# shendurelab/MIPGEN

Hardware: AMD Instinct MI355X
Metric: candidate MIPs scored/sec (SVR) (higher is better)
Workload: dtype f64

## Files before the change

### mipgen_amd/csrc/accel.hip

```cpp
#include "accel_internal.h"

thread_local char g_mipgen_accel_err[512] = "";

extern "C" {

int mipgen_accel_abi_version(void) { return MIPGEN_ACCEL_ABI_VERSION; }
const char* mipgen_accel_last_error(void) { return g_err; }

int mipgen_accel_device_count(void)
{
    int n = 0;
    if (hipGetDeviceCount(&n) != hipSuccess) return 0;
    return n;
}

int mipgen_accel_create(const mipgen_params* params, int device, void* stream, mipgen_accel** out)
{
    if (!params || !out) return fail(MIPGEN_E_INVALID, "null argument");
    *out = nullptr;
    if (params->abi_version != MIPGEN_ACCEL_ABI_VERSION) return fail(MIPGEN_E_INVALID, "abi_version %d != %d", params->abi_version, MIPGEN_ACCEL_ABI_VERSION);
    if (params->n_arm_pairs < 1 || params->n_arm_pairs > MIPGEN_MAX_ARM_PAIRS) return fail(MIPGEN_E_INVALID, "n_arm_pairs out of range");
    if (params->capture_increment <= 0) return fail(MIPGEN_E_INVALID, "capture_increment must be positive (the reference coerces 0 to 1 before this call)");
    if (params->max_capture_size < params->min_capture_size) return fail(MIPGEN_E_INVALID, "max_capture_size < min_capture_size");
    int ndev = mipgen_accel_device_count();
    if (ndev <= 0) return fail(MIPGEN_E_NODEVICE, "no HIP device: libmipgen_accel has no CPU path");
    if (device < 0 || device >= ndev) return fail(MIPGEN_E_INVALID, "device %d out of range (%d devices)", device, ndev);
    HIP_TRY(hipSetDevice(device));

    mipgen_accel* h = new mipgen_accel();
    h->copy.pool = h->scores.pool = h->partials.pool = h->records.pool = h->emitted.pool = h->survivors.pool = h->collapsed.pool = h->pos_region.pool =
        h->pos_local.pool = h->bases.pool = h->letters.pool = h->unmap.pool = h->fmt_pool.pool = h->fmt_text.pool = h->scan_temp.pool = &h->pool;
    h->device = device;
    h->params = *params;
    DevParams& D = h->hp;
    memset(&D, 0, sizeof D);
    D.min_capture = params->min_capture_size; D.max_capture = params->max_capture_size; D.inc = params->capture_increment;
    D.n_sizes_all = n_sizes_all(*params);
    D.n_pairs = params->n_arm_pairs;
    D.check_copy_number = params->check_copy_number; D.logistic_heuristic = params->logistic_heuristic;
    D.score_method = params->score_method;
    D.masked_arm_threshold = params->masked_arm_threshold; D.upper = params->upper_score_limit; D.lower = params->lower_score_limit;
    D.max_arm_copy_product = params->max_arm_copy_product; D.target_arm_copy = params->target_arm_copy;
    D.min_sum = 1 << 30; D.max_sum = 0; D.e_min = D.l_min = 1 << 30; D.e_max = D.l_max = 0;
    for (int i = 0; i <= MIPGEN_MAX_OLIGO; i++) D.len_slot[i] = -1;
    for (int i = 0; i < D.n_pairs; i++) {
        int e = params->arm_ext[i], l = params->arm_lig[i];
        if (e < 2 || l < 2 || e > MIPGEN_MAX_OLIGO || l > MIPGEN_MAX_OLIGO) { delete h; return fail(MIPGEN_E_INVALID, "arm length out of range [2,%d]", MIPGEN_MAX_OLIGO); }
        D.arm_ext[i] = (uint8_t)e; D.arm_lig[i] = (uint8_t)l;
        D.min_sum = std::min(D.min_sum, e + l); D.max_sum = std::max(D.max_sum, e + l);
        D.e_min = std::min(D.e_min, e); D.e_max = std::max(D.e_max, e);
        D.l_min = std::min(D.l_min, l); D.l_max = std::max(D.l_max, l);
        D.len_slot[e] = 0; D.len_slot[l] = 0;
    }
    if (params->min_capture_size - D.max_sum < 1) { delete h; return fail(MIPGEN_E_INVALID, "min_capture_size leaves no scan target (capture size <= arm length sum)"); }
    if ((params->arm_sum_key_max > 0 && params->arm_sum_key_max < D.max_sum) || (params->arm_sum_key_min > 0 && params->arm_sum_key_min > D.min_sum)) {
        delete h; return fail(MIPGEN_E_INVALID, "arm_sum_key_max / arm_sum_key_min inside the arm pairs' own sums [%d, %d]", D.min_sum, D.max_sum);
    }
    D.key_min_sum = params->arm_sum_key_min > 0 ? params->arm_sum_key_min : D.min_sum;
    if (params->min_capture_size - D.max_sum < 3) h->svr_geometry_error = "min_capture_size leaves a scan size < 3 (insert 3-mer frequencies are undefined)";
    int slot = 0;
    for (int i = 0; i <= MIPGEN_MAX_OLIGO; i++) if (D.len_slot[i] == 0) D.len_slot[i] = (int8_t)slot++;
    D.n_len_slots = slot;
    for (int i = 0; i < D.n_pairs;) {
        int j = i, s = D.arm_ext[i] + D.arm_lig[i];
        while (j < D.n_pairs && D.arm_ext[j] + D.arm_lig[j] == s) j++;
        for (int k = i; k < j; k++) D.group_end[k] = (uint16_t)j;
        i = j;
    }
    SvrGeom& G = h->geom;
    memset(&G, 0, sizeof G);
    G.nchunk = (D.n_pairs + SVR_MAX_CHUNK - 1) / SVR_MAX_CHUNK;
    G.chunk_len = (D.n_pairs + G.nchunk - 1) / G.nchunk;
    G.n_e = D.e_max - D.e_min + 1; G.n_l = D.l_max - D.l_min + 1;
    G.group = SVR_GROUP;
    G.wpc = 4;
    while (G.wpc > 1 && G.nchunk * G.wpc * 64 > SVR_MAX_THREADS) G.wpc--;
    if (G.nchunk * G.wpc * 64 > SVR_MAX_THREADS) {
        char msg[128];
        snprintf(msg, sizeof msg, "too many arm pairs for the dense SVR kernel (max %d)", SVR_MAX_CHUNK * (SVR_MAX_THREADS / 64));
        h->svr_geometry_error = msg;
        G.wpc = 1;
    }
    h->geom_few = G;
    h->have_few = false;
    if (h->svr_geometry_error.empty() && G.wpc == 4 && G.chunk_len > 8) {
        SvrGeom& F = h->geom_few;
        const int max_chunks = SVR_MAX_THREADS / 64 / 2;
        F.chunk_len = (D.n_pairs + max_chunks - 1) / max_chunks;
        F.nchunk = (D.n_pairs + F.chunk_len - 1) / F.chunk_len;
        F.wpc = 2;
        h->have_few = F.chunk_len < G.chunk_len && F.nchunk * F.wpc * 64 <= SVR_MAX_THREADS;
    }
    {
        const int n_arm = std::max(G.n_e, G.n_l) | 1;
        for (int strand = 0; strand < 2; strand++) {
            const int up_min = strand ? D.l_min : D.e_min, dn_min = strand ? D.e_min : D.l_min;
            for (int i = 0; i < MIPGEN_MAX_ARM_PAIRS + 16; i++) {
                const int a = std::min(i, D.n_pairs - 1);
                const int e = D.arm_ext[a], l = D.arm_lig[a];
                const uint32_t uU = (uint32_t)(((strand ? l : e) - up_min) * SVR_GROUP * 8);
                const uint32_t uD = (uint32_t)(((D.max_sum - (e + l)) * n_arm + ((strand ? e : l) - dn_min)) * SVR_GROUP * 8);
                D.pair_prog[strand][i] = uU | (uD << 16);
            }
        }
    }

    if (stream) { h->stream = (hipStream_t)stream; h->own_stream = false; }
    else {
        hipError_t e = hipStreamCreateWithFlags(&h->stream, hipStreamNonBlocking);
        if (e != hipSuccess) { delete h; return fail(MIPGEN_E_HIP, "hipStreamCreate: %s", hipGetErrorString(e)); }
        h->own_stream = true;
    }
    for (int i = 0; i < 101; i++) h->hconsts.log10_tab[i] = log10((double)i);
    h->hconsts.ln_base = log(MIPGEN_LOGISTIC_BASE);
    hipError_t e1 = hipMalloc((void**)&h->dp, sizeof(DevParams));
    hipError_t e2 = hipMalloc((void**)&h->dconsts, sizeof(HostConsts));
    if (e1 != hipSuccess || e2 != hipSuccess) { mipgen_accel_destroy(h); return fail(MIPGEN_E_NOMEM, "hipMalloc failed"); }
    if (hipHostMalloc((void**)&h->pb_over, sizeof(unsigned int), hipHostMallocMapped) != hipSuccess) { h->pb_over = nullptr; mipgen_accel_destroy(h); return fail(MIPGEN_E_NOMEM, "hipHostMalloc failed"); }
    *h->pb_over = 0u;
    hipError_t e3 = hipMemcpy(h->dp, &D, sizeof D, hipMemcpyHostToDevice);
    if (e3 == hipSuccess) e3 = hipMemcpy(h->dconsts, &h->hconsts, sizeof(HostConsts), hipMemcpyHostToDevice);
    if (e3 != hipSuccess) { mipgen_accel_destroy(h); return fail(MIPGEN_E_HIP, "hipMemcpy of the run parameters: %s", hipGetErrorString(e3)); }
    { int cus = 0; if (hipDeviceGetAttribute(&cus, hipDeviceAttributeMultiprocessorCount, device) == hipSuccess && cus > 0) h->n_cu = cus; }
    *out = h;
    return MIPGEN_OK;
}

void mipgen_accel_destroy(mipgen_accel* h)
{
    if (!h) return;
    (void)hipSetDevice(h->device);
    if (h->stream) (void)hipStreamSynchronize(h->stream);
    mipgen_reads_release(h);
    mipgen_consensus_release(h);
    h->call_run.release();
    h->locus_run.release();
    h->ins_call.release();
    h->locus_ins.release();
    h->locus_ins_call.release();
    h->model.release(); h->model_t.release(); h->sv_norm.release(); h->sv_coef.release(); h->sv_center.release(); h->regions.release(); h->bases.release(); h->unmap.release(); h->copy.release();
    h->log_tiles.release(); h->svr_tiles.release(); h->ld_tiles.release(); h->scores.release(); h->records.release();
    h->emitted.release(); h->survivors.release(); h->emitted_per_region.release(); h->pos_region.release(); h->pos_local.release();
    h->letters.release(); h->fmt_regions.release(); h->fmt_pool.release(); h->fmt_text.release(); h->scan_temp.release();
    h->fmt_a.release(); h->fmt_b.release(); h->fmt_c.release(); h->fmt_d.release();
    h->region_pos0.release(); h->region_base0.release(); h->col_tiles.release(); h->collapsed.release();
    h->cand_in.release(); h->cand_scores.release(); h->cand_feats.release(); h->cand_records.release(); h->cand_ints.release();
    h->win_img.release();
    h->pb.release(); h->sat.release(); h->surv_svr.release(); h->rs_keep.release(); h->rs_offs.release(); h->rs_idx.release();
    h->svr_tiles_lvl.release(); h->svr_tiles_kept.release(); h->run_bounds.release(); h->run_pbs.release(); h->run_state.release(); h->run_keep.release();
    h->run_offs.release(); h->skip_count.release();
    h->probe_recs.release(); h->probe_bytes.release(); h->probe_lrc.release(); h->probe_order.release();
    h->lrc_seq.release(); h->lrc_out.release(); h->lrc_offs.release(); h->lrc_lens.release(); h->lrc_denoms.release(); h->partials.release();
    h->pool.clear();
    if (h->dp) (void)hipFree(h->dp);
    if (h->dconsts) (void)hipFree(h->dconsts);
    if (h->pb_over) (void)hipHostFree(h->pb_over);
    for (hipEvent_t e : h->ev) if (e) (void)hipEventDestroy(e);
    if (h->own_stream && h->stream) (void)hipStreamDestroy(h->stream);
    delete h;
}

static int build_list_model(mipgen_accel* h, const std::vector<double>& rows, int n_sv)
{
    const int pad = std::max(64, (n_sv + 63) / 64 * 64);
    std::vector<double> center(MIPGEN_N_FEATURES, 0.0), mt((size_t)MIPGEN_N_FEATURES * pad, 0.0), sn((size_t)pad, 0.0), cf((size_t)pad, 0.0);
    for (int j = 0; j < MIPGEN_N_FEATURES; j++) {
        double s = 0.0;
        for (int i = 0; i < n_sv; i++) s += rows[(size_t)i * SV_ROW + j];
        center[(size_t)j] = n_sv ? s / n_sv : 0.0;
    }
    for (int i = 0; i < n_sv; i++) {
        double q = 0.0;
        for (int j = 0; j < MIPGEN_N_FEATURES; j++) {
            const double v = rows[(size_t)i * SV_ROW + j] - center[(size_t)j];
            mt[(size_t)j * pad + i] = v;
            q += v * v;
        }
        sn[(size_t)i] = q + rows[(size_t)i * SV_ROW + SVR_N_EXTRA];
        cf[(size_t)i] = rows[(size_t)i * SV_ROW + SVR_COEF];
    }
    if (h->model_t.reserve(mt.size()) || h->sv_norm.reserve(sn.size()) || h->sv_coef.reserve(cf.size()) || h->sv_center.reserve(center.size())) return MIPGEN_E_NOMEM;
    HIP_TRY(hipMemcpy(h->model_t.p, mt.data(), mt.size() * sizeof(double), hipMemcpyHostToDevice));
    HIP_TRY(hipMemcpy(h->sv_norm.p, sn.data(), sn.size() * sizeof(double), hipMemcpyHostToDevice));
    HIP_TRY(hipMemcpy(h->sv_coef.p, cf.data(), cf.size() * sizeof(double), hipMemcpyHostToDevice));
    HIP_TRY(hipMemcpy(h->sv_center.p, center.data(), center.size() * sizeof(double), hipMemcpyHostToDevice));
    h->n_sv_pad = pad;
    return MIPGEN_OK;
}

int mipgen_accel_set_model(mipgen_accel* h, int32_t n_sv, double gamma, double rho, const double* coef, const double* sv)
{
    if (!h || n_sv < 0 || (n_sv > 0 && (!coef || !sv))) return fail(MIPGEN_E_INVALID, "bad model arguments");
    HIP_TRY(hipSetDevice(h->device));
    std::vector<double> rows((size_t)std::max(n_sv, 1) * SV_ROW, 0.0);
    double s_guard = 0.0;
    for (int i = 0; i < n_sv; i++) {
        double* r = &rows[(size_t)i * SV_ROW];
        const double* x = sv + (size_t)i * MIPGEN_N_FEATURES;
        double ne = 0, ni = 0, nl = 0, nj = 0, tot = 0;
        for (int j = 0; j < MIPGEN_N_FEATURES; j++) {
            r[j] = x[j];
            double q = x[j] * x[j];
            tot += q;
            if (j <= 20) ne += q;
            else if (j >= F_INS && j <= 150) ni += q;
            else if (j >= F_LIG && j <= 172) nl += q;
            else if (j >= F_JUNC && j <= 189) nj += q;
        }
        r[SVR_COEF] = coef[i]; r[SVR_N_EXT] = ne; r[SVR_N_INS] = ni; r[SVR_N_LIG] = nl; r[SVR_N_JUNC] = nj;
        r[SVR_N_TOTAL] = tot; r[SVR_N_EXTRA] = 0.0;
        const int blk_base[3] = {F_EXT, F_INS, F_LIG}, blk_gc[3] = {F_EXT_GC, F_INS_GC, F_LIG_GC}, blk_step[3] = {5, 21, 5}, blk_thr[3] = {15, 63, 15};
        for (int b = 0; b < 3; b++)
            for (int c = 0; c < 4; c++) {
                const int idx = blk_step[b] * c;
                r[SVR_C1 + 4 * b + c] = x[blk_base[b] + idx + (idx >= blk_thr[b])] + ((c == BASE_C || c == BASE_G) ? x[blk_gc[b]] : 0.0);
            }
        s_guard += coef[i] * exp(-gamma * tot);
    }
    if (h->model.reserve(rows.size())) return MIPGEN_E_NOMEM;
    HIP_TRY(hipMemcpy(h->model.p, rows.data(), rows.size() * sizeof(double), hipMemcpyHostToDevice));
    h->n_sv = n_sv; h->gamma = gamma; h->rho = rho; h->s_guard = s_guard - rho;
    h->sum_abs_coef = 0.0;
    for (int i = 0; i < n_sv; i++) h->sum_abs_coef += fabs(coef[i]);
    return build_list_model(h, rows, n_sv);
}

int mipgen_accel_load_model_file(mipgen_accel* h, const char* path)
{
    if (!h || !path) return fail(MIPGEN_E_INVALID, "null argument");
    FILE* fp = fopen(path, "rb");
    if (!fp) return fail(MIPGEN_E_MODEL, "cannot open model file %s (the reference would dereference NULL here, svm.cpp:2507)", path);
    char cmd[128];
    std::string svm_type, kernel_type;
    double gamma = 0, rho = 0;
    int nr_class = 2, total_sv = -1;
    bool ok = true, seen_sv = false;
    while (ok && fscanf(fp, "%127s", cmd) == 1) {
        std::string c(cmd);
        if (c == "svm_type") { ok = fscanf(fp, "%127s", cmd) == 1; svm_type = cmd; }
        else if (c == "kernel_type") { ok = fscanf(fp, "%127s", cmd) == 1; kernel_type = cmd; }
        else if (c == "degree") { int d; ok = fscanf(fp, "%d", &d) == 1; }
        else if (c == "gamma") ok = fscanf(fp, "%lf", &gamma) == 1;
        else if (c == "coef0") { double d; ok = fscanf(fp, "%lf", &d) == 1; }
        else if (c == "nr_class") ok = fscanf(fp, "%d", &nr_class) == 1;
        else if (c == "total_sv") ok = fscanf(fp, "%d", &total_sv) == 1;
        else if (c == "rho") { int n = nr_class * (nr_class - 1) / 2; for (int i = 0; i < n && ok; i++) { double r; ok = fscanf(fp, "%lf", &r) == 1; if (i == 0) rho = r; } }
        else if (c == "label" || c == "nr_sv") { for (int i = 0; i < nr_class && ok; i++) { int d; ok = fscanf(fp, "%d", &d) == 1; } }
        else if (c == "probA" || c == "probB") { int n = nr_class * (nr_class - 1) / 2; for (int i = 0; i < n && ok; i++) { double d; ok = fscanf(fp, "%lf", &d) == 1; } }
        else if (c == "SV") { int ch; while ((ch = getc(fp)) != EOF && ch != '\n') {} seen_sv = true; break; }
        else { fclose(fp); return fail(MIPGEN_E_MODEL, "unknown text in model file: [%s]", cmd); }
    }
    if (!ok || !seen_sv || total_sv < 0) { fclose(fp); return fail(MIPGEN_E_MODEL, "malformed model header in %s", path); }
    if (svm_type != "epsilon_svr" && svm_type != "nu_svr") { fclose(fp); return fail(MIPGEN_E_MODEL, "svm_type %s unsupported (SVR only)", svm_type.c_str()); }
    if (kernel_type != "rbf") { fclose(fp); return fail(MIPGEN_E_MODEL, "kernel_type %s unsupported (rbf only)", kernel_type.c_str()); }
    std::vector<double> sv((size_t)std::max(total_sv, 1) * MIPGEN_N_FEATURES, 0.0), coef((size_t)std::max(total_sv, 1), 0.0), extra((size_t)std::max(total_sv, 1), 0.0);
    char* line = nullptr; size_t cap = 0;
    int got = 0;
    while (got < total_sv && getline(&line, &cap, fp) >= 0) {
        char* save = nullptr;
        char* p = strtok_r(line, " \t\n", &save);
        if (!p) continue;
        coef[got] = strtod(p, nullptr);
        for (int k = 1; k < nr_class - 1; k++) strtok_r(nullptr, " \t", &save);
        for (;;) {
            char* idx = strtok_r(nullptr, ":", &save);
            char* val = strtok_r(nullptr, " \t\n", &save);
            if (!val) break;
            long j = strtol(idx, nullptr, 10);
            double v = strtod(val, nullptr);
            if (j >= 1 && j <= MIPGEN_N_FEATURES) sv[(size_t)got * MIPGEN_N_FEATURES + (j - 1)] = v;
            else if (j > MIPGEN_N_FEATURES) extra[got] += v * v;
        }
        got++;
    }
    free(line);
    fclose(fp);
    if (got != total_sv) return fail(MIPGEN_E_MODEL, "model file has %d SV lines, header says %d", got, total_sv);
    int rc = mipgen_accel_set_model(h, total_sv, gamma, rho, coef.data(), sv.data());
    if (rc) return rc;
    bool any_extra = false;
    for (double x : extra) any_extra |= x != 0.0;
    if (any_extra) {
        std::vector<double> rows((size_t)total_sv * SV_ROW);
        HIP_TRY(hipMemcpy(rows.data(), h->model.p, rows.size() * sizeof(double), hipMemcpyDeviceToHost));
        double sg = 0;
        for (int i = 0; i < total_sv; i++) {
            rows[(size_t)i * SV_ROW + SVR_N_EXTRA] = extra[i];
            rows[(size_t)i * SV_ROW + SVR_N_TOTAL] += extra[i];
            sg += coef[i] * exp(-gamma * rows[(size_t)i * SV_ROW + SVR_N_TOTAL]);
        }
        HIP_TRY(hipMemcpy(h->model.p, rows.data(), rows.size() * sizeof(double), hipMemcpyHostToDevice));
        h->s_guard = sg - rho;
        return build_list_model(h, rows, total_sv);
    }
    return MIPGEN_OK;
}

int mipgen_accel_model_info(const mipgen_accel* h, int32_t* n_sv, double* gamma, double* rho)
{
    if (!h) return fail(MIPGEN_E_INVALID, "null handle");
    if (n_sv) *n_sv = h->n_sv;
    if (gamma) *gamma = h->gamma;
    if (rho) *rho = h->rho;
    return MIPGEN_OK;
}

int mipgen_accel_set_window_candidates(mipgen_accel* h, int64_t max_candidates)
{
    if (!h || max_candidates < 0) return fail(MIPGEN_E_INVALID, "bad arguments");
    h->window_cap = max_candidates;
    return MIPGEN_OK;
}

int mipgen_accel_set_window_breaks(mipgen_accel* h, const int32_t* first_regions, int32_t n)
{
    if (!h || n < 0 || (n > 0 && !first_regions)) return fail(MIPGEN_E_INVALID, "bad arguments");
    for (int i = 0; i < n; i++)
        if (first_regions[i] < 0 || (i > 0 && first_regions[i] <= first_regions[i - 1])) return fail(MIPGEN_E_INVALID, "window breaks must be ascending batch indices");
    h->window_breaks.assign(first_regions, first_regions + n);
    return MIPGEN_OK;
}

int mipgen_accel_set_print_exact(mipgen_accel* h, int32_t on)
{
    if (!h) return fail(MIPGEN_E_INVALID, "null handle");
    h->print_exact = on != 0;
    return MIPGEN_OK;
}

int mipgen_accel_set_logistic_subruns(mipgen_accel* h, int32_t n)
{
    if (!h || n < 0 || n > 8) return fail(MIPGEN_E_INVALID, "bad arguments");
    h->ld_subruns = n;
    h->logistic_tiles_ready = false;
    return MIPGEN_OK;
}

int mipgen_accel_set_sv_split(mipgen_accel* h, int32_t n_split)
{
    if (!h || n_split < 0 || n_split > 64) return fail(MIPGEN_E_INVALID, "n_split must be in [0, 64] (0 = automatic)");
    h->sv_split = n_split;
    return MIPGEN_OK;
}


int mipgen_accel_upload_regions(mipgen_accel* h, const mipgen_region* regions, int32_t n, mipgen_grid* grids_out)
{
    if (!h || n < 0 || (n > 0 && !regions)) return fail(MIPGEN_E_INVALID, "bad arguments");
    DIAG_CLOCK("upload");
    HIP_TRY(hipSetDevice(h->device));
    const mipgen_params& P = h->params;
    const DevParams& D = h->hp;
    h->cur_window = -1;
    h->windows.clear(); h->win_state.clear();
    h->hregions.assign((size_t)n, DevRegion());
    h->grids.assign((size_t)n, mipgen_grid());
    int64_t seq_total = 0, copy_total = 0, unmap_total = 0, cand_total = 0, pos_total = 0, cand_max = 0;
    int n_resident = 0;
    for (int i = 0; i < n; i++) n_resident += regions[i].copy == MIPGEN_COPY_RESIDENT;
    if (n_resident) {
        bool same = n_resident == n && h->resident_lens.size() == (size_t)n;
        for (int i = 0; same && i < n; i++) same = h->resident_lens[(size_t)i] == regions[i].seq_len;
        if (!same) return fail(MIPGEN_E_INVALID, "MIPGEN_COPY_RESIDENT: the batch is not the one mipgen_accel_count_oligo_copies_resident counted (regions, order, seq_len)");
    } else {
        h->resident_lens.clear();
    }
    for (int i = 0; i < n; i++) {
        const mipgen_region& R = regions[i];
        if (!R.seq || R.seq_len <= 0) return fail(MIPGEN_E_INVALID, "region %d has no sequence", i);
        if (R.seq_stop - R.seq_start + 1 != R.seq_len) return fail(MIPGEN_E_INVALID, "region %d: seq_len %d != seq_stop-seq_start+1 = %d", i, R.seq_len, R.seq_stop - R.seq_start + 1);
        DevRegion& d = h->hregions[i];
        mipgen_grid& g = h->grids[i];
        grid_of(P, D, R, &g);
        g.offset = cand_total;
        d.seq_off = seq_total;
        d.seq_len = R.seq_len; d.seq_start = R.seq_start; d.seq_stop = R.seq_stop;
        d.start_fl = R.start_flanked; d.stop_fl = R.stop_flanked;
        d.first_pos = g.first_pos; d.n_pos = g.n_pos; d.k0 = g.first_size_index; d.n_sizes = g.n_sizes;
        d.copy_off = R.copy ? copy_total : -1;
        d.unmap_off = R.unmappable ? unmap_total : -1;
        memcpy(d.lrc, R.long_range_content, sizeof d.lrc);
        seq_total += R.seq_len;
        if (R.copy) copy_total += (int64_t)D.n_len_slots * R.seq_len;
        if (R.unmappable) unmap_total += (int64_t)D.n_sizes_all * R.seq_len;
        cand_total += g.count;
        pos_total += g.n_pos;
        cand_max = std::max(cand_max, g.count);
    }
    if (pos_total > INT32_MAX) return fail(MIPGEN_E_INVALID, "batch has %lld scan positions (max %d): split the design", (long long)pos_total, INT32_MAX);
    DIAG_LAP("layout");
    uint8_t code_lut[256];
    for (int c = 0; c < 256; c++) code_lut[c] = base_code((char)c);
    std::vector<uint8_t> hb((size_t)std::max<int64_t>(seq_total, 1));
    std::vector<char> hl((size_t)std::max<int64_t>(seq_total, 1));
    std::vector<uint8_t> hu((size_t)std::max<int64_t>(unmap_total, 1));
    for (int i = 0; i < n; i++) {
        const mipgen_region& R = regions[i];
        const DevRegion& d = h->hregions[i];
        uint8_t* b = &hb[(size_t)d.seq_off];
        memcpy(&hl[(size_t)d.seq_off], R.seq, (size_t)R.seq_len);
        const char* ms = R.masked_seq ? R.masked_seq : R.seq;
        if (R.snp_class) for (int k = 0; k < R.seq_len; k++) b[k] = (uint8_t)(code_lut[(uint8_t)R.seq[k]] | (ms[k] == 'N' ? BASE_MASKED_BIT : 0) | ((R.snp_class[k] & 3) << BASE_SNP_SHIFT));
        else for (int k = 0; k < R.seq_len; k++) b[k] = (uint8_t)(code_lut[(uint8_t)R.seq[k]] | (ms[k] == 'N' ? BASE_MASKED_BIT : 0));
        if (R.unmappable) memcpy(&hu[(size_t)d.unmap_off], R.unmappable, (size_t)D.n_sizes_all * R.seq_len);
    }
    DIAG_LAP("pack");
    if (h->letters.reserve(hl.size())) return MIPGEN_E_NOMEM;
    HIP_TRY(hipMemcpyAsync(h->letters.p, hl.data(), hl.size(), hipMemcpyHostToDevice, h->stream));
    HIP_TRY(hipStreamSynchronize(h->stream));
    if (h->regions.reserve((size_t)std::max(n, 1)) || h->bases.reserve(hb.size()) || h->copy.reserve((size_t)std::max<int64_t>(copy_total, 1)) || h->unmap.reserve(hu.size()) ||
        h->survivors.reserve((size_t)std::max<int64_t>(2 * pos_total, 1)) || h->emitted_per_region.reserve((size_t)std::max(n, 1)) ||
        h->pos_region.reserve((size_t)std::max<int64_t>(pos_total, 1)) || h->pos_local.reserve((size_t)std::max<int64_t>(pos_total, 1)))
        return MIPGEN_E_NOMEM;

    DIAG_LAP("input buffers");
    int64_t cap = h->window_cap;
    if (cap <= 0) {
        size_t free_b = 0, total_b = 0;
        HIP_TRY(hipMemGetInfo(&free_b, &total_b));
        const int64_t have = (int64_t)(h->scores.cap * 8 + h->records.cap * 8 + h->emitted.cap) + (int64_t)free_b + (int64_t)h->pool.held();
        cap = std::max<int64_t>(1, (int64_t)((double)have * 0.85) / 17);
        cap = std::min<int64_t>(cap, std::max<int64_t>((int64_t)1 << 30, cand_max));
    }
    if (cand_max > cap && h->window_cap > 0) cap = cand_max;
    if (cand_max > cap) return fail(MIPGEN_E_NOMEM, "a single region has %lld dense candidates; device memory holds %lld", (long long)cand_max, (long long)cap);
    {
        Window w;
        size_t nb = 0;
        for (int i = 0; i < n; i++) {
            const mipgen_grid& g = h->grids[i];
            while (nb < h->window_breaks.size() && h->window_breaks[nb] < i) nb++;
            const bool forced = nb < h->window_breaks.size() && h->window_breaks[nb] == i;
            if (w.r1 > w.r0 && (forced || w.n_cand + g.count > cap)) {
                h->windows.push_back(w);
                Window nw; nw.r0 = nw.r1 = i; nw.cand0 = w.cand0 + w.n_cand; nw.pos0 = w.pos0 + w.n_pos;
                w = nw;
            }
            h->hregions[i].out_off = w.n_cand;
            w.n_cand += g.count; w.n_pos += g.n_pos; w.r1 = i + 1;
        }
        h->windows.push_back(w);
        h->win_state.assign(h->windows.size(), 0);
    }
    int64_t win_cand_max = 0;
    for (const Window& w : h->windows) win_cand_max = std::max(win_cand_max, w.n_cand);

    std::vector<int64_t> rpos0((size_t)n + 1, 0);
    h->h_region_base0.assign((size_t)n + 1, 0);
    for (int i = 0; i < n; i++) {
        const DevRegion& d = h->hregions[i];
        const int max_scan = D.max_capture - d.k0 * D.inc - D.min_sum;
        const int64_t nb = (d.n_pos > 0 && d.n_sizes > 0) ? (int64_t)d.n_pos + max_scan - 1 : 0;
        rpos0[(size_t)i + 1] = rpos0[(size_t)i] + d.n_pos;
        h->h_region_base0[(size_t)i + 1] = h->h_region_base0[(size_t)i] + 2 * nb;
    }
    std::vector<CollapseTile> ct;
    for (Window& w : h->windows) {
        w.col_tile0 = (int)ct.size();
        w.base0 = h->h_region_base0[(size_t)w.r0]; w.n_base_entries = h->h_region_base0[(size_t)w.r1] - w.base0;
        w.log_tile0 = w.n_log_tiles = w.svr_tile0 = w.n_svr_tiles = w.ld_tile0 = w.n_ld_tiles = 0;
        for (int i = w.r0; i < w.r1; i++) {
            const DevRegion& d = h->hregions[i];
            if (d.n_pos <= 0 || d.n_sizes <= 0) continue;
            for (int64_t j0 = 0; 2 * j0 < h->h_region_base0[(size_t)i + 1] - h->h_region_base0[(size_t)i]; j0 += 128) { CollapseTile t = {i, (int32_t)j0}; ct.push_back(t); }
        }
        w.n_col_tiles = (int)ct.size() - w.col_tile0;
    }
    h->record_tiles_ready = h->logistic_tiles_ready = h->svr_tiles_ready = false;
    h->svr_batch_error.clear();
    h->ld_lds = 0; h->log_span_max = 0; h->svr_lds = 0;
    DIAG_LAP("tiles");
    if (h->scores.reserve((size_t)std::max<int64_t>(win_cand_max, 1)) || h->records.reserve((size_t)std::max<int64_t>(win_cand_max, 1)) ||
        h->emitted.reserve((size_t)std::max<int64_t>(win_cand_max, 1)))
        return MIPGEN_E_NOMEM;
    if (h->region_pos0.reserve((size_t)n + 1) || h->region_base0.reserve((size_t)n + 1) || h->col_tiles.reserve(std::max<size_t>(ct.size(), 1)) ||
        h->collapsed.reserve((size_t)std::max<int64_t>(h->h_region_base0[(size_t)n], 1)))
        return MIPGEN_E_NOMEM;
    HIP_TRY(hipMemcpyAsync(h->region_pos0.p, rpos0.data(), ((size_t)n + 1) * sizeof(int64_t), hipMemcpyHostToDevice, h->stream));
    HIP_TRY(hipMemcpyAsync(h->region_base0.p, h->h_region_base0.data(), ((size_t)n + 1) * sizeof(int64_t), hipMemcpyHostToDevice, h->stream));
    if (!ct.empty()) HIP_TRY(hipMemcpyAsync(h->col_tiles.p, ct.data(), ct.size() * sizeof(CollapseTile), hipMemcpyHostToDevice, h->stream));
    HIP_TRY(mipgen_launch_fill_pos_map(h->stream, h->region_pos0.p, n, pos_total, h->pos_region.p, h->pos_local.p));
    if (n > 0) HIP_TRY(hipMemcpyAsync(h->regions.p, h->hregions.data(), (size_t)n * sizeof(DevRegion), hipMemcpyHostToDevice, h->stream));
    HIP_TRY(hipMemcpyAsync(h->bases.p, hb.data(), hb.size(), hipMemcpyHostToDevice, h->stream));
    if (copy_total && !n_resident) {
        int64_t max_block = 0;
        for (int i = 0; i < n; i++) if (regions[i].copy) max_block = std::max(max_block, (int64_t)D.n_len_slots * regions[i].seq_len);
        const int64_t chunk = std::min(copy_total, std::max<int64_t>((int64_t)1 << 20, max_block));
        PinnedPair<int32_t> pin;
        HIP_TRY(pin.alloc((size_t)chunk));
        int cur = 0;
        int64_t fill = 0, base = 0;
        auto flush = [&]() -> hipError_t {
            if (fill == 0) return hipSuccess;
            hipError_t e = hipMemcpyAsync(h->copy.p + base, pin.buf[cur], (size_t)fill * sizeof(int32_t), hipMemcpyHostToDevice, h->stream);
            if (e == hipSuccess) e = hipEventRecord(pin.done[cur], h->stream);
            if (e != hipSuccess) return e;
            pin.busy[cur] = true;
            base += fill; fill = 0; cur ^= 1;
            return pin.wait(cur);
        };
        for (int i = 0; i < n; i++) {
            const mipgen_region& R = regions[i];
            if (!R.copy) continue;
            const int64_t block = (int64_t)D.n_len_slots * R.seq_len;
            if (fill + block > chunk) HIP_TRY(flush());
            if (h->hregions[i].copy_off != base + fill) return fail(MIPGEN_E_INVALID, "internal: copy table offsets out of order");
            for (int len = 0; len <= MIPGEN_MAX_OLIGO; len++) {
                const int s = D.len_slot[len];
                if (s < 0) continue;
                int32_t* dst = pin.buf[cur] + fill + (int64_t)s * R.seq_len;
                if (R.copy[len]) memcpy(dst, R.copy[len], (size_t)R.seq_len * sizeof(int32_t));
                else memset(dst, 0, (size_t)R.seq_len * sizeof(int32_t));
            }
            fill += block;
        }
        HIP_TRY(flush());
        HIP_TRY(pin.wait(0)); HIP_TRY(pin.wait(1));
    }
    if (unmap_total) HIP_TRY(hipMemcpyAsync(h->unmap.p, hu.data(), hu.size(), hipMemcpyHostToDevice, h->stream));
    HIP_TRY(hipStreamSynchronize(h->stream));
    DIAG_LAP("buffers + copies");
    h->n_regions = n; h->n_cand = cand_total; h->total_pos = pos_total;
    h->ev_used.assign(h->windows.size(), 0);
#ifdef MIPGEN_DIAG
    fprintf(stderr, "[mipgen_accel] batch: %d regions, %lld candidates in %zu window(s)\n", n, (long long)cand_total, h->windows.size());
#endif
    if (grids_out) memcpy(grids_out, h->grids.data(), (size_t)n * sizeof(mipgen_grid));
    return MIPGEN_OK;
}

int64_t mipgen_accel_batch_candidates(const mipgen_accel* h) { return h ? h->n_cand : 0; }
int32_t mipgen_accel_window_count(const mipgen_accel* h) { return h ? (int32_t)h->windows.size() : 0; }

int mipgen_accel_window_info(const mipgen_accel* h, int32_t w, int32_t* first_region, int32_t* n_regions, int64_t* first_candidate,
                             int64_t* n_candidates, int64_t* first_position, int64_t* n_positions)
{
    if (!h || w < 0 || w >= (int32_t)h->windows.size()) return fail(MIPGEN_E_INVALID, "window %d out of range", w);
    const Window& W = h->windows[(size_t)w];
    if (first_region) *first_region = W.r0;
    if (n_regions) *n_regions = W.r1 - W.r0;
    if (first_candidate) *first_candidate = W.cand0;
    if (n_candidates) *n_candidates = W.n_cand;
    if (first_position) *first_position = W.pos0;
    if (n_positions) *n_positions = W.n_pos;
    return MIPGEN_OK;
}


double mipgen_accel_last_kernel_ms(mipgen_accel* h, int32_t which)
{
    if (h && which == 4) return h->kmer_count_ms;
    if (h && which == 5) return h->list_svr_ms;
    if (h && which == 6) return h->list_feat_ms;
    if (h && which == 7) return h->reads_assign_ms;
    if (h && which == 8) return h->sample_assign_ms;
    if (h && which == 9) return h->consensus_vote_ms;
    if (h && which == 10) return h->consensus_sort_ms;
    if (h && which == 11) return h->pileup_ms;
    if (h && which == 12) return h->gapped_ms;
    if (h && which == 13) return h->call_ms;
    if (h && which == 14) return h->locus_ms;
    if (h && which == 15) return h->insertions_ms;
    if (h && which == 16) return h->ins_call_ms;
    if (h && which == 17) return h->locus_ins_ms;
    if (h && which == 18) return h->tag_merge_ms;
    if (h && which == 19) return h->deletions_ms;
    if (!h || !h->timing) return -1.0;
    if (hipSetDevice(h->device) != hipSuccess) return -1.0;
    double total = 0.0;
    bool any = false;
    for (size_t w = 0; w < h->windows.size() && 4 * (w + 1) <= h->ev.size(); w++) {
        const uint8_t used = h->ev_used[w];
        if (!(used & 1)) continue;
        hipEvent_t* ev = &h->ev[4 * w];
        float ms = 0.f;
        hipError_t e = hipSuccess;
        if (which == 3) {
            if (!(used & 2)) continue;
            if (hipEventSynchronize(ev[3]) != hipSuccess) return -1.0;
            e = hipEventElapsedTime(&ms, ev[2], ev[3]);
        } else {
            if (hipEventSynchronize(ev[2]) != hipSuccess) return -1.0;
            if (which == 0) e = hipEventElapsedTime(&ms, ev[1], ev[2]);
            else if (which == 2) e = hipEventElapsedTime(&ms, ev[0], ev[1]);
            else e = hipEventElapsedTime(&ms, ev[0], ev[2]);
        }
        if (e != hipSuccess) return -1.0;
        total += ms; any = true;
    }
    return any ? total : -1.0;
}

int mipgen_accel_set_timing(mipgen_accel* h, int32_t enabled)
{
    if (!h) return fail(MIPGEN_E_INVALID, "null handle");
    h->timing = enabled != 0;
    std::fill(h->ev_used.begin(), h->ev_used.end(), 0);
    return MIPGEN_OK;
}

}
```

### mipgen_amd/csrc/accel_internal.h

```cpp
#pragma once
#include <hip/hip_runtime.h>

#include <algorithm>
#include <chrono>
#include <cmath>
#include <cstdarg>
#include <cstdio>
#include <cstdlib>
#include <cstring>
#include <string>
#include <unordered_map>
#include <vector>

#include "kernels.h"
#include "logistic_device.h"

extern thread_local char g_mipgen_accel_err[512];
#define g_err g_mipgen_accel_err
static inline int fail(int code, const char* fmt, ...)
{
    va_list ap;
    va_start(ap, fmt);
    vsnprintf(g_err, sizeof g_err, fmt, ap);
    va_end(ap);
    return code;
}
#define HIP_TRY(expr)                                                                             \
    do {                                                                                          \
        hipError_t e__ = (expr);                                                                  \
        if (e__ != hipSuccess) return fail(MIPGEN_E_HIP, "%s: %s", #expr, hipGetErrorString(e__)); \
    } while (0)

struct Window {
    int r0 = 0, r1 = 0;
    int64_t cand0 = 0, n_cand = 0;
    int64_t pos0 = 0, n_pos = 0;
    int log_tile0 = 0, n_log_tiles = 0, svr_tile0 = 0, n_svr_tiles = 0, col_tile0 = 0, n_col_tiles = 0, ld_tile0 = 0, n_ld_tiles = 0;
    int n_svr_few = 0;
    std::vector<int> lvl_tile0;
    int lvl0_few = 0;
    int64_t base0 = 0, n_base_entries = 0;
};

struct DevPool {
    struct Block { void* p; size_t bytes; };
    std::vector<Block> blocks;
    size_t held() const { size_t n = 0; for (const Block& b : blocks) n += b.bytes; return n; }
    void* take(size_t bytes, size_t* got)
    {
        int best = -1;
        for (int i = 0; i < (int)blocks.size(); i++)
            if (blocks[(size_t)i].bytes >= bytes && blocks[(size_t)i].bytes / 4 <= bytes && (best < 0 || blocks[(size_t)i].bytes < blocks[(size_t)best].bytes)) best = i;
        if (best < 0) return nullptr;
        void* p = blocks[(size_t)best].p;
        *got = blocks[(size_t)best].bytes;
        blocks.erase(blocks.begin() + best);
        return p;
    }
    void give(void* p, size_t bytes) { if (bytes >= ((size_t)1 << 20)) blocks.push_back({p, bytes}); else (void)hipFree(p); }
    void clear() { for (const Block& b : blocks) (void)hipFree(b.p); blocks.clear(); }
};

template <typename T>
struct DevBuf {
    T* p = nullptr;
    size_t cap = 0;
    DevPool* pool = nullptr;
    int reserve(size_t n)
    {
        if (n <= cap) return 0;
        release();
        size_t want = n + std::min<size_t>(n / 8, (size_t)1 << 20) + 64;
        if (pool) {
            size_t got = 0;
            if (void* q = pool->take(want * sizeof(T), &got)) { p = (T*)q; cap = got / sizeof(T); return 0; }
        }
        hipError_t e = hipMalloc((void**)&p, want * sizeof(T));
        if (e != hipSuccess && pool && !pool->blocks.empty()) {
            (void)hipGetLastError();
            pool->clear();
            e = hipMalloc((void**)&p, want * sizeof(T));
        }
        if (e != hipSuccess) { p = nullptr; return fail(MIPGEN_E_NOMEM, "hipMalloc(%zu bytes): %s", want * sizeof(T), hipGetErrorString(e)); }
        cap = want;
        return 0;
    }
    void release()
    {
        if (p) { if (pool) pool->give(p, cap * sizeof(T)); else (void)hipFree(p); }
        p = nullptr; cap = 0;
    }
};
static inline size_t padded(size_t count, size_t size) { return (count + count / 8 + 64) * size; }

struct SortedPairs {
    DevBuf<uint64_t> keys, keys_sorted;
    DevBuf<uint32_t> ids, ids_sorted;
    DevBuf<char> temp;
    size_t held() const { return (keys.cap + keys_sorted.cap) * 8 + (ids.cap + ids_sorted.cap) * 4 + temp.cap; }
    void release() { keys.release(); keys_sorted.release(); ids.release(); ids_sorted.release(); temp.release(); }
    static size_t bytes(size_t n, size_t scratch) { return 2 * padded(n, 8) + 2 * padded(n, 4) + padded(scratch, 1); }
    static hipError_t scratch_bytes(hipStream_t st, int64_t n, int end_bit, int64_t n_runs, int64_t n_scan, size_t* scratch)
    {
        size_t t_sort = 0, t_runs = 0, t_scan = 0;
        hipError_t e = mipgen_consensus_sort(st, nullptr, &t_sort, nullptr, nullptr, nullptr, nullptr, n, end_bit);
        if (e == hipSuccess && n_runs) e = mipgen_consensus_runs(st, nullptr, &t_runs, nullptr, n_runs, nullptr, nullptr, nullptr);
        if (e == hipSuccess && n_scan) e = mipgen_consensus_scan_u32(st, nullptr, &t_scan, nullptr, nullptr, n_scan);
        *scratch = std::max<size_t>(std::max(t_sort, std::max(t_runs, t_scan)), 1);
        return e;
    }
    int reserve(size_t n, size_t scratch) { return keys.reserve(n) || keys_sorted.reserve(n) || ids.reserve(n) || ids_sorted.reserve(n) || temp.reserve(scratch) ? MIPGEN_E_NOMEM : MIPGEN_OK; }
    hipError_t sort(hipStream_t st, int64_t n, int end_bit) { size_t all = temp.cap; return mipgen_consensus_sort(st, temp.p, &all, keys.p, keys_sorted.p, ids.p, ids_sorted.p, n, end_bit); }
    hipError_t runs(hipStream_t st, int64_t n, uint64_t* run_keys, int32_t* run_counts, unsigned long long* n_runs) { size_t all = temp.cap; return mipgen_consensus_runs(st, temp.p, &all, keys_sorted.p, n, run_keys, run_counts, n_runs); }
    hipError_t scan_u32(hipStream_t st, const int32_t* in, uint32_t* out, int64_t n) { size_t all = temp.cap; return mipgen_consensus_scan_u32(st, temp.p, &all, in, out, n); }
    hipError_t scan_i64(hipStream_t st, const int64_t* in, int64_t* out, int64_t n) { size_t all = temp.cap; return mipgen_consensus_scan_i64(st, temp.p, &all, in, out, n); }
};

template <typename T>
struct PinnedPair {
    T* buf[2] = {nullptr, nullptr};
    hipEvent_t done[2] = {nullptr, nullptr};
    bool busy[2] = {false, false};
    hipError_t alloc(size_t n)
    {
        for (int b = 0; b < 2; b++) {
            hipError_t e = hipHostMalloc((void**)&buf[b], std::max<size_t>(n, 1) * sizeof(T), hipHostMallocDefault);
            if (e != hipSuccess) return e;
            e = hipEventCreateWithFlags(&done[b], hipEventDisableTiming);
            if (e != hipSuccess) return e;
        }
        return hipSuccess;
    }
    hipError_t wait(int b) { hipError_t e = busy[b] ? hipEventSynchronize(done[b]) : hipSuccess; busy[b] = false; return e; }
    ~PinnedPair() { for (int b = 0; b < 2; b++) { if (done[b]) { if (busy[b]) (void)hipEventSynchronize(done[b]); (void)hipEventDestroy(done[b]); } if (buf[b]) (void)hipHostFree(buf[b]); } }
};

enum : uint8_t {
    WIN_SURVIVORS = 1,
    WIN_MASK = 2,
    WIN_COLLAPSED = 4,
    WIN_SURV_SVR = 8,
    WIN_TEXT = 16,
};

struct RescoreList {
    DevBuf<mipgen_candidate> cands; DevBuf<int64_t> idx; DevBuf<double> vals; DevBuf<unsigned int> count;
    void release() { cands.release(); idx.release(); vals.release(); count.release(); }
};

struct ReadsSession;

struct RowScratch {
    DevBuf<int32_t> mol_len;
    DevBuf<int64_t> pos_off;
    DevBuf<uint32_t> start;
    DevBuf<uint2> units;
    DevBuf<PileupCounters> pctr;
    size_t held() const { return mol_len.cap * 4 + pos_off.cap * 8 + start.cap * 4 + units.cap * 8 + pctr.cap * sizeof(PileupCounters); }
    void release() { mol_len.release(); pos_off.release(); start.release(); units.release(); pctr.release(); }
};
struct CountScratch {
    RowScratch row;
    DevBuf<int32_t> counts;
    DevBuf<int64_t> proj_off;
    DevBuf<uint32_t> list;
    DevBuf<uint8_t> mol_seq, need, proj;
    DevBuf<GappedCounters> ctr;
    size_t held() const { return row.held() + counts.cap * 4 + proj_off.cap * 8 + list.cap * 4 + mol_seq.cap + need.cap + proj.cap + ctr.cap * sizeof(GappedCounters); }
    void release() { row.release(); counts.release(); proj_off.release(); list.release(); mol_seq.release(); need.release(); proj.release(); ctr.release(); }
};
struct RowArgs;
struct PoolArgs {
    bool have = false;
    std::vector<int32_t> mol_len;
    std::string mol_seq;
    int32_t min_family = 1, min_quality = 0, max_indel = 0, bg_max_ppm = 0;
    void remember(const RowArgs& A, int64_t n_pos, int32_t bg_max_ppm_);
};
struct PoolState : PoolArgs {
    DevBuf<int32_t> pool;
    mipgen_gapped_totals last{0, 0, 0, 0, 0, 0, 0, 0};
    bool have_last = false;
    void drop() { have = have_last = false; }
    void release() { drop(); pool.release(); }
};
struct CallScratch {
    CountScratch pile, gapped;
    PoolState state;
    DevBuf<uint8_t> ref;
    size_t held() const { return pile.held() + gapped.held() + state.pool.cap * 4 + ref.cap; }
    void release() { state.release(); pile.release(); gapped.release(); ref.release(); }
};
struct CallRun {
    DevBuf<mipgen_call_record> cand, records;
    SortedPairs pairs;
    DevBuf<CallCounters> ctr;
    DevBuf<int32_t> counts, pool;
    DevBuf<uint8_t> ref;
    int64_t n_calls = -1;
    size_t held() const { return (cand.cap + records.cap) * sizeof(mipgen_call_record) + pairs.held() + ctr.cap * sizeof(CallCounters) + (counts.cap + pool.cap) * 4 + ref.cap; }
    void release() { cand.release(); records.release(); pairs.release(); ctr.release(); counts.release(); pool.release(); ref.release(); n_calls = -1; }
};
struct LocusPlan {
    DevBuf<int64_t> plan;
    SortedPairs pairs;
    DevBuf<uint32_t> src, first;
    int64_t n_pos = 0, n_loci = 0;
    bool have = false;
    size_t held() const { return plan.cap * 8 + pairs.held() + (src.cap + first.cap) * 4; }
    void release_transient() { plan.release(); pairs.release(); }
    void release() { release_transient(); src.release(); first.release(); have = false; n_pos = n_loci = 0; }
};
struct LocusRun {
    LocusPlan plan;
    DevBuf<int32_t> counts, merged;
    DevBuf<LocusCounters> ctr;
    size_t held() const { return plan.held() + (counts.cap + merged.cap) * 4 + ctr.cap * sizeof(LocusCounters); }
    void release() { plan.release(); counts.release(); merged.release(); ctr.release(); }
};
struct LocusScratch {
    LocusPlan plan;
    DevBuf<uint8_t> ref;
    CountScratch pile, gapped;
    DevBuf<int32_t> merged;
    DevBuf<LocusCounters> ctr;
    PoolState state;
    size_t held() const { return plan.held() + ref.cap + pile.held() + gapped.held() + (merged.cap + state.pool.cap) * 4 + ctr.cap * sizeof(LocusCounters); }
    void release() { plan.release(); ref.release(); pile.release(); gapped.release(); merged.release(); ctr.release(); state.release(); }
};
struct InsScratch {
    CountScratch count;
    DevBuf<int32_t> anchors;
    DevBuf<InsCounters> ctr;
    SortedPairs pairs;
    DevBuf<mipgen_insertion_record> records;
    int64_t n_alleles = -1;
    size_t event_held() const { return pairs.held() + records.cap * sizeof(mipgen_insertion_record); }
    size_t table_held() const { return anchors.cap * 4 + ctr.cap * sizeof(InsCounters); }
    void release() { count.release(); anchors.release(); ctr.release(); pairs.release(); records.release(); n_alleles = -1; }
};
struct DelScratch {
    CountScratch count;
    DevBuf<int32_t> sites;
    DevBuf<DelCounters> ctr;
    SortedPairs pairs;
    DevBuf<mipgen_deletion_record> records;
    int64_t n_alleles = -1;
    size_t event_held() const { return pairs.held() + records.cap * sizeof(mipgen_deletion_record); }
    size_t table_held() const { return sites.cap * 4 + ctr.cap * sizeof(DelCounters); }
    void release() { count.release(); sites.release(); ctr.release(); pairs.release(); records.release(); n_alleles = -1; }
};
struct InsPool {
    PoolArgs args;
    DevBuf<int32_t> S;
    DevBuf<uint64_t> pool_keys;
    DevBuf<InsPoolSums> pool_sums;
    DevBuf<InsPoolCounters> ctr;
    SortedPairs pairs;
    DevBuf<InsPoolSums> sums;
    DevBuf<uint32_t> run_start;
    DevBuf<int32_t> run_counts;
    int64_t n_pos = 0, rows = 0, n_entries = 0, n_alleles = 0;
    size_t entry_held() const { return pairs.held() + pool_keys.cap * 8 + (sums.cap + pool_sums.cap) * sizeof(InsPoolSums) + (run_start.cap + run_counts.cap) * 4; }
    size_t table_held() const { return S.cap * 4 + ctr.cap * sizeof(InsPoolCounters); }
    void release_transient() { pairs.release(); sums.release(); run_start.release(); run_counts.release(); }
    void release() { args.have = false; release_transient(); S.release(); pool_keys.release(); pool_sums.release(); ctr.release(); n_pos = rows = n_entries = n_alleles = 0; }
};
struct InsCallRun {
    CallRun run;
    DevBuf<mipgen_insertion_call_record> out;
    DevBuf<mipgen_insertion_record> records;
    DevBuf<int32_t> span, pool_span;
    DevBuf<uint64_t> pool_keys;
    DevBuf<InsPoolSums> pool_sums;
    int64_t n_calls = -1;
    size_t call_held() const { return run.held() + out.cap * sizeof(mipgen_insertion_call_record); }
    size_t upload_held() const { return records.cap * sizeof(mipgen_insertion_record) + (span.cap + pool_span.cap) * 4 + pool_keys.cap * 8 + pool_sums.cap * sizeof(InsPoolSums); }
    void release() { run.release(); out.release(); records.release(); span.release(); pool_span.release(); pool_keys.release(); pool_sums.release(); n_calls = -1; }
};
struct LocusInsMap {
    DevBuf<uint32_t> own, prev;
    bool have = false;
    size_t held() const { return (own.cap + prev.cap) * 4; }
    void release() { own.release(); prev.release(); have = false; }
};
struct LocusInsFold {
    SortedPairs pairs;
    DevBuf<uint32_t> run_start;
    DevBuf<mipgen_insertion_record> records;
    DevBuf<int32_t> anchors;
    DevBuf<LocusInsCounters> ctr;
    int64_t n_alleles = -1;
    size_t pair_held() const { return pairs.held() + run_start.cap * 4 + records.cap * sizeof(mipgen_insertion_record); }
    size_t table_held() const { return anchors.cap * 4 + ctr.cap * sizeof(LocusInsCounters); }
    void release() { pairs.release(); run_start.release(); records.release(); anchors.release(); ctr.release(); n_alleles = -1; }
};
struct LocusInsRun {
    LocusPlan plan;
    LocusInsMap map;
    DevBuf<mipgen_insertion_record> records;
    DevBuf<int32_t> anchors;
    LocusInsFold fold;
    size_t upload_held() const { return records.cap * sizeof(mipgen_insertion_record) + anchors.cap * 4; }
    void release() { plan.release(); map.release(); records.release(); anchors.release(); fold.release(); }
};
struct LocusInsScratch {
    LocusInsMap map;
    InsPool pool;
    void drop() { map.have = false; pool.args.have = false; }
    void release() { map.release(); pool.release(); }
};
struct ConsensusResult {
    int64_t n_groups = 0, ext_bytes = 0, lig_bytes = 0;
    int64_t n = 0, rows = 0;
    CountScratch pile, gapped;
    CallScratch call;
    LocusScratch locus;
    InsScratch ins;
    InsPool ins_pool;
    LocusInsScratch locus_ins;
    DelScratch del;
    DevBuf<uint64_t> keys;
    DevBuf<int32_t> family;
    DevBuf<int64_t> ext_off, lig_off;
    DevBuf<uint8_t> ext_seq, ext_qual, lig_seq, lig_qual;
    mipgen_tag_merge_totals tag_totals{0, 0, 0, 0, 0};
    bool merged = false;
    DevBuf<uint64_t> raw_keys;
    DevBuf<int32_t> raw_family, raw_root;
    ConsensusView view() const { return {keys.p, family.p, ext_off.p, lig_off.p, ext_seq.p, ext_qual.p, lig_seq.p, lig_qual.p, n_groups}; }
    void release() { keys.release(); family.release(); ext_off.release(); lig_off.release(); ext_seq.release(); ext_qual.release(); lig_seq.release(); lig_qual.release(); raw_keys.release(); raw_family.release(); raw_root.release(); pile.release(); gapped.release(); call.release(); locus.release(); ins.release(); ins_pool.release(); locus_ins.release(); del.release(); }
};

struct mipgen_accel {
    int device = 0;
    hipStream_t stream = nullptr;
    bool own_stream = false;
    mipgen_params params;
    DevParams hp;
    DevParams* dp = nullptr;
    HostConsts* dconsts = nullptr;
    HostConsts hconsts;
    SvrGeom geom;
    SvrGeom geom_few;
    bool have_few = false;
    int n_sv = 0;
    double gamma = 0, rho = 0, s_guard = 0;
    DevBuf<double> model;
    std::string svr_geometry_error;
    std::string svr_batch_error;
    bool record_tiles_ready = false, logistic_tiles_ready = false, svr_tiles_ready = false;
    int sv_split = 0;
    int ld_subruns = 0;
    int n_cu = 256;
    int n_regions = 0;
    int64_t n_cand = 0;
    int64_t total_pos = 0;
    std::vector<DevRegion> hregions;
    std::vector<mipgen_grid> grids;
    DevBuf<DevRegion> regions;
    DevBuf<uint8_t> bases, unmap;
    DevBuf<char> letters;
    DevBuf<FmtRegion> fmt_regions;
    DevBuf<char> fmt_pool, fmt_text, scan_temp;
    DevBuf<int64_t> fmt_a, fmt_b, fmt_c, fmt_d;
    int64_t fmt_bytes = 0;
    DevPool pool;
    DevBuf<int32_t> copy;
    std::vector<int32_t> resident_lens;
    std::vector<mipgen_big_copy> big_copies;
    DevBuf<LogTile> log_tiles;
    DevBuf<SvrTile> svr_tiles, ld_tiles;
    size_t ld_lds = 0;
    int log_span_max = 0;
    size_t svr_lds = 0;
    int64_t window_cap = 0;
    std::vector<int32_t> window_breaks;
    std::vector<Window> windows;
    int cur_window = -1;
    std::vector<uint8_t> win_state;
    DevBuf<double> scores, partials;
    DevBuf<uint64_t> records;
    DevBuf<uint8_t> emitted;
    DevBuf<mipgen_survivor> survivors;
    DevBuf<unsigned long long> emitted_per_region;
    DevBuf<int32_t> pos_region, pos_local;
    std::vector<int64_t> h_region_base0;
    DevBuf<int64_t> region_pos0, region_base0;
    DevBuf<CollapseTile> col_tiles;
    DevBuf<int32_t> collapsed;
    bool print_exact = true;
    double sum_abs_coef = 0.0;
    RescoreList pb;
    DevBuf<double> surv_svr;
    DevBuf<int64_t> rs_keep, rs_offs, rs_idx;
    RescoreList sat;
    DevBuf<uint8_t> win_img;
    std::vector<int64_t> win_roff;
    std::vector<int32_t> win_lens;
    int win_sizes = 0;
    int64_t win_total = 0;
    bool dyn_skip = false;
    int svr_levels = 1;
    DevBuf<SvrTile> svr_tiles_lvl, svr_tiles_kept;
    DevBuf<uint32_t> run_bounds;
    DevBuf<double> run_pbs;
    DevBuf<uint8_t> run_state;
    DevBuf<int64_t> run_keep, run_offs;
    DevBuf<unsigned long long> skip_count;
    unsigned long long skipped_total = 0;
    bool skip_count_valid = false;
    unsigned int* pb_over = nullptr;
    DevBuf<double> model_t, sv_norm, sv_coef, sv_center;
    int n_sv_pad = 0;
    double kmer_count_ms = -1.0;
    double list_feat_ms = -1.0, list_svr_ms = -1.0;
    int64_t kmer_genome_bytes = 0;
    DevBuf<mipgen_candidate> cand_in;
    DevBuf<double> cand_scores, cand_feats;
    DevBuf<uint64_t> cand_records;
    DevBuf<mipgen_candidate_ints> cand_ints;
    DevBuf<ProbeRec> probe_recs;
    DevBuf<uint8_t> probe_bytes;
    DevBuf<double> probe_lrc;
    DevBuf<int32_t> probe_order;
    DevBuf<char> lrc_seq;
    DevBuf<double> lrc_out;
    DevBuf<int64_t> lrc_offs;
    DevBuf<int32_t> lrc_lens, lrc_denoms;
    ReadsSession* reads = nullptr;
    int64_t reads_key_cap = 0;
    double reads_assign_ms = -1.0;
    double sample_assign_ms = -1.0;
    ConsensusResult* consensus = nullptr;
    double consensus_vote_ms = -1.0;
    double consensus_sort_ms = -1.0;
    double tag_merge_ms = -1.0;
    double pileup_ms = -1.0;
    double gapped_ms = -1.0;
    CallRun call_run;
    double call_ms = -1.0;
    LocusRun locus_run;
    double locus_ms = -1.0;
    double insertions_ms = -1.0;
    InsCallRun ins_call;
    double ins_call_ms = -1.0;
    LocusInsRun locus_ins;
    InsCallRun locus_ins_call;
    double locus_ins_ms = -1.0;
    double deletions_ms = -1.0;
    bool timing = false;
    std::vector<hipEvent_t> ev;
    std::vector<uint8_t> ev_used;
};

static inline int n_sizes_all(const mipgen_params& P)
{
    if (P.max_capture_size < P.min_capture_size) return 0;
    return (P.max_capture_size - P.min_capture_size) / P.capture_increment + 1;
}

static inline void grid_of(const mipgen_params& P, const DevParams& D, const mipgen_region& R, mipgen_grid* g)
{
    int cur = R.start_flanked - P.max_capture_size + (P.arm_sum_key_max > 0 ? P.arm_sum_key_max : D.max_sum);
    if (cur < 0) cur = 0;
    g->first_pos = cur + 1;
    g->n_pos = std::max(0, R.stop_flanked - cur);
    int K = D.n_sizes_all, k0 = 0;
    while (k0 < K) {
        int C = P.max_capture_size - k0 * P.capture_increment;
        if (C > R.stop_flanked - R.start_flanked + P.max_mip_overlap && C - P.capture_increment >= P.min_capture_size) k0++;
        else break;
    }
    g->first_size_index = k0;
    g->n_sizes = K - k0;
    g->count = (int64_t)g->n_pos * g->n_sizes * P.n_arm_pairs * 2;
    g->offset = 0;
}

static inline bool win_has(const mipgen_accel* h, int w, uint8_t bits) { return w >= 0 && (h->win_state[(size_t)w] & bits) == bits; }
static inline void win_set(mipgen_accel* h, int w, uint8_t bits) { h->win_state[(size_t)w] |= bits; }

static inline uint8_t base_code(char c)
{
    switch (c) {
        case 'A': return BASE_A; case 'C': return BASE_C; case 'G': return BASE_G; case 'T': return BASE_T;
        case 'N': return BASE_N; case '-': return BASE_DASH; default: return BASE_OTHER;
    }
}

#ifdef MIPGEN_DIAG
struct DiagClock {
    const char* what; std::chrono::steady_clock::time_point t = std::chrono::steady_clock::now();
    explicit DiagClock(const char* w) : what(w) {}
    void lap(const char* stage) { const auto n_ = std::chrono::steady_clock::now(); fprintf(stderr, "[mipgen_accel] %s: %s %.3f s\n", what, stage, std::chrono::duration<double>(n_ - t).count()); t = n_; }
};
#define DIAG_CLOCK(name) DiagClock diag_clock(name)
#define DIAG_LAP(stage) diag_clock.lap(stage)
#else
#define DIAG_CLOCK(name) do { } while (0)
#define DIAG_LAP(stage) do { } while (0)
#endif

static inline int free_device_bytes(size_t* free_b)
{
    size_t total_b = 0;
    HIP_TRY(hipMemGetInfo(free_b, &total_b));
    return MIPGEN_OK;
}
struct IdleOnExit { hipStream_t s; bool idle = false; hipError_t wait() { idle = true; return hipStreamSynchronize(s); } ~IdleOnExit() { if (!idle) (void)hipStreamSynchronize(s); } };

struct SpanTimer {
    bool on;
    hipStream_t st;
    std::vector<hipEvent_t> ev;
    ~SpanTimer() { for (hipEvent_t e : ev) (void)hipEventDestroy(e); }
    void mark() { hipEvent_t e = nullptr; if (on && (on = hipEventCreate(&e) == hipSuccess)) { ev.push_back(e); (void)hipEventRecord(e, st); } }
    int add_to(double* sum) const
    {
        int n = 0;
        float ms = 0.f;
        for (size_t k = 0; on && k + 1 < ev.size(); k += 2)
            if (hipEventElapsedTime(&ms, ev[k], ev[k + 1]) == hipSuccess) { *sum += ms; n++; }
        return n;
    }
};

extern "C" {
int mipgen_pick_sv_split(int n_tiles, int n_sv, int n_cu);
int mipgen_ensure_events(mipgen_accel* h);
int mipgen_ensure_tiles(mipgen_accel* h, int32_t method);
int mipgen_pb_check(mipgen_accel* h);
void mipgen_reads_release(mipgen_accel* h);
void mipgen_consensus_release(mipgen_accel* h);
}
```

### mipgen_amd/csrc/accel_score.hip

```cpp
#include "accel_internal.h"

extern "C" {

int mipgen_pb_check(mipgen_accel* h)
{
    if (!h->pb_over || *h->pb_over == 0u) return MIPGEN_OK;
    const unsigned int v = *h->pb_over;
    *h->pb_over = 0u;
    return fail(MIPGEN_E_STATE, "print-exact re-score: %u scores on a 6-digit rounding boundary did not fit the re-score list "
                                "(mipgen_accel_set_print_exact(h, 0) waives the guarantee)", v);
}

struct RescoreLimits { unsigned int cap; double tol_rel, tol_abs; };
static RescoreLimits rescore_limits(const mipgen_accel* h, int kind, int method, int64_t n)
{
    const bool svr = method == MIPGEN_SCORE_SVR;
    int64_t cap;
    if (kind == RESCORE_SATURATED) cap = std::min<int64_t>(n / 4096 + 4096, (int64_t)1 << 20);
    else if (kind == RESCORE_SURV) cap = svr ? std::min<int64_t>(n / 256 + 1024, (int64_t)1 << 22) : std::min<int64_t>(n / 4096 + 64, (int64_t)1 << 20);
    else cap = svr ? std::min<int64_t>(n / 1024 + 4096, (int64_t)1 << 24) : std::min<int64_t>(n / 8192 + 256, (int64_t)1 << 22);
    return {(unsigned int)cap, svr ? 1e-10 : 1e-11, svr ? 1e-13 * std::max(1.0, h->sum_abs_coef) : 1e-300};
}

static ListSrc list_src(const mipgen_accel* h, const mipgen_candidate* cands, const ProbeSrc* ps)
{
    if (ps) return {LIST_PROBES, {}, *ps};
    return {LIST_BATCH, {h->dp, h->regions.p, cands, h->bases.p, h->copy.p, h->unmap.p}, {}};
}

static int rescore(mipgen_accel* h, const RescoreSrc& src, int method, const ProbeSrc* ps = nullptr)
{
    const bool sat = src.kind == RESCORE_SATURATED;
    if (!sat && (!h->print_exact || src.n <= 0 || (method == MIPGEN_SCORE_SVR && h->n_sv <= 0))) return MIPGEN_OK;
    const RescoreLimits lim = rescore_limits(h, src.kind, method, src.n);
    RescoreList& L = sat ? h->sat : h->pb;
    if ((!ps && L.cands.reserve(lim.cap)) || L.idx.reserve(lim.cap) || L.vals.reserve(lim.cap) || L.count.reserve(1)) return MIPGEN_E_NOMEM;
    if (sat) HIP_TRY(mipgen_launch_index_candidates(h->stream, h->dp, h->regions.p, src.r0, src.r1, L.idx.p, L.count.p, lim.cap, L.cands.p));
    else {
        HIP_TRY(hipMemsetAsync(L.count.p, 0, sizeof(unsigned int), h->stream));
        HIP_TRY(mipgen_launch_print_boundary_scan(h->stream, h->dp, h->regions.p, &src, lim.tol_rel, lim.tol_abs, L.cands.p, L.idx.p, L.count.p, lim.cap, h->n_cu));
    }
    ListSrc listed = list_src(h, L.cands.p, ps);
    if (ps) { listed.probes.sel = L.idx.p; listed.probes.order = nullptr; }
    HIP_TRY(mipgen_launch_candidates(h->stream, (int)lim.cap, listed, h->dconsts, h->model.p, h->n_sv, h->gamma, h->rho, method, L.vals.p, nullptr, nullptr, nullptr, 1,
                                     L.count.p));
    HIP_TRY(mipgen_launch_scatter_scores(h->stream, L.vals.p, L.idx.p, lim.cap, L.count.p, src.scores, src.surv, sat ? nullptr : h->pb_over));
    return MIPGEN_OK;
}

static int device_scan_i64(mipgen_accel* h, const int64_t* in, int64_t* out, int64_t n)
{
    size_t temp_bytes = 0;
    HIP_TRY(mipgen_scan_i64(h->stream, nullptr, &temp_bytes, in, out, n));
    if (h->scan_temp.reserve(temp_bytes + 16)) return MIPGEN_E_NOMEM;
    HIP_TRY(mipgen_scan_i64(h->stream, h->scan_temp.p, &temp_bytes, in, out, n));
    return MIPGEN_OK;
}

static int fix_survivor_print_boundaries(mipgen_accel* h, int w, int method)
{
    const Window& W = h->windows[(size_t)w];
    return rescore(h, {RESCORE_SURV, 2 * W.n_pos, nullptr, nullptr, nullptr, h->survivors.p + 2 * W.pos0, W.r0, W.r1, W.cand0}, method);
}

static bool list_is_batched(int n, int method, bool want_scores) { return method == MIPGEN_SCORE_SVR && n >= 256 && want_scores; }
static bool list_runs_feature_kernel(int n, int method, bool want_scores, bool ints) { return list_is_batched(n, method, want_scores) && !ints; }

static int score_list(mipgen_accel* h, int n, int method, bool want_scores, bool features, bool ints, hipEvent_t* le, const ProbeSrc* ps = nullptr)
{
    const bool batched = list_is_batched(n, method, want_scores);
    if (batched && h->cand_feats.reserve((size_t)n * MIPGEN_N_FEATURES)) return MIPGEN_E_NOMEM;
    const bool time_list = le && batched && !ints && h->timing;
    if (time_list) { for (int k = 0; k < 3; k++) HIP_TRY(hipEventCreate(&le[k])); HIP_TRY(hipEventRecord(le[0], h->stream)); }
    const ListSrc src = list_src(h, h->cand_in.p, ps);
    if (list_runs_feature_kernel(n, method, want_scores, ints))
        HIP_TRY(mipgen_launch_features_batch(h->stream, n, src, h->dconsts, h->cand_records.p, h->cand_feats.p));
    else
        HIP_TRY(mipgen_launch_candidates(h->stream, n, src, h->dconsts, h->model.p, h->n_sv, h->gamma, h->rho, method, batched ? nullptr : h->cand_scores.p,
                                         h->cand_records.p, (features || batched) ? h->cand_feats.p : nullptr, ints ? h->cand_ints.p : nullptr, 0, nullptr));
    if (time_list) HIP_TRY(hipEventRecord(le[1], h->stream));
    if (batched) HIP_TRY(mipgen_launch_svr_gemm(h->stream, n, h->cand_feats.p, h->cand_records.p, h->model_t.p, h->sv_norm.p, h->sv_coef.p, h->sv_center.p, h->n_sv_pad,
                                            h->gamma, h->rho, h->cand_scores.p));
    if (time_list) HIP_TRY(hipEventRecord(le[2], h->stream));
    if (!batched) return MIPGEN_OK;
    return rescore(h, {ps ? RESCORE_PROBES : RESCORE_LIST, n, h->cand_scores.p, h->cand_records.p, ps ? nullptr : h->cand_in.p, nullptr, 0, 0, 0}, MIPGEN_SCORE_SVR, ps);
}

static int svr_window_via_list(mipgen_accel* h, const Window& W)
{
    const int64_t CH = (int64_t)1 << 19;
    const size_t n_max = (size_t)std::min<int64_t>(CH, std::max<int64_t>(W.n_cand, 1));
    if (h->cand_in.reserve(n_max) || h->cand_records.reserve(n_max) || h->cand_feats.reserve(n_max * MIPGEN_N_FEATURES)) return MIPGEN_E_NOMEM;
    for (int64_t c0 = 0; c0 < W.n_cand; c0 += CH) {
        const int n = (int)std::min<int64_t>(CH, W.n_cand - c0);
        HIP_TRY(mipgen_launch_dense_candidates(h->stream, h->dp, h->regions.p, W.r0, W.r1, c0, n, h->cand_in.p));
        HIP_TRY(mipgen_launch_features_batch(h->stream, n, list_src(h, h->cand_in.p, nullptr), h->dconsts, h->cand_records.p, h->cand_feats.p));
        HIP_TRY(mipgen_launch_svr_gemm(h->stream, n, h->cand_feats.p, h->cand_records.p, h->model_t.p, h->sv_norm.p, h->sv_coef.p, h->sv_center.p, h->n_sv_pad,
                                       h->gamma, h->rho, h->scores.p + c0));
        HIP_TRY(mipgen_launch_dense_list_fix(h->stream, n, h->records.p + c0, h->rho, h->s_guard, h->scores.p + c0));
    }
    return MIPGEN_OK;
}

static int score_window_impl(mipgen_accel* h, int w, int32_t method, bool fix_dense = true)
{
    if (int rc = mipgen_ensure_tiles(h, method)) return rc;
    const Window& W = h->windows[(size_t)w];
    const bool svr_via_list = method == MIPGEN_SCORE_SVR && (!h->svr_geometry_error.empty() || !h->svr_batch_error.empty());
    if (svr_via_list && h->model_t.p == nullptr) return fail(MIPGEN_E_MODEL, "SVR scoring requested but no model is loaded");
    hipEvent_t* ev = nullptr;
    if (h->timing) { if (mipgen_ensure_events(h)) return MIPGEN_E_HIP; ev = &h->ev[4 * (size_t)w]; }
    if (ev) HIP_TRY(hipEventRecord(ev[0], h->stream));
    unsigned int sat_cap = 0;
    if (method == MIPGEN_SCORE_LOGISTIC) {
        sat_cap = rescore_limits(h, RESCORE_SATURATED, method, W.n_cand).cap;
        if (h->sat.idx.reserve(sat_cap) || h->sat.count.reserve(1)) return MIPGEN_E_NOMEM;
        HIP_TRY(hipMemsetAsync(h->sat.count.p, 0, sizeof(unsigned int), h->stream));
    }
    if (method == MIPGEN_SCORE_LOGISTIC && h->ld_lds > 0)
        HIP_TRY(mipgen_launch_logistic_dense(h->stream, W.n_ld_tiles, h->ld_lds, h->dp, h->regions.p, h->ld_tiles.p + W.ld_tile0, h->bases.p, h->copy.p,
                                             h->unmap.p, h->dconsts, h->scores.p, h->records.p, h->sat.idx.p, h->sat.count.p, sat_cap));
    else
        HIP_TRY(mipgen_launch_records_logistic(h->stream, method == MIPGEN_SCORE_LOGISTIC, W.n_log_tiles, h->log_span_max, h->dp, h->regions.p,
                                               h->log_tiles.p + W.log_tile0, h->bases.p, h->copy.p, h->unmap.p, h->dconsts, h->scores.p, h->records.p,
                                               sat_cap ? h->sat.idx.p : nullptr, sat_cap ? h->sat.count.p : nullptr, sat_cap));
    if (ev) HIP_TRY(hipEventRecord(ev[1], h->stream));
    if (sat_cap) { if (int rc = rescore(h, {RESCORE_SATURATED, W.n_cand, h->scores.p, nullptr, nullptr, nullptr, W.r0, W.r1, 0}, method)) return rc; }
    if (svr_via_list) {
        if (int rc = svr_window_via_list(h, W)) return rc;
    } else if (method == MIPGEN_SCORE_SVR) {
        const double gamma_l2e = h->gamma * 1.4426950408889634074;
        int split = h->sv_split > 0 ? h->sv_split : mipgen_pick_sv_split(W.n_svr_tiles, h->n_sv, h->n_cu);
        split = std::max(1, std::min(split, (h->n_sv + SVR_GROUP - 1) / SVR_GROUP));
        if (split > 1 && h->partials.reserve((size_t)(split - 1) * (size_t)std::max<int64_t>(W.n_cand, 1))) return MIPGEN_E_NOMEM;
        const int levels = (int)W.lvl_tile0.size() - 1;
        if (h->dyn_skip && h->svr_levels > 1 && levels > 1) {
            int max_run = 0;
            for (int l = 0; l < levels; l++) max_run = std::max(max_run, W.lvl_tile0[(size_t)l + 1] - W.lvl_tile0[(size_t)l]);
            if (h->run_pbs.reserve((size_t)W.n_pos) || h->run_state.reserve((size_t)W.n_pos) || h->run_keep.reserve((size_t)max_run + 1) ||
                h->run_offs.reserve((size_t)max_run + 1) || h->svr_tiles_kept.reserve((size_t)max_run) || h->skip_count.reserve(1))
                return MIPGEN_E_NOMEM;
            HIP_TRY(hipMemsetAsync(h->run_pbs.p, 0, (size_t)W.n_pos * sizeof(double), h->stream));
            HIP_TRY(hipMemsetAsync(h->run_state.p, 0, (size_t)W.n_pos, h->stream));
            if (!h->skip_count_valid) { HIP_TRY(hipMemsetAsync(h->skip_count.p, 0, sizeof(unsigned long long), h->stream)); h->skip_count_valid = true; }
            const double margin = 1e-6 * std::max(1.0, fabs(h->hp.upper)) + 1e-12 * std::max(1.0, h->sum_abs_coef);
            for (int l = 0; l < levels; l++) {
                const SvrTile* tl = h->svr_tiles_lvl.p + W.lvl_tile0[(size_t)l];
                int nt = W.lvl_tile0[(size_t)l + 1] - W.lvl_tile0[(size_t)l];
                if (l > 0 && nt > 0) {
                    HIP_TRY(mipgen_launch_svr_run_state(h->stream, W.n_pos, h->dp, h->regions.p, h->pos_region.p + W.pos0, h->pos_local.p + W.pos0, h->run_bounds.p,
                                                        h->svr_levels, l - 1, margin, h->scores.p, h->records.p, h->run_pbs.p, h->run_state.p));
                    HIP_TRY(mipgen_launch_svr_tile_keep(h->stream, nt, tl, h->region_pos0.p, W.pos0, h->run_state.p, h->run_keep.p));
                    if (int rc = device_scan_i64(h, h->run_keep.p, h->run_offs.p, (int64_t)nt + 1)) return rc;
                    HIP_TRY(mipgen_launch_svr_tile_compact(h->stream, nt, tl, h->run_keep.p, h->run_offs.p, h->svr_tiles_kept.p, h->dp, h->regions.p, h->scores.p,
                                                           h->skip_count.p));
                    int64_t kept = 0;
                    HIP_TRY(hipMemcpyAsync(&kept, h->run_offs.p + nt, sizeof kept, hipMemcpyDeviceToHost, h->stream));
                    HIP_TRY(hipStreamSynchronize(h->stream));
                    tl = h->svr_tiles_kept.p; nt = (int)kept;
                }
                const int nt_few = l == 0 ? W.lvl0_few : 0;
                HIP_TRY(mipgen_launch_svr_dense(h->stream, nt - nt_few, nt_few, h->svr_lds, h->dp, &h->geom, &h->geom_few, h->regions.p, tl, h->bases.p, h->copy.p,
                                                (const double*)h->dconsts, h->model.p, h->n_sv, gamma_l2e, h->rho, h->s_guard, h->records.p, h->scores.p, W.n_cand, 1,
                                                nullptr));
            }
        } else
        HIP_TRY(mipgen_launch_svr_dense(h->stream, W.n_svr_tiles - W.n_svr_few, W.n_svr_few, h->svr_lds, h->dp, &h->geom, &h->geom_few, h->regions.p,
                                        h->svr_tiles.p + W.svr_tile0, h->bases.p, h->copy.p, (const double*)h->dconsts ,
                                        h->model.p, h->n_sv, gamma_l2e, h->rho, h->s_guard, h->records.p, h->scores.p, W.n_cand, split, h->partials.p));
    }
    if (fix_dense) { if (int rc = rescore(h, {RESCORE_DENSE, W.n_cand, h->scores.p, h->records.p, nullptr, nullptr, W.r0, W.r1, 0}, method)) return rc; }
    if (ev) { HIP_TRY(hipEventRecord(ev[2], h->stream)); h->ev_used[(size_t)w] |= 1; }
    if (h->cur_window >= 0) h->win_state[(size_t)h->cur_window] &= (uint8_t)~(WIN_MASK | WIN_TEXT);
    h->win_state[(size_t)w] = 0; h->cur_window = w;
    return MIPGEN_OK;
}

static int replay_window_impl(mipgen_accel* h, bool want_mask)
{
    const int w = h->cur_window;
    const Window& W = h->windows[(size_t)w];
    if (W.r1 > W.r0) HIP_TRY(hipMemsetAsync(h->emitted_per_region.p + W.r0, 0, (size_t)(W.r1 - W.r0) * sizeof(unsigned long long), h->stream));
    if (want_mask && W.n_cand) HIP_TRY(hipMemsetAsync(h->emitted.p, 0, (size_t)W.n_cand, h->stream));
    HIP_TRY(mipgen_launch_replay_condense(h->stream, (int)W.n_pos, h->dp, h->hp.n_pairs, h->hp.n_sizes_all, h->regions.p, h->pos_region.p + W.pos0,
                                          h->pos_local.p + W.pos0, h->scores.p, h->records.p, h->copy.p, W.cand0, want_mask ? h->emitted.p : nullptr,
                                          h->survivors.p + 2 * W.pos0, h->emitted_per_region.p));
    if (h->timing && h->ev.size() >= 4 * ((size_t)w + 1)) { HIP_TRY(hipEventRecord(h->ev[4 * (size_t)w + 3], h->stream)); h->ev_used[(size_t)w] |= 2; }
    h->win_state[(size_t)w] = (uint8_t)((h->win_state[(size_t)w] & WIN_TEXT) | WIN_SURVIVORS | (want_mask ? WIN_MASK : 0));
    return MIPGEN_OK;
}

static int collapse_window_impl(mipgen_accel* h)
{
    const Window& W = h->windows[(size_t)h->cur_window];
    HIP_TRY(mipgen_launch_collapse(h->stream, W.n_col_tiles, h->col_tiles.p + W.col_tile0, h->dp, h->regions.p, h->region_pos0.p, h->region_base0.p,
                                   h->survivors.p, h->copy.p, W.cand0, h->collapsed.p, h->hp.max_capture - h->hp.min_sum));
    win_set(h, h->cur_window, WIN_COLLAPSED);
    return MIPGEN_OK;
}

static int check_scoring_args(mipgen_accel* h, int32_t method)
{
    if (!h) return fail(MIPGEN_E_INVALID, "null handle");
    if (method != MIPGEN_SCORE_LOGISTIC && method != MIPGEN_SCORE_SVR) return fail(MIPGEN_E_INVALID, "method must be logistic or svr");
    if (h->windows.empty()) return fail(MIPGEN_E_STATE, "no resident region batch");
    if (method == MIPGEN_SCORE_SVR && h->n_sv <= 0 && h->model.p == nullptr) return fail(MIPGEN_E_MODEL, "SVR scoring requested but no model is loaded");
    return MIPGEN_OK;
}

static int begin_scoring_call(mipgen_accel* h, int32_t method, int32_t w)
{
    if (int rc = check_scoring_args(h, method)) return rc;
    if (w < 0 || w >= (int32_t)h->windows.size()) return fail(MIPGEN_E_INVALID, "window %d out of range (%zu windows)", w, h->windows.size());
    HIP_TRY(hipSetDevice(h->device));
    std::fill(h->ev_used.begin(), h->ev_used.end(), 0);
    return MIPGEN_OK;
}

int mipgen_accel_score_window(mipgen_accel* h, int32_t w, int32_t method)
{
    if (int rc = begin_scoring_call(h, method, w)) return rc;
    return score_window_impl(h, w, method);
}

int mipgen_accel_score_resident(mipgen_accel* h, int32_t method)
{
    if (int rc = check_scoring_args(h, method)) return rc;
    if (h->windows.size() != 1)
        return fail(MIPGEN_E_STATE, "the resident batch spans %zu result windows: use mipgen_accel_score_window / mipgen_accel_score_condense_all", h->windows.size());
    return mipgen_accel_score_window(h, 0, method);
}

int mipgen_accel_score_condense_window(mipgen_accel* h, int32_t w, int32_t method)
{
    if (int rc = begin_scoring_call(h, method, w)) return rc;
    if (int rc = score_window_impl(h, w, method, false)) return rc;
    if (int rc = replay_window_impl(h, false)) return rc;
    return fix_survivor_print_boundaries(h, w, method);
}

int mipgen_accel_score_condense_all(mipgen_accel* h, int32_t method)
{
    if (int rc = begin_scoring_call(h, method, 0)) return rc;
    for (int w = 0; w < (int)h->windows.size(); w++) {
        if (int rc = score_window_impl(h, w, method, false)) return rc;
        if (int rc = replay_window_impl(h, false)) return rc;
        if (int rc = fix_survivor_print_boundaries(h, w, method)) return rc;
        if (int rc = collapse_window_impl(h)) return rc;
    }
    return MIPGEN_OK;
}

int mipgen_accel_set_dynamic_skip(mipgen_accel* h, int32_t on)
{
    if (!h) return fail(MIPGEN_E_INVALID, "null handle");
    h->dyn_skip = on != 0;
    return MIPGEN_OK;
}

int mipgen_accel_skip_state(mipgen_accel* h, uint8_t* state, double* previous_best, int64_t capacity)
{
    if (!h || capacity < 0) return fail(MIPGEN_E_INVALID, "bad arguments");
    if (h->cur_window < 0 || !h->run_state.p) return fail(MIPGEN_E_STATE, "no window scored with the dynamic skip");
    const Window& W = h->windows[(size_t)h->cur_window];
    if (capacity < W.n_pos) return fail(MIPGEN_E_INVALID, "capacity %lld < %lld scan positions", (long long)capacity, (long long)W.n_pos);
    HIP_TRY(hipSetDevice(h->device));
    if (state) HIP_TRY(hipMemcpyAsync(state, h->run_state.p, (size_t)W.n_pos, hipMemcpyDeviceToHost, h->stream));
    if (previous_best) HIP_TRY(hipMemcpyAsync(previous_best, h->run_pbs.p, (size_t)W.n_pos * sizeof(double), hipMemcpyDeviceToHost, h->stream));
    HIP_TRY(hipStreamSynchronize(h->stream));
    return MIPGEN_OK;
}

int mipgen_accel_skipped_candidates(mipgen_accel* h, int64_t* n)
{
    if (!h || !n) return fail(MIPGEN_E_INVALID, "bad arguments");
    *n = 0;
    if (!h->skip_count_valid) return MIPGEN_OK;
    HIP_TRY(hipSetDevice(h->device));
    unsigned long long v = 0;
    HIP_TRY(hipMemcpyAsync(&v, h->skip_count.p, sizeof v, hipMemcpyDeviceToHost, h->stream));
    HIP_TRY(hipMemsetAsync(h->skip_count.p, 0, sizeof v, h->stream));
    HIP_TRY(hipStreamSynchronize(h->stream));
    *n = (int64_t)v;
    return MIPGEN_OK;
}

int mipgen_accel_result_device_ptrs(const mipgen_accel* h, void** scores_dev, void** records_dev)
{
    if (!h) return fail(MIPGEN_E_INVALID, "null handle");
    if (scores_dev) *scores_dev = h->scores.p;
    if (records_dev) *records_dev = h->records.p;
    return MIPGEN_OK;
}

int mipgen_accel_download_results(mipgen_accel* h, double* scores, uint64_t* records, int64_t first, int64_t count)
{
    if (!h) return fail(MIPGEN_E_INVALID, "null handle");
    if (h->cur_window < 0) return fail(MIPGEN_E_STATE, "nothing scored yet");
    const Window& W = h->windows[(size_t)h->cur_window];
    if (first < W.cand0 || count < 0 || first + count > W.cand0 + W.n_cand)
        return fail(MIPGEN_E_INVALID, "range [%lld,+%lld) outside the scored window [%lld,+%lld)", (long long)first, (long long)count, (long long)W.cand0, (long long)W.n_cand);
    HIP_TRY(hipSetDevice(h->device));
    if (count == 0) { HIP_TRY(hipStreamSynchronize(h->stream)); return MIPGEN_OK; }
    const int64_t off = first - W.cand0;
    if (scores) HIP_TRY(hipMemcpyAsync(scores, h->scores.p + off, (size_t)count * sizeof(double), hipMemcpyDeviceToHost, h->stream));
    if (records) HIP_TRY(hipMemcpyAsync(records, h->records.p + off, (size_t)count * sizeof(uint64_t), hipMemcpyDeviceToHost, h->stream));
    HIP_TRY(hipStreamSynchronize(h->stream));
    return mipgen_pb_check(h);
}

int mipgen_accel_score_regions(mipgen_accel* h, const mipgen_region* regions, int32_t n, int32_t method, mipgen_grid* grids_out,
                               double* scores, uint64_t* records, int64_t capacity)
{
    int rc = mipgen_accel_upload_regions(h, regions, n, grids_out);
    if (rc) return rc;
    if (h->n_cand > capacity) return fail(MIPGEN_E_INVALID, "result capacity %lld < %lld candidates", (long long)capacity, (long long)h->n_cand);
    for (int w = 0; w < (int)h->windows.size(); w++) {
        const Window& W = h->windows[(size_t)w];
        rc = mipgen_accel_score_window(h, w, method);
        if (rc) return rc;
        rc = mipgen_accel_download_results(h, scores ? scores + W.cand0 : nullptr, records ? records + W.cand0 : nullptr, W.cand0, W.n_cand);
        if (rc) return rc;
    }
    return MIPGEN_OK;
}

int mipgen_accel_score_candidates(mipgen_accel* h, const mipgen_candidate* cands, int32_t n, int32_t method, double* scores,
                                  uint64_t* records, double* features, mipgen_candidate_ints* ints)
{
    if (!h || n < 0 || (n > 0 && !cands)) return fail(MIPGEN_E_INVALID, "bad arguments");
    if (method != MIPGEN_SCORE_LOGISTIC && method != MIPGEN_SCORE_SVR) return fail(MIPGEN_E_INVALID, "method must be logistic or svr");
    if (h->regions.p == nullptr) return fail(MIPGEN_E_STATE, "no resident region batch");
    if (method == MIPGEN_SCORE_SVR && h->model.p == nullptr) return fail(MIPGEN_E_MODEL, "SVR scoring requested but no model is loaded");
    if (n == 0) return MIPGEN_OK;
    for (int i = 0; i < n; i++) if (cands[i].region < 0 || cands[i].region >= h->n_regions) return fail(MIPGEN_E_INVALID, "candidate %d: region %d not resident", i, cands[i].region);
    HIP_TRY(hipSetDevice(h->device));
    if (h->cand_in.reserve((size_t)n) || h->cand_scores.reserve((size_t)n) || h->cand_records.reserve((size_t)n) ||
        (features && h->cand_feats.reserve((size_t)n * MIPGEN_N_FEATURES)) || (ints && h->cand_ints.reserve((size_t)n)))
        return MIPGEN_E_NOMEM;
    HIP_TRY(hipMemcpyAsync(h->cand_in.p, cands, (size_t)n * sizeof(mipgen_candidate), hipMemcpyHostToDevice, h->stream));
    hipEvent_t le[3] = {nullptr, nullptr, nullptr};
    if (int rc = score_list(h, n, method, scores != nullptr, features != nullptr, ints != nullptr, le)) return rc;
    if (scores) HIP_TRY(hipMemcpyAsync(scores, h->cand_scores.p, (size_t)n * sizeof(double), hipMemcpyDeviceToHost, h->stream));
    if (records) HIP_TRY(hipMemcpyAsync(records, h->cand_records.p, (size_t)n * sizeof(uint64_t), hipMemcpyDeviceToHost, h->stream));
    if (features) HIP_TRY(hipMemcpyAsync(features, h->cand_feats.p, (size_t)n * MIPGEN_N_FEATURES * sizeof(double), hipMemcpyDeviceToHost, h->stream));
    if (ints) HIP_TRY(hipMemcpyAsync(ints, h->cand_ints.p, (size_t)n * sizeof(mipgen_candidate_ints), hipMemcpyDeviceToHost, h->stream));
    HIP_TRY(hipStreamSynchronize(h->stream));
    if (int rc_pb = mipgen_pb_check(h)) return rc_pb;
    if (le[0]) {
        float a = 0.f, b = 0.f;
        if (hipEventElapsedTime(&a, le[0], le[1]) == hipSuccess && hipEventElapsedTime(&b, le[1], le[2]) == hipSuccess) { h->list_feat_ms = a; h->list_svr_ms = b; }
        for (hipEvent_t e : le) (void)hipEventDestroy(e);
    }
    return MIPGEN_OK;
}

int mipgen_accel_score_probes(mipgen_accel* h, const mipgen_probe* probes, int32_t n, const double* lrc, int32_t n_lrc, int32_t method, double* scores,
                              double* features, mipgen_candidate_ints* ints)
{
    if (!h || n < 0 || (n > 0 && !probes) || n_lrc < 0 || (n_lrc > 0 && !lrc)) return fail(MIPGEN_E_INVALID, "bad arguments");
    if (method != MIPGEN_SCORE_LOGISTIC && method != MIPGEN_SCORE_SVR) return fail(MIPGEN_E_INVALID, "method must be logistic or svr");
    if (method == MIPGEN_SCORE_SVR && h->model.p == nullptr) return fail(MIPGEN_E_MODEL, "SVR scoring requested but no model is loaded");
    if (n == 0) return MIPGEN_OK;
    int64_t total = 0;
    for (int i = 0; i < n; i++) {
        const mipgen_probe& q = probes[i];
        if (!q.ext_seq || !q.lig_seq || !q.ins_seq) return fail(MIPGEN_E_INVALID, "probe %d: %s sequence is NULL", i, !q.ext_seq ? "extension arm" : !q.lig_seq ? "ligation arm" : "insert");
        const size_t e = strlen(q.ext_seq), l = strlen(q.lig_seq), s = strlen(q.ins_seq);
        if (e < MIPGEN_MIN_OLIGO || l < MIPGEN_MIN_OLIGO) return fail(MIPGEN_E_INVALID, "probe %d: empty %s arm", i, e < MIPGEN_MIN_OLIGO ? "extension" : "ligation");
        if (e > MIPGEN_MAX_OLIGO || l > MIPGEN_MAX_OLIGO) return fail(MIPGEN_E_INVALID, "probe %d: arm of %zu bases (at most %d)", i, std::max(e, l), MIPGEN_MAX_OLIGO);
        if (s > (size_t)INT32_MAX) return fail(MIPGEN_E_INVALID, "probe %d: insert too long", i);
        if (q.lrc_index < -1 || q.lrc_index >= n_lrc) return fail(MIPGEN_E_INVALID, "probe %d: long-range row %d out of range (%d rows)", i, q.lrc_index, n_lrc);
        total += (int64_t)(e + l + s);
    }
    std::vector<ProbeRec> recs((size_t)n);
    std::vector<uint8_t> packed((size_t)std::max<int64_t>(total, 1));
    int64_t at = 0;
    for (int i = 0; i < n; i++) {
        const mipgen_probe& q = probes[i];
        ProbeRec& r = recs[(size_t)i];
        r.ext_len = (int32_t)strlen(q.ext_seq); r.lig_len = (int32_t)strlen(q.lig_seq); r.ins_len = (int32_t)strlen(q.ins_seq);
        r.ext_off = at; memcpy(&packed[(size_t)at], q.ext_seq, (size_t)r.ext_len); at += r.ext_len;
        r.lig_off = at; memcpy(&packed[(size_t)at], q.lig_seq, (size_t)r.lig_len); at += r.lig_len;
        r.ins_off = at; memcpy(&packed[(size_t)at], q.ins_seq, (size_t)r.ins_len); at += r.ins_len;
        r.ext_copy = q.ext_copy; r.lig_copy = q.lig_copy; r.lrc_index = q.lrc_index;
        r.guard = q.mip_seq && strchr(q.mip_seq, '-') != nullptr;
        r.pad = 0;
    }
    std::vector<int32_t> order;
    if (list_runs_feature_kernel(n, method, scores != nullptr, ints != nullptr)) {
        const int NB = 64;
        auto bucket = [](int32_t len) { return NB - 1 - std::min(len >> 6, NB - 1); };
        int64_t first[NB + 1] = {0};
        for (int i = 0; i < n; i++) first[bucket(recs[(size_t)i].ins_len) + 1]++;
        for (int b = 0; b < NB; b++) first[b + 1] += first[b];
        order.resize((size_t)n);
        for (int i = 0; i < n; i++) order[(size_t)first[bucket(recs[(size_t)i].ins_len)]++] = i;
    }
    HIP_TRY(hipSetDevice(h->device));
    HIP_TRY(hipStreamSynchronize(h->stream));
    struct KeepOver { unsigned int* p; unsigned int v; ~KeepOver() { if (p) *p = v; } } keep_over{h->pb_over, h->pb_over ? *h->pb_over : 0u};
    if (h->pb_over) *h->pb_over = 0u;
    if (h->probe_recs.reserve((size_t)n) || h->probe_bytes.reserve(packed.size()) || (n_lrc > 0 && h->probe_lrc.reserve((size_t)n_lrc * MIPGEN_N_LRC)) ||
        (!order.empty() && h->probe_order.reserve((size_t)n)) || h->cand_scores.reserve((size_t)n) || h->cand_records.reserve((size_t)n) ||
        (features && h->cand_feats.reserve((size_t)n * MIPGEN_N_FEATURES)) || (ints && h->cand_ints.reserve((size_t)n)))
        return MIPGEN_E_NOMEM;
    struct IdleOnExit { hipStream_t s; ~IdleOnExit() { (void)hipStreamSynchronize(s); } } idle_on_exit{h->stream};
    HIP_TRY(hipMemcpyAsync(h->probe_recs.p, recs.data(), (size_t)n * sizeof(ProbeRec), hipMemcpyHostToDevice, h->stream));
    HIP_TRY(hipMemcpyAsync(h->probe_bytes.p, packed.data(), packed.size(), hipMemcpyHostToDevice, h->stream));
    if (n_lrc > 0) HIP_TRY(hipMemcpyAsync(h->probe_lrc.p, lrc, (size_t)n_lrc * MIPGEN_N_LRC * sizeof(double), hipMemcpyHostToDevice, h->stream));
    if (!order.empty()) HIP_TRY(hipMemcpyAsync(h->probe_order.p, order.data(), (size_t)n * sizeof(int32_t), hipMemcpyHostToDevice, h->stream));
    const ProbeSrc ps = {h->probe_recs.p, h->probe_bytes.p, h->probe_lrc.p, nullptr, order.empty() ? nullptr : h->probe_order.p};
    hipEvent_t le[3] = {nullptr, nullptr, nullptr};
    int rc = score_list(h, n, method, scores != nullptr, features != nullptr, ints != nullptr, le, &ps);
    if (rc == MIPGEN_OK) {
        hipError_t e_ = hipSuccess;
        if (scores) e_ = hipMemcpyAsync(scores, h->cand_scores.p, (size_t)n * sizeof(double), hipMemcpyDeviceToHost, h->stream);
        if (e_ == hipSuccess && features) e_ = hipMemcpyAsync(features, h->cand_feats.p, (size_t)n * MIPGEN_N_FEATURES * sizeof(double), hipMemcpyDeviceToHost, h->stream);
        if (e_ == hipSuccess && ints) e_ = hipMemcpyAsync(ints, h->cand_ints.p, (size_t)n * sizeof(mipgen_candidate_ints), hipMemcpyDeviceToHost, h->stream);
        if (e_ == hipSuccess) e_ = hipStreamSynchronize(h->stream);
        if (e_ != hipSuccess) rc = fail(MIPGEN_E_HIP, "mipgen_accel_score_probes: %s", hipGetErrorString(e_));
    } else (void)hipStreamSynchronize(h->stream);
    if (rc == MIPGEN_OK) rc = mipgen_pb_check(h);
    if (le[0]) {
        float a = 0.f, b = 0.f;
        if (rc == MIPGEN_OK && hipEventElapsedTime(&a, le[0], le[1]) == hipSuccess && hipEventElapsedTime(&b, le[1], le[2]) == hipSuccess) { h->list_feat_ms = a; h->list_svr_ms = b; }
        for (hipEvent_t e : le) if (e) (void)hipEventDestroy(e);
    }
    return rc;
}

static void lrc_mers(LrcMers& M)
{
    static const char* mers[MIPGEN_N_LRC] = MIPGEN_FEATURE_MERS;
    auto code = [](char c) { return c == 'A' ? 0 : c == 'C' ? 1 : c == 'G' ? 2 : 3; };
    for (int i = 0; i < MIPGEN_N_LRC; i++) {
        const int k = (int)strlen(mers[i]);
        int cd = 0, rc = 0;
        for (int j = 0; j < k; j++) cd = cd * 4 + code(mers[i][j]);
        for (int j = k - 1; j >= 0; j--) rc = rc * 4 + (3 - code(mers[i][j]));
        M.k[i] = (int8_t)k; M.code[i] = (int8_t)cd; M.rc[i] = (int8_t)(rc == cd ? -1 : rc);
    }
}

int mipgen_accel_long_range_content_batch(mipgen_accel* h, int32_t n, const char* const* extended_seqs, const int32_t* lens,
                                          const int32_t* chrom_seq_starts, const int32_t* chrom_seq_stops, double* out)
{
    if (!h || n < 0 || (n > 0 && (!extended_seqs || !lens || !chrom_seq_starts || !chrom_seq_stops || !out))) return fail(MIPGEN_E_INVALID, "bad arguments");
    if (n == 0) return MIPGEN_OK;
    HIP_TRY(hipSetDevice(h->device));
    LrcMers M;
    lrc_mers(M);
    std::vector<int64_t> offs((size_t)n);
    std::vector<int32_t> denoms((size_t)n);
    int64_t total = 0;
    for (int i = 0; i < n; i++) {
        if (lens[i] < 0 || (lens[i] > 0 && !extended_seqs[i])) return fail(MIPGEN_E_INVALID, "long-range sequence %d is missing", i);
        offs[(size_t)i] = total; total += lens[i];
        denoms[(size_t)i] = chrom_seq_stops[i] - chrom_seq_starts[i] + 2001;
    }
    std::vector<char> packed((size_t)std::max<int64_t>(total, 1));
    for (int i = 0; i < n; i++) if (lens[i]) memcpy(&packed[(size_t)offs[(size_t)i]], extended_seqs[i], (size_t)lens[i]);
    if (h->lrc_seq.reserve(packed.size()) || h->lrc_out.reserve((size_t)n * MIPGEN_N_LRC) || h->lrc_offs.reserve((size_t)n) ||
        h->lrc_lens.reserve((size_t)n) || h->lrc_denoms.reserve((size_t)n))
        return MIPGEN_E_NOMEM;
    HIP_TRY(hipMemcpyAsync(h->lrc_seq.p, packed.data(), packed.size(), hipMemcpyHostToDevice, h->stream));
    HIP_TRY(hipMemcpyAsync(h->lrc_offs.p, offs.data(), (size_t)n * sizeof(int64_t), hipMemcpyHostToDevice, h->stream));
    HIP_TRY(hipMemcpyAsync(h->lrc_lens.p, lens, (size_t)n * sizeof(int32_t), hipMemcpyHostToDevice, h->stream));
    HIP_TRY(hipMemcpyAsync(h->lrc_denoms.p, denoms.data(), (size_t)n * sizeof(int32_t), hipMemcpyHostToDevice, h->stream));
    HIP_TRY(mipgen_launch_long_range(h->stream, n, h->lrc_seq.p, h->lrc_offs.p, h->lrc_lens.p, h->lrc_denoms.p, &M, h->lrc_out.p));
    HIP_TRY(hipMemcpyAsync(out, h->lrc_out.p, (size_t)n * MIPGEN_N_LRC * sizeof(double), hipMemcpyDeviceToHost, h->stream));
    HIP_TRY(hipStreamSynchronize(h->stream));
    return MIPGEN_OK;
}

int mipgen_accel_long_range_content(mipgen_accel* h, const char* extended_seq, int32_t len, int32_t chrom_seq_start,
                                    int32_t chrom_seq_stop, double* out44)
{
    if (!h || !extended_seq || len < 0 || !out44) return fail(MIPGEN_E_INVALID, "bad arguments");
    return mipgen_accel_long_range_content_batch(h, 1, &extended_seq, &len, &chrom_seq_start, &chrom_seq_stop, out44);
}

int mipgen_accel_replay_condense(mipgen_accel* h)
{
    if (!h) return fail(MIPGEN_E_INVALID, "null handle");
    if (h->cur_window < 0) return fail(MIPGEN_E_STATE, "replay requested before scoring");
    HIP_TRY(hipSetDevice(h->device));
    return replay_window_impl(h, true);
}

int mipgen_accel_download_replay(mipgen_accel* h, int64_t* emitted_per_region, mipgen_survivor* survivors, int64_t survivor_capacity,
                                 uint8_t* emitted_mask, int64_t mask_capacity)
{
    if (!h) return fail(MIPGEN_E_INVALID, "null handle");
    if (!win_has(h, h->cur_window, WIN_SURVIVORS)) return fail(MIPGEN_E_STATE, "mipgen_accel_replay_condense has not run on these scores");
    const Window& W = h->windows[(size_t)h->cur_window];
    if (int rc = mipgen_accel_synchronize(h)) return rc;
    if (emitted_per_region && W.r1 > W.r0)
        HIP_TRY(hipMemcpy(emitted_per_region, h->emitted_per_region.p + W.r0, (size_t)(W.r1 - W.r0) * sizeof(int64_t), hipMemcpyDeviceToHost));
    if (survivors) {
        if (survivor_capacity < 2 * W.n_pos) return fail(MIPGEN_E_INVALID, "survivor capacity too small");
        if (W.n_pos) HIP_TRY(hipMemcpy(survivors, h->survivors.p + 2 * W.pos0, (size_t)(2 * W.n_pos) * sizeof(mipgen_survivor), hipMemcpyDeviceToHost));
    }
    if (emitted_mask) {
        if (!win_has(h, h->cur_window, WIN_MASK)) return fail(MIPGEN_E_STATE, "the emitted mask is only kept by mipgen_accel_replay_condense, not by mipgen_accel_score_condense_all");
        if (mask_capacity < W.n_cand) return fail(MIPGEN_E_INVALID, "mask capacity too small");
        if (W.n_cand) HIP_TRY(hipMemcpy(emitted_mask, h->emitted.p, (size_t)W.n_cand, hipMemcpyDeviceToHost));
    }
    return MIPGEN_OK;
}

int mipgen_accel_collapse(mipgen_accel* h)
{
    if (!h) return fail(MIPGEN_E_INVALID, "null handle");
    if (!win_has(h, h->cur_window, WIN_SURVIVORS)) return fail(MIPGEN_E_STATE, "collapse requested before replay + condense");
    HIP_TRY(hipSetDevice(h->device));
    return collapse_window_impl(h);
}

int mipgen_accel_region_bases(const mipgen_accel* h, int32_t region, int64_t* first_entry, int32_t* n_bases)
{
    if (!h || region < 0 || region >= h->n_regions) return fail(MIPGEN_E_INVALID, "region %d out of range", region);
    if (first_entry) *first_entry = h->h_region_base0[(size_t)region];
    if (n_bases) *n_bases = (int32_t)((h->h_region_base0[(size_t)region + 1] - h->h_region_base0[(size_t)region]) / 2);
    return MIPGEN_OK;
}

int mipgen_accel_download_collapsed(mipgen_accel* h, int32_t window, int32_t* best_scan_index, int64_t capacity)
{
    if (!h || !best_scan_index) return fail(MIPGEN_E_INVALID, "bad arguments");
    for (size_t w = 0; w < h->win_state.size(); w++)
        if ((window < 0 || (size_t)window == w) && !win_has(h, (int)w, WIN_COLLAPSED))
            return fail(MIPGEN_E_STATE, "mipgen_accel_collapse / mipgen_accel_score_condense_all has not run on the current scores of window %zu", w);
    if (h->win_state.empty()) return fail(MIPGEN_E_STATE, "no resident region batch");
    int64_t first = 0, count = h->h_region_base0.empty() ? 0 : h->h_region_base0.back();
    if (window >= 0) {
        if (window >= (int32_t)h->windows.size()) return fail(MIPGEN_E_INVALID, "window %d out of range", window);
        first = h->windows[(size_t)window].base0; count = h->windows[(size_t)window].n_base_entries;
    }
    if (capacity < count) return fail(MIPGEN_E_INVALID, "collapsed capacity %lld < %lld entries", (long long)capacity, (long long)count);
    HIP_TRY(hipSetDevice(h->device));
    HIP_TRY(hipStreamSynchronize(h->stream));
    if (count) HIP_TRY(hipMemcpy(best_scan_index, h->collapsed.p + first, (size_t)count * sizeof(int32_t), hipMemcpyDeviceToHost));
    return MIPGEN_OK;
}

int mipgen_accel_format_all_mips(mipgen_accel* h, const mipgen_record_names* names, const char* middle, int64_t first_index, int64_t* n_records, int64_t* n_bytes)
{
    if (!h || !middle || !n_records || !n_bytes) return fail(MIPGEN_E_INVALID, "bad arguments");
    if (!win_has(h, h->cur_window, WIN_SURVIVORS | WIN_MASK)) return fail(MIPGEN_E_STATE, "format_all_mips needs mipgen_accel_replay_condense on the scored window first");
// ... 151 lines not shown
```

### mipgen_amd/csrc/accel_tiles.hip

```cpp
#include "accel_internal.h"

extern "C" {

int mipgen_pick_sv_split(int n_tiles, int n_sv, int n_cu)
{
    const int groups = (n_sv + SVR_GROUP - 1) / SVR_GROUP;
    const double PH0 = 6.0;
    int best = 1;
    double best_cost = 0;
    for (int s = 1; s <= 8; s++) {
        if (s > 1 && groups / s < 32) break;
        const int64_t units = (int64_t)n_tiles * s, rounds = (units + n_cu - 1) / n_cu;
        const double cost = (double)rounds * (PH0 + (double)((groups + s - 1) / s));
        if (s == 1 || cost < best_cost * 0.98) { best = s; best_cost = cost; }
    }
    return best;
}

int mipgen_ensure_events(mipgen_accel* h)
{
    const size_t want = 4 * h->windows.size();
    while (h->ev.size() < want) {
        hipEvent_t e = nullptr;
        HIP_TRY(hipEventCreate(&e));
        h->ev.push_back(e);
    }
    return 0;
}

static int build_record_tiles(mipgen_accel* h)
{
    if (h->record_tiles_ready) return MIPGEN_OK;
    const DevParams& D = h->hp;
    const int Lmax = std::max(D.e_max, D.l_max);
    std::vector<LogTile> lt;
    int span_max = 0;
    for (Window& w : h->windows) {
        w.log_tile0 = (int)lt.size();
        for (int i = w.r0; i < w.r1; i++) {
            const DevRegion& d = h->hregions[i];
            if (d.n_pos <= 0 || d.n_sizes <= 0) continue;
            const int Cmax = D.max_capture - d.k0 * D.inc;
            const int NPL = 8;
            for (int p0 = 0; p0 < d.n_pos; p0 += NPL) {
                LogTile t = {i, p0, std::min(NPL, d.n_pos - p0), 0};
                lt.push_back(t);
                span_max = std::max(span_max, t.np + Cmax + Lmax);
            }
        }
        w.n_log_tiles = (int)lt.size() - w.log_tile0;
    }
    if (h->log_tiles.reserve(std::max<size_t>(lt.size(), 1))) return MIPGEN_E_NOMEM;
    if (!lt.empty()) HIP_TRY(hipMemcpy(h->log_tiles.p, lt.data(), lt.size() * sizeof(LogTile), hipMemcpyHostToDevice));
    h->log_span_max = span_max;
    h->record_tiles_ready = true;
    return MIPGEN_OK;
}

static int build_logistic_tiles(mipgen_accel* h)
{
    if (h->logistic_tiles_ready) return MIPGEN_OK;
    const DevParams& D = h->hp;
    const int Lmax = std::max(D.e_max, D.l_max);
    std::vector<SvrTile> ldt;
    size_t ld_lds = 0;
    bool ld_ok = true;
    const int64_t ld_np_cap = h->total_pos * 2 < 8192 ? 8 : (h->total_pos * 2 < 65536 ? 16 : 64);
    for (Window& w : h->windows) {
        w.ld_tile0 = (int)ldt.size();
        for (int i = w.r0; i < w.r1 && ld_ok; i++) {
            const DevRegion& d = h->hregions[i];
            if (d.n_pos <= 0 || d.n_sizes <= 0) continue;
            const int Cmax = D.max_capture - d.k0 * D.inc;
            const int nkc = (d.n_sizes + 8) / 9;
            int kc_max = 0;
            for (int c = 0; c < nkc; c++) kc_max = std::max(kc_max, (int)((int64_t)d.n_sizes * (c + 1) / nkc) - (int)((int64_t)d.n_sizes * c / nkc));
            const int ssr = (kc_max - 1) * D.inc + D.max_sum - D.min_sum + 1, ssmax = Cmax - D.min_sum;
            const int ssmin_all = Cmax - (d.n_sizes - 1) * D.inc - D.max_sum;
            const int subs = h->ld_subruns > 0 ? h->ld_subruns : (h->total_pos >= 1000000 ? 3 : (h->total_pos >= 25000 ? 2 : 1));
            int np = (int)std::min<int64_t>({ld_np_cap, (int64_t)d.n_pos, 64});
            size_t b = 0;
            for (; np >= 1; np--) {
                const int np_all = std::min(subs * np, d.n_pos);
                b = std::max(mipgen_logistic_dense_lds_bytes(np_all, np, ssr, ssmax, Lmax, D.e_max - D.e_min + 1, D.l_max - D.l_min + 1),
                             mipgen_logistic_dense_lds_bytes(np_all, np, ssr, ssmax, Lmax, D.l_max - D.l_min + 1, D.e_max - D.e_min + 1));
                if (b <= 80 * 1024) break;
            }
            if (np < 1 || ssmin_all < 1) { ld_ok = false; break; }
            ld_lds = std::max(ld_lds, b);
            for (int p0 = 0; p0 < d.n_pos; p0 += subs * np) { SvrTile t = {i, np, p0, std::min(subs * np, d.n_pos - p0), 0, d.n_sizes, 0, 0}; ldt.push_back(t); }
        }
        w.n_ld_tiles = (int)ldt.size() - w.ld_tile0;
    }
    if (!ld_ok) {
        for (Window& w : h->windows) { w.ld_tile0 = 0; w.n_ld_tiles = 0; }
        h->ld_lds = 0;
        h->logistic_tiles_ready = true;
        return build_record_tiles(h);
    }
    if (h->ld_tiles.reserve(std::max<size_t>(ldt.size(), 1))) return MIPGEN_E_NOMEM;
    if (!ldt.empty()) HIP_TRY(hipMemcpy(h->ld_tiles.p, ldt.data(), ldt.size() * sizeof(SvrTile), hipMemcpyHostToDevice));
    h->ld_lds = ld_lds;
    h->logistic_tiles_ready = true;
    return MIPGEN_OK;
}

static int build_svr_tiles(mipgen_accel* h)
{
    if (h->svr_tiles_ready) return MIPGEN_OK;
    if (int rc = build_record_tiles(h)) return rc;
    const DevParams& D = h->hp;
    const int Lmax = std::max(D.e_max, D.l_max);
    const int n_arm = std::max(h->geom.n_e, h->geom.n_l) | 1;
    std::vector<SvrTile> st, st_lvl;
    std::vector<double> st_cost;
    size_t svr_lds = 0;
    int max_levels = 1;
    struct Run { int ki0, kc, np; };
    struct Shape { std::vector<Run> runs; size_t lds = 0; };
    std::unordered_map<uint64_t, Shape> shapes;
    auto shape_of = [&](const DevRegion& d, bool few) -> const Shape& {
        const int lanes = 64 * (few ? h->geom_few.wpc : h->geom.wpc);
        const uint64_t key = ((uint64_t)(uint32_t)d.n_pos << 32) | ((uint64_t)(uint16_t)d.k0 << 16) | (uint64_t)(uint16_t)d.n_sizes | (few ? (uint64_t)1 << 15 : 0);
        auto it = shapes.find(key);
        if (it != shapes.end()) return it->second;
        Shape best;
        double best_cost = 0;
        const int Cmax = D.max_capture - d.k0 * D.inc;
        for (int kc_cap = std::min(9, d.n_sizes); kc_cap >= 1; kc_cap--) {
            const int nkc = (d.n_sizes + kc_cap - 1) / kc_cap;
            if (kc_cap < std::min(9, d.n_sizes) && nkc == (d.n_sizes + kc_cap) / (kc_cap + 1)) continue;
            std::vector<Run> runs;
            double ent = 0, slots = 0;
            size_t lds_r = 0;
            bool ok = true;
            for (int c = 0; c < nkc && ok; c++) {
                const int ki0 = (int)((int64_t)d.n_sizes * c / nkc), ki1 = (int)((int64_t)d.n_sizes * (c + 1) / nkc);
                const int kc = ki1 - ki0;
                const int Cmax_t = Cmax - ki0 * D.inc, Cmin_t = Cmax_t - (kc - 1) * D.inc;
                const int ssmax = Cmax_t - D.min_sum, ssmin = Cmin_t - D.max_sum, ssr = ssmax - ssmin + 1;
                int np = std::max(1, std::min(lanes / kc, d.n_pos));
                size_t lds_t = 0;
                for (; np >= 1; np--) {
                    lds_t = mipgen_svr_lds_bytes_tile(np, ssr, ssmax, Lmax, n_arm, h->geom.group, h->geom.n_e, h->geom.n_l, h->geom.nchunk * h->geom.wpc * 64, 0);
                    if (lds_t <= 160 * 1024) break;
                }
                if (np < 1) { ok = false; break; }
                { const int np_cf = np - ((np + D.inc) % 32); if (np_cf >= 1 && np_cf * 10 >= np * 9) { np = np_cf; lds_t = mipgen_svr_lds_bytes_tile(np, ssr, ssmax, Lmax, n_arm, h->geom.group, h->geom.n_e, h->geom.n_l, h->geom.nchunk * h->geom.wpc * 64, 0); } }
                { const int nt = (d.n_pos + np - 1) / np, np_even = (d.n_pos + nt - 1) / nt;
                  if (np_even < np) { np = np_even; lds_t = mipgen_svr_lds_bytes_tile(np, ssr, ssmax, Lmax, n_arm, h->geom.group, h->geom.n_e, h->geom.n_l, h->geom.nchunk * h->geom.wpc * 64, 0); } }
                runs.push_back({ki0, kc, np});
                lds_r = std::max(lds_r, lds_t);
                const double tiles = std::ceil((double)d.n_pos / np);
                ent += tiles * (np * (h->geom.n_e + h->geom.n_l) / 2.0 + (np + ssr - 1) * (h->geom.n_e + h->geom.n_l) / 2.0 + (double)np * ssr);
                slots += tiles * lanes;
            }
            if (!ok) continue;
            const double cost = 47.0 * ent + 2.7 * slots * D.n_pairs / 1.0;
            if (best.runs.empty() || cost < best_cost) { best.runs = runs; best_cost = cost; best.lds = lds_r; }
        }
        return shapes.emplace(key, std::move(best)).first->second;
    };
    for (Window& w : h->windows) {
        w.svr_tile0 = (int)st.size();
        int n_few_regions = 0;
        for (int i = w.r0; i < w.r1; i++) if (h->hregions[i].n_pos > 0 && h->hregions[i].n_sizes == 1) n_few_regions++;
        const bool win_few = h->have_few && n_few_regions >= h->n_cu;
        std::vector<uint8_t> st_few;
        for (int i = w.r0; i < w.r1; i++) {
            const DevRegion& d = h->hregions[i];
            if (d.n_pos <= 0 || d.n_sizes <= 0) continue;
            const bool few = win_few && d.n_sizes == 1;
            const Shape& shape = shape_of(d, false);
            if (shape.runs.empty()) { svr_lds = (size_t)1 << 30; continue; }
            svr_lds = std::max(svr_lds, shape.lds);
            const int Cmax = D.max_capture - d.k0 * D.inc;
            for (size_t lvl = 0; lvl < shape.runs.size(); lvl++) {
                const Run& r = shape.runs[lvl];
                max_levels = std::max(max_levels, (int)lvl + 1);
                for (int p0 = 0; p0 < d.n_pos; p0 += r.np) {
                    const int npt = std::min(r.np, d.n_pos - p0);
                    const int Cmax_t = Cmax - r.ki0 * D.inc, ssmax = Cmax_t - D.min_sum, ssr = (r.kc - 1) * D.inc + D.max_sum - D.min_sum + 1;
                    const double ent = (npt + (npt + ssr - 1)) * (h->geom.n_e + h->geom.n_l) / 2.0 + (double)npt * ssr;
                    const double cost = 19.0 * ent + 100.0 * (npt + ssmax + 2 * Lmax) + 75000.0;
                    const int nthr = h->geom.nchunk * h->geom.wpc * 64;
                    const int it_pitch = svr_it_pitch(npt, r.kc, D.inc, h->geom.wpc * 64, ssmax - ssr + 1, ssmax, Lmax, n_arm, h->geom.group, h->geom.n_e, h->geom.n_l, nthr);
                    if (it_pitch) svr_lds = std::max(svr_lds, mipgen_svr_lds_bytes_tile(npt, ssr, ssmax, Lmax, n_arm, h->geom.group, h->geom.n_e, h->geom.n_l, nthr, it_pitch));
                    const int fits = mipgen_svr_scores_fit_lds(npt, r.kc, D.n_pairs, ssr, ssmax, Lmax, n_arm, h->geom.group, h->geom.n_e, h->geom.n_l, nthr, it_pitch);
                    for (int s2 = 0; s2 < 2; s2++) { SvrTile t = {i, s2, p0, npt, r.ki0, r.kc, (int)lvl, fits | (it_pitch << 8)}; st.push_back(t); st_cost.push_back(cost); st_few.push_back(few ? 1 : 0); }
                }
            }
        }
        {
            const size_t t0 = (size_t)w.svr_tile0, n = st.size() - t0;
            std::vector<size_t> order(n);
            for (size_t k = 0; k < n; k++) order[k] = k;
            std::stable_sort(order.begin(), order.end(), [&](size_t a, size_t b) { return st_few[a] != st_few[b] ? st_few[a] < st_few[b] : st_cost[t0 + a] > st_cost[t0 + b]; });
            std::vector<SvrTile> sorted(n);
            for (size_t k = 0; k < n; k++) sorted[k] = st[t0 + order[k]];
            std::copy(sorted.begin(), sorted.end(), st.begin() + (ptrdiff_t)t0);
            w.n_svr_few = 0;
            for (size_t k = 0; k < n; k++) w.n_svr_few += st_few[k];
        }
        w.n_svr_tiles = (int)st.size() - w.svr_tile0;
        {
            const size_t t0 = (size_t)w.svr_tile0, n = (size_t)w.n_svr_tiles;
            int wl = 0;
            for (size_t k = 0; k < n; k++) wl = std::max(wl, st[t0 + k].level + 1);
            w.lvl_tile0.assign(1, (int)st_lvl.size());
            for (int lvl = 0; lvl < wl; lvl++) {
                for (size_t k = 0; k < n; k++) if (st[t0 + k].level == lvl) st_lvl.push_back(st[t0 + k]);
                w.lvl_tile0.push_back((int)st_lvl.size());
            }
            w.lvl0_few = w.n_svr_few;
        }
    }
    h->svr_batch_error.clear();
    if (svr_lds > 160 * 1024) {
        h->svr_batch_error = "an SVR tile needs more than 160 KiB of LDS: capture range / arm lists too wide";
        st.clear();
        for (Window& w : h->windows) { w.svr_tile0 = 0; w.n_svr_tiles = 0; }
        svr_lds = 0;
    }
    if (h->svr_tiles.reserve(std::max<size_t>(st.size(), 1))) return MIPGEN_E_NOMEM;
    if (!st.empty()) HIP_TRY(hipMemcpy(h->svr_tiles.p, st.data(), st.size() * sizeof(SvrTile), hipMemcpyHostToDevice));
    h->svr_levels = st.empty() ? 1 : max_levels;
    if (h->svr_levels > 1) {
        std::vector<uint32_t> rb((size_t)h->n_regions * (size_t)max_levels, 0u);
        for (const SvrTile& t : st) rb[(size_t)t.region * (size_t)max_levels + (size_t)t.level] = (uint32_t)t.ki0 | ((uint32_t)t.kc << 16);
        if (h->svr_tiles_lvl.reserve(st_lvl.size()) || h->run_bounds.reserve(rb.size())) return MIPGEN_E_NOMEM;
        HIP_TRY(hipMemcpy(h->svr_tiles_lvl.p, st_lvl.data(), st_lvl.size() * sizeof(SvrTile), hipMemcpyHostToDevice));
        HIP_TRY(hipMemcpy(h->run_bounds.p, rb.data(), rb.size() * sizeof(uint32_t), hipMemcpyHostToDevice));
    }
    h->svr_lds = svr_lds;
    h->svr_tiles_ready = true;
    return MIPGEN_OK;
}

int mipgen_ensure_tiles(mipgen_accel* h, int32_t method)
{
    if (method == MIPGEN_SCORE_SVR) return h->svr_geometry_error.empty() ? build_svr_tiles(h) : build_record_tiles(h);
    return build_logistic_tiles(h);
}


}
```

### mipgen_amd/csrc/kernels.h

```cpp
#pragma once
#include <hip/hip_runtime.h>
#include "common.h"
#include "reads_common.h"
#include "call_model.h"
#include "insertion_call_model.h"

struct HostConsts;
struct LrcMers { int8_t k[MIPGEN_N_LRC], code[MIPGEN_N_LRC], rc[MIPGEN_N_LRC]; };
struct FmtRegion {
    int32_t chr_off, chr_len;
    int32_t label_off, label_len;
    int32_t feature_start, feature_stop;
    int64_t rb0;
};
struct FmtConst {
    char middle[96];
    int32_t middle_len;
    int32_t n_regions;
    int64_t first_index;
};

struct KmerParams {
    int32_t n_k;
    int32_t k[MIPGEN_MAX_OLIGO];
    int32_t kmax;
    int32_t filter_bits;
    uint64_t cap_mask;
};

struct ConsensusView {
    const uint64_t* __restrict__ keys;
    const int32_t* __restrict__ family;
    const int64_t* __restrict__ ext_off;
    const int64_t* __restrict__ lig_off;
    const uint8_t* __restrict__ ext_seq;
    const uint8_t* __restrict__ ext_qual;
    const uint8_t* __restrict__ lig_seq;
    const uint8_t* __restrict__ lig_qual;
    int64_t n_groups;
};

struct PileRow {
    const uint2* __restrict__ units;
    int64_t n_small, n_big;
    const uint32_t* __restrict__ start;
    const int32_t* __restrict__ mol_len;
    const int64_t* __restrict__ pos_off;
    int32_t n;
    int64_t n_pos;
    uint32_t cell0;
    int min_family, min_quality;
};

struct CallCounters { unsigned long long tested, too_deep, candidates, calls; };
#define MIPGEN_CALL_MAX_POSITIONS (((int64_t)1 << 29) - 1)

struct InsPoolCounters { unsigned long long entries, alleles; };

struct LocusCounters { unsigned long long covered, bases, discordant, deletions, insertions, ins_discordant; };

struct LocusInsCounters { unsigned long long loci, span, insertions, ins_discordant, ambiguous, alleles, folded, dropped; };

extern "C" {
size_t mipgen_logistic_lds_bytes(int span);
hipError_t mipgen_launch_records_logistic(hipStream_t, int score, int n_tiles, int span_max, const DevParams*, const DevRegion*, const LogTile*, const uint8_t*, const int32_t*,
                                          const uint8_t*, const HostConsts*, double*, uint64_t*, int64_t* sat_idx, unsigned int* sat_count, unsigned int sat_cap);
size_t mipgen_logistic_dense_lds_bytes(int np_all, int np, int ssr, int ssmax, int Lmax, int n_up, int n_dn);
hipError_t mipgen_launch_logistic_dense(hipStream_t, int n_tiles, size_t lds_bytes, const DevParams*, const DevRegion*, const SvrTile*, const uint8_t*, const int32_t*,
                                        const uint8_t*, const HostConsts*, double*, uint64_t*, int64_t* sat_idx, unsigned int* sat_count, unsigned int sat_cap);
size_t mipgen_svr_lds_bytes_tile(int np, int ss_range, int ssmax, int Lmax, int n_arm, int group, int n_e, int n_l, int n_threads, int it_pitch);
int mipgen_svr_scores_fit_lds(int np, int kc, int n_pairs, int ss_range, int ssmax, int Lmax, int n_arm, int group, int n_e, int n_l, int n_threads, int it_pitch);
hipError_t mipgen_launch_svr_dense(hipStream_t, int n_tiles, int n_tiles_few, size_t lds_bytes, const DevParams*, const SvrGeom*, const SvrGeom* geom_few, const DevRegion*,
                                   const SvrTile*, const uint8_t*, const int32_t*, const double* log10_tab, const double* model, int n_sv, double gamma_l2e, double rho,
                                   double s_guard, const uint64_t* records, double* scores, int64_t n_cand, int n_split, double* partials);
hipError_t mipgen_launch_svr_run_state(hipStream_t s, int64_t n_pos, const DevParams* P, const DevRegion* regions, const int32_t* pos_region, const int32_t* pos_local,
                                       const uint32_t* run_bounds, int max_levels, int level, double margin, const double* scores, const uint64_t* records, double* pbs,
                                       uint8_t* state);
hipError_t mipgen_launch_svr_tile_keep(hipStream_t s, int n_tiles, const SvrTile* tiles, const int64_t* region_pos0, int64_t win_pos0, const uint8_t* state, int64_t* keep);
hipError_t mipgen_launch_svr_tile_compact(hipStream_t s, int n_tiles, const SvrTile* tiles, const int64_t* keep, const int64_t* offs, SvrTile* out, const DevParams* P,
                                          const DevRegion* regions, double* scores, unsigned long long* skipped);
hipError_t mipgen_launch_svr_gemm(hipStream_t, int n, const double* feats, const uint64_t* records, const double* model_t, const double* sv_norm, const double* sv_coef,
                                  const double* center, int n_sv_pad, double gamma, double rho, double* scores);
hipError_t mipgen_launch_features_batch(hipStream_t, int n, const ListSrc&, const HostConsts*, uint64_t* records, double* features);
hipError_t mipgen_launch_candidates(hipStream_t, int n, const ListSrc&, const HostConsts*, const double* model, int n_sv, double gamma, double rho, int method, double* scores,
                                    uint64_t* records, double* features, mipgen_candidate_ints*, int literal, const unsigned int* n_dev);
hipError_t mipgen_launch_dense_candidates(hipStream_t, const DevParams* P, const DevRegion* regions, int r0, int r1, int64_t c0, int n, mipgen_candidate* out);
hipError_t mipgen_launch_dense_list_fix(hipStream_t, int n, const uint64_t* records, double rho, double s_guard, double* scores);
hipError_t mipgen_launch_print_boundary_scan(hipStream_t, const DevParams*, const DevRegion*, const RescoreSrc*, double tol_rel, double tol_abs, mipgen_candidate* out,
                                             int64_t* out_idx, unsigned int* count, unsigned int cap, int n_cu);
hipError_t mipgen_launch_index_candidates(hipStream_t, const DevParams*, const DevRegion*, int r0, int r1, const int64_t* idx, const unsigned int* count, unsigned int cap,
                                          mipgen_candidate* out);
hipError_t mipgen_launch_scatter_scores(hipStream_t, const double* src, const int64_t* idx, int64_t cap, const unsigned int* n_dev, double* dst, mipgen_survivor* dst_surv,
                                        unsigned int* over);
hipError_t mipgen_launch_surv_keep(hipStream_t, const mipgen_survivor* surv, int64_t n, int64_t* keep, double* svr);
hipError_t mipgen_launch_surv_candidates(hipStream_t, const DevParams*, const DevRegion*, int r0, int r1, const mipgen_survivor* surv, int64_t n, int64_t cand0,
                                         const int64_t* offs, mipgen_candidate* out, int64_t* out_idx);
hipError_t mipgen_launch_long_range(hipStream_t, int n, const char* seqs, const int64_t* offs, const int32_t* lens, const int32_t* denoms, const LrcMers*, double* out);
hipError_t mipgen_launch_replay_condense(hipStream_t, int total_pos, const DevParams*, int n_pairs, int n_sizes_max, const DevRegion*, const int32_t* pos_region,
                                         const int32_t* pos_local, const double* scores, const uint64_t* records, const int32_t* copy, int64_t cand_base, uint8_t* emitted,
                                         mipgen_survivor* survivors, unsigned long long* emitted_per_region);
hipError_t mipgen_launch_collapse(hipStream_t, int n_tiles, const CollapseTile* tiles, const DevParams*, const DevRegion*, const int64_t* region_pos0,
                                  const int64_t* region_base0, const mipgen_survivor* survivors, const int32_t* copy, int64_t cand_base, int32_t* collapsed, int max_scan_all);
hipError_t mipgen_launch_fill_pos_map(hipStream_t, const int64_t* region_pos0, int n_regions, int64_t total, int32_t* pos_region, int32_t* pos_local);
hipError_t mipgen_launch_fmt_count(hipStream_t, int64_t n_rb, int r0, const FmtConst*, const FmtRegion*, const DevParams*, const DevRegion*, const uint8_t* emitted,
                                   int64_t* cnt);
hipError_t mipgen_launch_fmt_records(hipStream_t, int write, int64_t n_rb, int r0, const FmtConst*, const FmtRegion*, const char* pool, const DevParams*, const DevRegion*,
                                     const char* letters, const int32_t* copy, const double* scores, const uint64_t* records, const uint8_t* emitted, const int64_t* rank0,
                                     const int64_t* off, int64_t* len_out, char* text);
hipError_t mipgen_scan_i64(hipStream_t, void* temp, size_t* temp_bytes, const int64_t* in, int64_t* out, int64_t n);
hipError_t mipgen_launch_kmer_insert(hipStream_t, const char* seq, int64_t len, const KmerParams*, uint64_t* keys, uint32_t* filter);
hipError_t mipgen_launch_kmer_fold(hipStream_t, const uint32_t* filter, int filter_bits, uint32_t* folded);
hipError_t mipgen_launch_kmer_count(hipStream_t, const char* genome, int64_t len, const KmerParams*, const uint64_t* keys, const uint32_t* filter, const uint32_t* folded,
                                    unsigned int* counts, int n_cu);
hipError_t mipgen_launch_kmer_lookup(hipStream_t, const char* seq, int64_t len, const KmerParams*, const uint64_t* keys, const unsigned int* counts, int32_t* out);
hipError_t mipgen_launch_kmer_place(hipStream_t, const int32_t* src, int64_t len, const KmerParams*, const int64_t* roff, int n_regions, int32_t* dst, void* big,
                                    unsigned int* n_big, unsigned int big_cap);
hipError_t mipgen_launch_window_spans(hipStream_t st, const char* q, const int64_t* roff, int n_regions, uint16_t* dist_bad, uint16_t* dist_end, uint16_t* dist_start);
hipError_t mipgen_launch_seed_index(hipStream_t st, const char* q, int64_t total, int k, const uint64_t* keys, uint64_t cap_mask, unsigned int* rmult, unsigned int* rstart,
                                    unsigned int* rfill, uint32_t* rlist, unsigned int* alloc, int phase);
hipError_t mipgen_launch_window_verify(hipStream_t st, const char* G, int64_t glen, const char* q, int64_t total, const int32_t* sizes, int n_sizes, int k,
                                       const uint64_t* keys, uint64_t cap_mask, const unsigned int* counts, const uint32_t* filter, int filter_bits, const unsigned int* rmult,
                                       const unsigned int* rstart, const uint32_t* rlist, const uint16_t* dist_start, unsigned int* ctr);
hipError_t mipgen_launch_window_flags(hipStream_t st, const char* q, int64_t total, const int32_t* sizes, int n_sizes, int k, const uint64_t* keys, uint64_t cap_mask,
                                      const unsigned int* counts, const uint16_t* dist_bad, const uint16_t* dist_end, const unsigned int* ctr, uint8_t* unmap,
                                      const int64_t* roff, int n_regions, const int32_t* bounds, uint8_t* any);
hipError_t mipgen_launch_read_assign(hipStream_t, const ReadsParams*, const ReadProbe* probes, const SeedTable* ext_seeds, const SeedTable* lig_seeds, int64_t pair0,
                                     int64_t n_pairs, const uint8_t* ext_bytes, const int64_t* ext_off, int64_t ext_base, const uint8_t* lig_bytes, const int64_t* lig_off,
                                     int64_t lig_base, int32_t* assign, unsigned long long* reads, uint64_t* keys, int64_t key_cap, ReadsCounters* ctr,
                                     const int32_t* row);
hipError_t mipgen_launch_sample_assign(hipStream_t, const SampleTable*, int64_t n_pairs, const uint8_t* idx_bytes, const int64_t* idx_off, int64_t idx_base, int32_t* row,
                                       int32_t* sample_index, unsigned long long* row_pairs, SampleCounters* sctr);
hipError_t mipgen_launch_reads_histogram(hipStream_t, const uint64_t* keys, int64_t n, unsigned long long* unique);
hipError_t mipgen_reads_sort_unique(hipStream_t, void* temp, size_t* temp_bytes, uint64_t* keys, uint64_t* alt, int64_t n, int end_bit, unsigned long long* n_out);
hipError_t mipgen_launch_member_keys(hipStream_t, const ReadsParams*, int64_t n_pairs, uint32_t pair0, const int32_t* assign, const int32_t* row, const uint8_t* ext_bytes,
                                     const int64_t* ext_off, int64_t ext_base, const uint8_t* lig_bytes, const int64_t* lig_off, int64_t lig_base, int64_t qdelta,
                                     uint64_t sentinel, uint64_t* keys, uint32_t* ids, ConsensusPair* recs, ConsensusCounters* cctr);
hipError_t mipgen_consensus_sort(hipStream_t, void* temp, size_t* temp_bytes, const uint64_t* keys_in, uint64_t* keys_out, const uint32_t* ids_in, uint32_t* ids_out, int64_t n,
                                 int end_bit);
hipError_t mipgen_consensus_runs(hipStream_t, void* temp, size_t* temp_bytes, const uint64_t* keys, int64_t n, uint64_t* group_keys, int32_t* family,
                                 unsigned long long* n_groups);
hipError_t mipgen_consensus_scan_u32(hipStream_t, void* temp, size_t* temp_bytes, const int32_t* family, uint32_t* group_start, int64_t n);
hipError_t mipgen_consensus_scan_i64(hipStream_t, void* temp, size_t* temp_bytes, const int64_t* len, int64_t* off, int64_t n);
hipError_t mipgen_launch_consensus_partition(hipStream_t, const int32_t* family, int64_t n_groups, uint32_t* order, ConsensusCounters* cctr);
hipError_t mipgen_launch_consensus_len(hipStream_t, int te, int tl, int64_t n_groups, const uint32_t* order, int64_t n_big, const uint32_t* group_start, const int32_t* family,
                                       const uint32_t* ids, const ConsensusPair* recs, int64_t* ext_len, int64_t* lig_len);
hipError_t mipgen_launch_consensus_vote(hipStream_t, int te, int tl, int64_t n_groups, const uint32_t* order, int64_t n_small, int64_t n_big, const uint32_t* group_start,
                                        const int32_t* family, const uint32_t* ids, const ConsensusPair* recs, const int64_t* ext_off, const int64_t* lig_off, uint8_t* ext_seq,
                                        uint8_t* ext_qual, uint8_t* lig_seq, uint8_t* lig_qual);
struct TagMergeCounters;
hipError_t mipgen_launch_tag_parent(hipStream_t, const uint64_t* keys, const int32_t* family, int64_t n_groups, int tag_bases, int32_t* parent);
hipError_t mipgen_launch_tag_root(hipStream_t, const int32_t* parent, const int32_t* family, int64_t n_groups, int32_t* root, TagMergeCounters* ctr);
hipError_t mipgen_launch_tag_rewrite(hipStream_t, const uint64_t* keys_sorted, const uint32_t* ids_sorted, int64_t n_pairs, int64_t n_members, const uint64_t* group_keys,
                                     int64_t n_groups, const int32_t* root, uint64_t* keys, uint32_t* ids);
hipError_t mipgen_launch_pileup_prepare(hipStream_t, const ConsensusView& C, const PileRow& R, int64_t n_units, uint32_t* start, uint2* units, PileupCounters* ctr);
hipError_t mipgen_launch_pileup(hipStream_t, const ConsensusView& C, const PileRow& R, int64_t n_units, int32_t* counts, PileupCounters* ctr);
size_t mipgen_gap_align_lds_bytes(int max_len, int W);
hipError_t mipgen_launch_gap_list(hipStream_t, const ConsensusView& C, const PileRow& R, const uint8_t* mol_seq, uint32_t g_first, int64_t n_row_groups, int max_indel,
                                  int planes, uint8_t* need, uint32_t* list, int64_t* proj_off, GappedCounters* ctr);
hipError_t mipgen_launch_gapped(hipStream_t, const ConsensusView& C, const PileRow& R, int64_t n_units, const uint8_t* mol_seq, uint32_t g_first, int max_indel, int max_len,
                                int planes, const uint32_t* list, int64_t n_sides, const int64_t* proj_off, uint8_t* proj, int32_t* counts, GappedCounters* ctr);
hipError_t mipgen_launch_insertions(hipStream_t, const ConsensusView& C, const PileRow& R, int64_t n_units, uint32_t g_first, const int64_t* proj_off, const uint8_t* proj,
                                    int32_t* anchors, uint64_t* keys, int64_t cap, InsCounters* ctr);
hipError_t mipgen_launch_insertion_records(hipStream_t, const uint64_t* run_keys, const int32_t* run_counts, const unsigned long long* n_runs, int64_t cap,
                                           mipgen_insertion_record* records);
hipError_t mipgen_launch_deletions(hipStream_t, const ConsensusView& C, const PileRow& R, int64_t n_units, uint32_t g_first, const int64_t* proj_off, const uint8_t* proj,
                                   int32_t* sites, uint64_t* keys, int64_t cap, DelCounters* ctr);
hipError_t mipgen_launch_deletion_records(hipStream_t, const uint64_t* run_keys, const int32_t* run_counts, const unsigned long long* n_runs, int64_t cap, const int32_t* sites,
                                          int64_t n_pos, mipgen_deletion_record* records);
hipError_t mipgen_launch_call_pool(hipStream_t, const int32_t* counts, int columns, int64_t n_pos, int32_t bg_max_ppm, int32_t* pool);
hipError_t mipgen_launch_call_flag(hipStream_t, const int32_t* counts, int columns, const int32_t* pool, const uint8_t* ref, int64_t n_pos, int own_row_is_sample,
                                   const CallModel& P, mipgen_call_record* cand, CallCounters* ctr);
hipError_t mipgen_launch_call_tail(hipStream_t, mipgen_call_record* cand, int64_t n_cand, int64_t n_pos, const CallModel& P, uint64_t* keys, uint32_t* ids, CallCounters* ctr);
hipError_t mipgen_launch_call_gather(hipStream_t, const mipgen_call_record* cand, const uint32_t* ids, int64_t n_cand, const CallCounters* ctr, mipgen_call_record* records);
hipError_t mipgen_launch_ins_pool_append(hipStream_t, const int32_t* anchors, int64_t n_pos, const mipgen_insertion_record* records, int64_t n_records, int32_t bg_max_ppm,
                                         int32_t* S, uint64_t* keys, InsPoolSums* sums, uint32_t* ids, int64_t cap, InsPoolCounters* ctr);
hipError_t mipgen_launch_ins_pool_reduce(hipStream_t, const int32_t* run_counts, const uint32_t* run_start, const unsigned long long* n_runs, int64_t n_entries,
                                         const uint32_t* ids_sorted, const InsPoolSums* entry_sums, InsPoolSums* pool_sums);
hipError_t mipgen_launch_ins_call_flag(hipStream_t, const mipgen_insertion_record* records, int64_t n_records, const int32_t* span, int span_stride, int64_t n_pos,
                                       const uint64_t* pool_keys, const InsPoolSums* pool_sums, int64_t n_pool, const int32_t* pool_span, int own_row_is_sample,
                                       const CallModel& P, mipgen_call_record* cand, CallCounters* ctr);
hipError_t mipgen_launch_ins_call_records(hipStream_t, const mipgen_call_record* calls, int64_t n_calls, const mipgen_insertion_record* records, int64_t n_records,
                                          mipgen_insertion_call_record* out);
hipError_t mipgen_launch_locus_keys(hipStream_t, const int64_t* plan, int64_t n_pos, int64_t n_loci, uint64_t* keys, uint32_t* ids);
hipError_t mipgen_launch_locus_index(hipStream_t, const uint64_t* keys_sorted, const uint32_t* ids_sorted, const int64_t* plan, int64_t n_pos, int64_t n_loci, uint32_t* src,
                                     uint32_t* first);
hipError_t mipgen_launch_locus_merge(hipStream_t, const int32_t* counts, int columns, const uint32_t* src, const uint32_t* first, int64_t n_pos, int64_t n_loci,
                                     int32_t* merged, LocusCounters* ctr);
hipError_t mipgen_launch_locus_anchor_map(hipStream_t, const uint32_t* src, const uint32_t* first, int64_t n_pos, int64_t n_loci, uint32_t* own, uint32_t* prev);
hipError_t mipgen_launch_locus_ins_fold(hipStream_t, const mipgen_insertion_record* records, int64_t n_records, const uint32_t* own, const uint32_t* prev, int64_t n_pos,
                                        uint64_t* keys, uint32_t* ids, int64_t cap, LocusInsCounters* ctr);
hipError_t mipgen_launch_locus_ins_reduce(hipStream_t, const uint64_t* run_keys, const int32_t* run_counts, const uint32_t* run_start, const unsigned long long* n_runs,
                                          int64_t n_pairs, const uint32_t* ids_sorted, const mipgen_insertion_record* records, int64_t n_records, mipgen_insertion_record* out);
hipError_t mipgen_launch_locus_anchor_merge(hipStream_t, const int32_t* anchors, const uint32_t* src, const uint32_t* first, int64_t n_pos, int64_t n_loci,
                                            int32_t* locus_anchors, LocusInsCounters* ctr);
}
```

### mipgen_amd/csrc/kernels_logistic.hip

```cpp
#include <hip/hip_runtime.h>
#include "kernels.h"
#include "device_utils.h"

#include "logistic_device.h"
#include "mip_record.h"
#include "prefix_words.h"

#define LOG_RINV 512
template <bool SCORE>
__global__ __launch_bounds__(LOG_THREADS) void k_records_logistic(
    const DevParams* __restrict__ P, const DevRegion* __restrict__ regions, const LogTile* __restrict__ tiles,
    int n_tiles, const uint8_t* __restrict__ bases, const int32_t* __restrict__ copy,
    const uint8_t* __restrict__ unmap, const HostConsts* __restrict__ HC, double* __restrict__ scores,
    uint64_t* __restrict__ records, int64_t* __restrict__ sat_idx, unsigned int* __restrict__ sat_count, unsigned int sat_cap)
{
    extern __shared__ __align__(16) unsigned char smem[];
    const LogTile tile = tiles[xcd_remap(blockIdx.x, n_tiles)];
    const DevRegion& R = regions[tile.region];
    const int tid = threadIdx.x;

    const int A = P->n_pairs;
    const int nK = R.n_sizes;
    const int Cmax = P->max_capture - R.k0 * P->inc;
    const int Lmax = max(P->e_max, P->l_max);
    const int p_first = R.first_pos + tile.p0;
    const int lo = p_first - Lmax;
    const int span = tile.np + Cmax + Lmax;

    PrefixWords W = prefix_words_carve(smem, span);
    double* rinv = (double*)(W.scratch + PW_SCRATCH);
    W.sb = (uint8_t*)(rinv + LOG_RINV);

    for (int i = tid; i < LOG_RINV; i += LOG_THREADS) rinv[i] = i > 0 ? 1.0 / (double)i : 0.0;
    prefix_words_build<LOG_THREADS>(W, R, bases, lo, span);

    const uint32_t row = (uint32_t)(2 * A);
    const uint32_t per_pos = row * (uint32_t)nK;
    const uint32_t n_cand = per_pos * (uint32_t)tile.np;
    const uint32_t M_row = 0xFFFFFFFFu / row + 1, M_k = 0xFFFFFFFFu / (uint32_t)nK + 1;
    const int64_t out_base = R.out_off + (int64_t)tile.p0 * per_pos;
    const double thr = P->masked_arm_threshold;

    for (uint32_t idx = tid; idx < n_cand; idx += LOG_THREADS) {
        uint32_t rc = fastdiv(idx, M_row);
        uint32_t in_row = idx - rc * row;
        uint32_t pl = nK == 1 ? rc : fastdiv(rc, M_k);
        uint32_t ki = rc - pl * (uint32_t)nK;
        const bool minus = in_row >= (uint32_t)A;
        const int a = (int)(minus ? in_row - (uint32_t)A : in_row);
        const int e = P->arm_ext[a], l = P->arm_lig[a];
        const int C = Cmax - (int)ki * P->inc;
        const int ss = C - e - l;
        const int p = p_first + (int)pl;

        uint64_t rec = 0;
        double score = 0.0;
        if (constructed(R, p, C, e, l)) {
            const ArmStarts st = arm_starts(p, ss, e, l, minus);
            const int ext_start = st.ext, lig_start = st.lig;
            const int be = ext_start - lo, bl = lig_start - lo, bi = p - lo;
            const ArmCounts ce = arm_window(W, be, e), cl = arm_window(W, bl, l);
            const bool guard = (ce.bad + cl.bad) != 0;
            const int ext_copy = oligo_copy(P, R, copy, ext_start, e), lig_copy = oligo_copy(P, R, copy, lig_start, l);
            const bool mapping = unmapped(P, R, unmap, R.k0 + (int)ki, minus, ext_start, lig_start);
            const uint32_t masked_n = ce.masked + cl.masked;
            int snp_count;
            const uint32_t flags = record_flags(mapping, (int)masked_n, l + e, thr, (int)(ce.snp_any + cl.snp_any), (int)(ce.snp_bad + cl.snp_bad),
                                                (int)(ce.snp_ok + cl.snp_ok), guard, snp_count);
            const uint32_t jc = lig_junction(W.sb, bl, l, minus);
            rec = pack_record(ext_copy, lig_copy, (int)masked_n, snp_count, flags, jc);

            if (SCORE) {
                if (guard) score = -1000.0;
                else {
                    const InsertCounts t = insert_window(W, bi, ss, minus);
                    const int run = t.run;
                    Vars x;
                    const double dl = (double)e, ll = (double)l, dn = (double)ss;
                    const double e_g = minus ? (double)ce.nC : (double)ce.nG, l_g = minus ? (double)cl.nC : (double)cl.nG,
                                 t_g = minus ? (double)t.nC : (double)t.nG;
                    const double e_a = minus ? (double)ce.nT : (double)ce.nA, l_a = minus ? (double)cl.nT : (double)cl.nA,
                                 t_a = minus ? (double)t.nT : (double)t.nA;
                    const double e_gc = (double)(ce.nC + ce.nG), l_gc = (double)(cl.nC + cl.nG), t_gc = (double)(t.nC + t.nG);
                    const double re = rinv[e], rl = rinv[l], rn = ss < LOG_RINV ? rinv[ss] : 1.0 / dn;
                    x.v[MLV_BPS] = run < LOG_RINV ? dn * rinv[run] : dn / (double)run;
                    x.v[MLV_TLEN] = ss > 250 ? 250.0 : dn;
                    x.v[MLV_ELEN] = dl; x.v[MLV_LLEN] = ll;
                    x.v[MLV_EGC] = e_gc * re; x.v[MLV_LGC] = l_gc * rl; x.v[MLV_TGC] = t_gc * rn;
                    x.v[MLV_EG] = e_g * re; x.v[MLV_LG] = l_g * rl; x.v[MLV_TG] = t_g * rn;
                    x.v[MLV_EA] = e_a * re; x.v[MLV_LA] = l_a * rl; x.v[MLV_TA] = t_a * rn;
                    x.v[MLV_JS] = jc < 16 ? c_junction_scores[jc] : 0.0;
                    x.v[MLV_LEC] = log_copy_dev(HC, ext_copy);
                    x.v[MLV_LLC] = log_copy_dev(HC, lig_copy);
                    const double ex = logistic_exponent(x);
                    score = logistic_from_exponent_fast(HC, ex);
                    const double tb = ex * (HC->ln_base * 1.4426950408889634074);
                    if (SCORE && sat_count && tb >= 52.99 && tb <= 54.01) { const unsigned int at = atomicAdd(sat_count, 1u); if (at < sat_cap) sat_idx[at] = out_base + idx; }
                }
            }
        }
        records[out_base + idx] = rec;
        if (SCORE) scores[out_base + idx] = score;
    }
}

extern "C" size_t mipgen_logistic_lds_bytes(int span)
{
    return (prefix_words_u64(span) + LOG_RINV) * sizeof(uint64_t) + (size_t)span + 16;
}

extern "C" hipError_t mipgen_launch_records_logistic(
    hipStream_t stream, int score, int n_tiles, int span_max, const DevParams* P, const DevRegion* regions,
    const LogTile* tiles, const uint8_t* bases, const int32_t* copy, const uint8_t* unmap, const HostConsts* HC, double* scores,
    uint64_t* records, int64_t* sat_idx, unsigned int* sat_count, unsigned int sat_cap)
{
    if (n_tiles <= 0) return hipSuccess;
    size_t lds = mipgen_logistic_lds_bytes(span_max);
    if (score)
        hipLaunchKernelGGL(k_records_logistic<true>, dim3(n_tiles), dim3(LOG_THREADS), lds, stream, P, regions, tiles, n_tiles,
                           bases, copy, unmap, HC, scores, records, sat_idx, sat_count, sat_cap);
    else
        hipLaunchKernelGGL(k_records_logistic<false>, dim3(n_tiles), dim3(LOG_THREADS), lds, stream, P, regions, tiles, n_tiles,
                           bases, copy, unmap, HC, scores, records, (int64_t*)nullptr, (unsigned int*)nullptr, 0u);
    return hipGetLastError();
}
```

### mipgen_amd/csrc/kernels_replay.hip

```cpp
#include <hip/hip_runtime.h>
#include <limits.h>
#include <algorithm>
#include "kernels.h"
#include "device_utils.h"
#include "mip_record.h"

#define REPLAY_WAVES 4

namespace {

__device__ __forceinline__ int to_int_x86(double v)
{
    if (!(v == v) || v >= 2147483648.0 || v <= -2147483649.0) return INT_MIN;
    return (int)v;
}

__device__ __forceinline__ double readlane_d(double x, int l)
{
    return __hiloint2double(__builtin_amdgcn_readlane(__double2hiint(x), l), __builtin_amdgcn_readlane(__double2loint(x), l));
}
__device__ __forceinline__ uint64_t readlane_u64(uint64_t x, int l)
{
    return ((uint64_t)(uint32_t)__builtin_amdgcn_readlane((int)(x >> 32), l) << 32) | (uint32_t)__builtin_amdgcn_readlane((int)(uint32_t)x, l);
}
__device__ __forceinline__ int top_bit(uint64_t m) { return 63 - __builtin_clzll(m); }

__device__ __forceinline__ bool condense_take(bool held, double cur_masked, int cur_copy, double sc, int snp, double thr, int target_copy, double lower,
                                              double upper, double best_score, int best_snp, double chosen_masked, int chosen_copy,
                                              bool& update_chosen, bool& stops)
{
    const bool rA = !held;
    const bool rB = (cur_masked > thr) & (cur_masked < chosen_masked);
    const bool rC = (cur_copy > target_copy) & (cur_copy < chosen_copy);
    const bool rD = cur_copy <= target_copy;
    const bool above = sc > best_score;
    const bool rE = (sc < lower) & above;
    const bool hi_sc = sc > lower;
    const bool rF = snp < best_snp;
    const bool rG = (snp == best_snp) & above;
    const bool early = rA | rB | rC;
    const bool last_rule = !early & rD & !rE & hi_sc & !rF & rG;
    update_chosen = !last_rule;
    stops = last_rule & (sc > upper);
    return early | (rD & (rE | (hi_sc & (rF | rG))));
}

struct Fold {
    int64_t best_idx;
    double best_score;
    uint64_t best_rec;
    int best_snp;
    bool stop;
    int chosen_copy;
    double chosen_masked;
};

__device__ __forceinline__ void fold_strand_start(Fold& F) { F.best_idx = -1; F.best_score = 0.0; F.best_rec = 0; F.best_snp = 0; F.stop = false; }

__device__ __forceinline__ void condense_row(Fold& F, uint64_t em, uint64_t r, double sc, int e, int l, int ki, int s, int64_t row_idx0, int pi,
                                             const DevParams* P, const DevRegion& R, const int32_t* copy)
{
    const int target_copy = P->target_arm_copy;
    const double thr = P->masked_arm_threshold;
    int ext_copy = (int)MIPGEN_REC_EXT_COPY(r), lig_copy = (int)MIPGEN_REC_LIG_COPY(r);
    if (F.best_idx >= 0 && !(em & __ballot(sc > F.best_score || ext_copy > target_copy || lig_copy > target_copy || thr < 0.0 ||
                                           MIPGEN_REC_MASKED_N(r) != 0 || (int)MIPGEN_REC_SNP_COUNT(r) < F.best_snp))) return;
    const uint64_t sat_mask = R.copy_off >= 0 ? em & __ballot(ext_copy == 65535 || lig_copy == 65535) : 0;
    if (sat_mask && __builtin_amdgcn_inverse_ballot_w64(sat_mask)) {
        const int C = P->max_capture - (R.k0 + ki) * P->inc;
        const ArmStarts st = arm_starts(R.first_pos + pi, C - e - l, e, l, s != 0);
        ext_copy = true_arm_copy(P, R, copy, st.ext, e, (uint32_t)ext_copy);
        lig_copy = true_arm_copy(P, R, copy, st.lig, l, (uint32_t)lig_copy);
    }
    const bool ok = !((int64_t)ext_copy * lig_copy > P->max_arm_copy_product) && !(MIPGEN_REC_FLAGS(r) & MIPGEN_FLAG_MAPPING);
    const int cur_copy = ext_copy > lig_copy ? ext_copy : lig_copy;
    double cur_masked = 0.0;
    if (em & __ballot(MIPGEN_REC_MASKED_N(r) != 0)) cur_masked = (double)MIPGEN_REC_MASKED_N(r) / (double)(l + e);
    const int snp = (int)MIPGEN_REC_SNP_COUNT(r);
    uint64_t pending = em & __ballot(ok);
    while (pending) {
        bool update_chosen, stops;
        const bool take = condense_take(F.best_idx >= 0, cur_masked, cur_copy, sc, snp, thr, target_copy, P->lower, P->upper, F.best_score, F.best_snp,
                                        F.chosen_masked, F.chosen_copy, update_chosen, stops);
        const uint64_t tmask = __ballot(take) & pending;
        if (!tmask) break;
        const int f = top_bit(tmask);
        F.best_idx = row_idx0 + f;
        F.best_score = readlane_d(sc, f);
        F.best_rec = readlane_u64(r, f);
        F.best_snp = (int)MIPGEN_REC_SNP_COUNT(F.best_rec);
        if (__builtin_amdgcn_readlane((int)update_chosen, f)) {
            F.chosen_masked = readlane_d(cur_masked, f);
            F.chosen_copy = __builtin_amdgcn_readlane(cur_copy, f);
        }
        if (__builtin_amdgcn_readlane((int)stops, f)) { F.stop = true; break; }
        pending &= (1ull << f) - 1;
    }
}

__device__ __forceinline__ void write_survivor(mipgen_survivor* survivors, int gp, int s, const Fold& F, int64_t cand_base)
{
    if ((threadIdx.x & 63) == 0) {
        mipgen_survivor out;
        out.cand_index = F.best_idx < 0 ? -1 : F.best_idx + cand_base; out.score = F.best_score; out.record = F.best_rec;
        survivors[2 * (int64_t)gp + s] = out;
    }
}

struct Lists {
    uint64_t ends;
    uint64_t min_sum;
    uint64_t below, above;
};

__device__ __forceinline__ Lists row_lists(bool in, int e, int l, int gend, int key_min_sum)
{
    const int lane = threadIdx.x & 63;
    const uint64_t lane_bit = 1ull << lane, below_me = lane_bit - 1;
    Lists L;
    L.ends = __ballot(in && lane + 1 == gend);
    L.min_sum = __ballot(in && e + l == key_min_sum);
    const uint64_t ends_below = L.ends & below_me;
    const int lo = ends_below ? top_bit(ends_below) + 1 : 0;
    const uint64_t seg = in ? ((gend >= 64 ? ~0ull : (1ull << gend) - 1) & ~((1ull << lo) - 1)) : 0;
    L.below = seg & below_me; L.above = seg & ~below_me & ~lane_bit;
    return L;
}

struct RowPair { bool in; int e, l; Lists L; };
__device__ __forceinline__ RowPair row_pair(const DevParams* P, int lane)
{
    RowPair W;
    W.in = lane < P->n_pairs;
    W.e = W.in ? P->arm_ext[lane] : 1; W.l = W.in ? P->arm_lig[lane] : 1;
    W.L = row_lists(W.in, W.e, W.l, W.in ? P->group_end[lane] : 0, P->key_min_sum);
    return W;
}

struct ReplayPos {
    int ri, pi;
    const DevRegion& R;
    int A, nK;
    int64_t base;
    double upper;
    bool heuristic;
};
__device__ __forceinline__ ReplayPos replay_pos(int gp, const DevParams* P, const DevRegion* regions, const int32_t* pos_region, const int32_t* pos_local)
{
    const int ri = pos_region[gp], pi = pos_local[gp];
    const DevRegion& R = regions[ri];
    const int A = P->n_pairs, nK = R.n_sizes;
    const int64_t per_pos = (int64_t)nK * A * 2;
    return ReplayPos{ri, pi, R, A, nK, R.out_off + (int64_t)pi * per_pos, P->upper, P->score_method == MIPGEN_SCORE_LOGISTIC && P->logistic_heuristic};
}

__device__ __forceinline__ uint64_t replay_row(double& pbs, double plus, double minus, bool valid, bool heuristic, double upper, const Lists& L)
{
    const uint64_t vmask = __ballot(valid);
    bool mine = valid;
    if (heuristic && vmask && __ballot(valid && !(plus >= 0.0 && plus < 1.0 && minus >= 0.0 && minus < 1.0))) {
        const uint64_t below = vmask & L.below;
        const int src = below ? top_bit(below) : (int)(threadIdx.x & 63);
        const double pp = __shfl(plus, src, 64), pm = __shfl(minus, src, 64);
        const int ip = below ? to_int_x86(pp) : 0, im = below ? to_int_x86(pm) : 0;
        const bool cond = valid && plus < (double)ip && minus < (double)im;
        const uint64_t cmask = __ballot(cond);
        mine = valid && !(cmask & L.below);
    }
    uint64_t emit_all = __ballot(mine);
    if (emit_all) {
        const double pb = (minus > plus) ? minus : plus;
        const bool last_of_list = mine && !(emit_all & L.above);
        if (!__ballot(last_of_list && pb > upper)) {
            pbs = readlane_d(pb, top_bit(emit_all));
        } else {
            uint64_t ends = L.ends;
            int a0 = 0;
            while (ends) {
                const int a1 = __builtin_ctzll(ends) + 1;
                ends &= ends - 1;
                const uint64_t sg = (a1 >= 64 ? ~0ull : (1ull << a1) - 1) & ~((1ull << a0) - 1);
                if (pbs > upper && !((L.min_sum >> a0) & 1)) emit_all &= ~sg;
                else if (emit_all & sg) pbs = readlane_d(pb, top_bit(emit_all & sg));
                a0 = a1;
            }
        }
    }
    return emit_all;
}

}

__global__ __launch_bounds__(REPLAY_WAVES * 64) void k_replay_condense(
    int total_pos, int n_chunks, int lds_pitch, const DevParams* __restrict__ P, const DevRegion* __restrict__ regions,
    const int32_t* __restrict__ pos_region, const int32_t* __restrict__ pos_local, const double* __restrict__ scores,
    const uint64_t* __restrict__ records, const int32_t* __restrict__ copy, int64_t cand_base, uint8_t* __restrict__ emitted,
    mipgen_survivor* __restrict__ survivors, unsigned long long* __restrict__ emitted_per_region)
{
    extern __shared__ uint64_t s_masks[];
    const int lane = threadIdx.x & 63;
    const int wave = __builtin_amdgcn_readfirstlane(threadIdx.x >> 6);
    const int gp = blockIdx.x * REPLAY_WAVES + wave;
    if (gp >= total_pos) return;
    uint64_t* emask = s_masks + (size_t)wave * lds_pitch;
    const auto [ri, pi, R, A, nK, base, upper, heuristic] = replay_pos(gp, P, regions, pos_region, pos_local);
    const int min_sum = P->key_min_sum;
    const uint64_t lane_bit = 1ull << lane, below_me = lane_bit - 1;

    unsigned long long n_emitted = 0;
    double pbs = 0.0;
    for (int ki = 0; ki < nK; ki++) {
        if (lane < n_chunks) emask[ki * n_chunks + lane] = 0;
        if (pbs > upper) continue;
        int prev_plus = 0, prev_minus = 0;
        bool skip_ahead = false, list_skipped = false;
        int list_end = 0;
        for (int c = 0; c < n_chunks; c++) {
            const int a = c * 64 + lane;
            const bool in = a < A;
            const int64_t idx = base + ((int64_t)ki * 2) * A + a;
            const double plus = in ? scores[idx] : 0.0, minus = in ? scores[idx + A] : 0.0;
            const bool valid = in && (MIPGEN_REC_FLAGS(records[idx]) & MIPGEN_FLAG_VALID);
            const uint64_t vmask_all = __ballot(valid);
            uint64_t emit_chunk = 0;
            const int c_end = min(A, c * 64 + 64);
            int a0 = c * 64;
            while (a0 < c_end) {
                if (a0 == list_end) {
                    list_end = P->group_end[a0];
                    list_skipped = pbs > upper && (P->arm_ext[a0] + P->arm_lig[a0]) != min_sum;
                    prev_plus = 0; prev_minus = 0; skip_ahead = false;
                }
                const int a1 = min(list_end, c_end);
                if (!list_skipped && !skip_ahead) {
                    const int lo = a0 - c * 64, hi = a1 - c * 64;
                    const uint64_t seg = (hi >= 64 ? ~0ull : ((1ull << hi) - 1)) & ~((1ull << lo) - 1);
                    const uint64_t vmask = vmask_all & seg;
                    if (vmask) {
                        uint64_t emit = vmask;
                        if (heuristic) {
                            const uint64_t below = vmask & below_me;
                            const int src = below ? top_bit(below) : lane;
                            const double pp = __shfl(plus, src, 64), pm = __shfl(minus, src, 64);
                            const int ip = below ? to_int_x86(pp) : prev_plus, im = below ? to_int_x86(pm) : prev_minus;
                            const bool cond = (vmask & lane_bit) && plus < (double)ip && minus < (double)im;
                            const uint64_t cmask = __ballot(cond);
                            if (cmask) { emit = vmask & ((2ull << __builtin_ctzll(cmask)) - 1); skip_ahead = true; }
                        }
                        const int last = top_bit(emit);
                        const double lp = readlane_d(plus, last), lm = readlane_d(minus, last);
                        pbs = (lm > lp) ? lm : lp;
                        prev_minus = to_int_x86(lm); prev_plus = to_int_x86(lp);
                        emit_chunk |= emit;
                        n_emitted += 2ull * (unsigned)__builtin_popcountll(emit);
                    }
                }
                a0 = a1;
            }
            if (emit_chunk) {
                if (lane == 0) emask[ki * n_chunks + c] = emit_chunk;
                if (emitted && (emit_chunk & lane_bit)) { emitted[idx] = 1; emitted[idx + A] = 1; }
            }
        }
    }
    if (n_emitted && lane == 0) atomicAdd(&emitted_per_region[ri], n_emitted);
    __builtin_amdgcn_fence(__ATOMIC_ACQ_REL, "wavefront");
    __builtin_amdgcn_wave_barrier();

    Fold F;
    F.chosen_copy = 0; F.chosen_masked = 0.0;
    for (int s = 0; s < 2; s++) {
        fold_strand_start(F);
        for (int ki = nK - 1; ki >= 0 && !F.stop; ki--) {
            for (int c = n_chunks - 1; c >= 0 && !F.stop; c--) {
                const uint64_t em = emask[ki * n_chunks + c];
                if (!em) continue;
                const int a = c * 64 + lane;
                const bool mine = (em & lane_bit) != 0;
                const int64_t row_idx0 = base + ((int64_t)ki * 2 + s) * A + c * 64;
                const uint64_t r = mine ? records[row_idx0 + lane] : 0;
                const double sc = mine ? scores[row_idx0 + lane] : 0.0;
                const int e = mine ? P->arm_ext[a] : 1, l = mine ? P->arm_lig[a] : 1;
                condense_row(F, em, r, sc, e, l, ki, s, row_idx0, pi, P, R, copy);
            }
        }
        write_survivor(survivors, gp, s, F, cand_base);
    }
}

#define REPLAY_ROWS 8

template <bool WIDE>
__global__ __launch_bounds__(REPLAY_WAVES * 64) void k_replay_condense_narrow(
    int total_pos, int lds_pitch, const DevParams* __restrict__ P, const DevRegion* __restrict__ regions,
    const int32_t* __restrict__ pos_region, const int32_t* __restrict__ pos_local, const double* __restrict__ scores,
    const uint64_t* __restrict__ records, const int32_t* __restrict__ copy, int64_t cand_base, uint8_t* __restrict__ emitted,
    mipgen_survivor* __restrict__ survivors, unsigned long long* __restrict__ emitted_per_region)
{
    extern __shared__ uint64_t s_masks[];
    const int lane = threadIdx.x & 63;
    const int wave = __builtin_amdgcn_readfirstlane(threadIdx.x >> 6);
    const int gp = blockIdx.x * REPLAY_WAVES + wave;
    if (gp >= total_pos) return;
    uint64_t* emask = s_masks + (size_t)wave * lds_pitch;
    const auto [ri, pi, R, A, nK, base, upper, heuristic] = replay_pos(gp, P, regions, pos_region, pos_local);
    const uint64_t lane_bit = 1ull << lane;
    const auto [in, e, l, L] = row_pair(P, lane);
    const BoundsSpan span = bounds_span(R.seq_stop, R.first_pos + pi, e, l);
    const bool ok_lo = in && span.ok_lo;
    const int c_span = span.c_span;
    const int c_top = span_top(P->max_capture - R.k0 * P->inc, e, l), c_inc = P->inc;

    unsigned long long n_emitted = 0;
    double pbs = 0.0;
    for (int k0 = 0; k0 < nK; k0 += REPLAY_ROWS) {
        double bp[REPLAY_ROWS], bm[REPLAY_ROWS];
        if (pbs > upper) {
            if (lane < REPLAY_ROWS && k0 + lane < nK) emask[k0 + lane] = 0;
            continue;
        }
        if constexpr (WIDE) {
        {
            const double* srow = scores + base;
            const int la = min(lane, A - 1);
#pragma unroll
            for (int q = 0; q < REPLAY_ROWS; q++) {
                bp[q] = 0.0; bm[q] = 0.0;
                if (k0 + q < nK) {
                    const int off = ((k0 + q) * 2) * A + la;
                    bp[q] = srow[off]; bm[q] = srow[off + A];
                }
            }
            __builtin_amdgcn_sched_barrier(0);
#pragma unroll
            for (int q = 0; q < REPLAY_ROWS; q++) {
                bp[q] = in ? bp[q] : 0.0; bm[q] = in ? bm[q] : 0.0;
            }
        }
        } else {
#pragma unroll
        for (int q = 0; q < REPLAY_ROWS; q++) {
            const bool on = in && k0 + q < nK;
            const int64_t idx = base + ((int64_t)(k0 + q) * 2) * A + lane;
            bp[q] = on ? scores[idx] : 0.0; bm[q] = on ? scores[idx + A] : 0.0;
        }
        }
#pragma unroll
        for (int q = 0; q < REPLAY_ROWS; q++) {
            const int ki = k0 + q;
            if (ki >= nK) break;
            uint64_t emit_all = 0;
            if (!(pbs > upper)) {
                const bool valid = span_constructed(ok_lo, c_span, c_top - ki * c_inc);
                emit_all = replay_row(pbs, bp[q], bm[q], valid, heuristic, upper, L);
                n_emitted += 2ull * (unsigned)__builtin_popcountll(emit_all);
                if (emitted && (emit_all & lane_bit)) {
                    const int64_t idx = base + ((int64_t)ki * 2) * A + lane;
                    emitted[idx] = 1; emitted[idx + A] = 1;
                }
            }
            if (lane == 0) emask[ki] = emit_all;
        }
    }
    if (n_emitted && lane == 0) atomicAdd(&emitted_per_region[ri], n_emitted);
    __builtin_amdgcn_fence(__ATOMIC_ACQ_REL, "wavefront");
    __builtin_amdgcn_wave_barrier();

    Fold F;
    F.chosen_copy = 0; F.chosen_masked = 0.0;
    const int k_top = ((nK - 1) / REPLAY_ROWS) * REPLAY_ROWS;
    for (int s = 0; s < 2; s++) {
        fold_strand_start(F);
        for (int k0 = k_top; k0 >= 0 && !F.stop; k0 -= REPLAY_ROWS) {
            uint64_t em[REPLAY_ROWS], br[REPLAY_ROWS];
            double bs[REPLAY_ROWS];
            if constexpr (WIDE) {
            {
                const double* srow = scores + base;
                const uint64_t* rrow = records + base;
                const int la = min(lane, A - 1);
#pragma unroll
                for (int q = 0; q < REPLAY_ROWS; q++) em[q] = k0 + q < nK ? emask[k0 + q] : 0;
#pragma unroll
                for (int q = 0; q < REPLAY_ROWS; q++) {
                    br[q] = 0; bs[q] = 0.0;
                    if (em[q]) {
                        const int off = ((k0 + q) * 2 + s) * A + la;
                        br[q] = rrow[off]; bs[q] = srow[off];
                    }
                }
                __builtin_amdgcn_sched_barrier(0);
#pragma unroll
                for (int q = 0; q < REPLAY_ROWS; q++) {
                    const bool mine = (em[q] & lane_bit) != 0;
                    br[q] = mine ? br[q] : 0; bs[q] = mine ? bs[q] : 0.0;
                }
            }
            } else {
#pragma unroll
            for (int q = 0; q < REPLAY_ROWS; q++) {
                em[q] = k0 + q < nK ? emask[k0 + q] : 0;
                const bool mine = (em[q] & lane_bit) != 0;
                const int64_t idx = base + ((int64_t)(k0 + q) * 2 + s) * A + lane;
                br[q] = mine ? records[idx] : 0; bs[q] = mine ? scores[idx] : 0.0;
            }
            }
#pragma unroll
            for (int q = REPLAY_ROWS - 1; q >= 0; q--) {
                if (F.stop || !em[q]) continue;
                const int ki = k0 + q;
                condense_row(F, em[q], br[q], bs[q], e, l, ki, s, base + ((int64_t)ki * 2 + s) * A, pi, P, R, copy);
            }
        }
        write_survivor(survivors, gp, s, F, cand_base);
    }
}


template <int CR>
__global__ __launch_bounds__(REPLAY_WAVES * 64) void k_replay_condense_carry(
    int total_pos, const DevParams* __restrict__ P, const DevRegion* __restrict__ regions,
    const int32_t* __restrict__ pos_region, const int32_t* __restrict__ pos_local, const double* __restrict__ scores,
    const uint64_t* __restrict__ records, const int32_t* __restrict__ copy, int64_t cand_base, uint8_t* __restrict__ emitted,
    mipgen_survivor* __restrict__ survivors, unsigned long long* __restrict__ emitted_per_region)
{
    const int lane = threadIdx.x & 63;
    const int gp = blockIdx.x * REPLAY_WAVES + __builtin_amdgcn_readfirstlane(threadIdx.x >> 6);
    if (gp >= total_pos) return;
    const auto [ri, pi, R, A, nK, base, upper, heuristic] = replay_pos(gp, P, regions, pos_region, pos_local);
    const auto [in, e, l, L] = row_pair(P, lane);

    double bp[CR], bm[CR];
    uint64_t rp[CR], rm[CR], em[CR];
#pragma unroll
    for (int q = 0; q < CR; q++) {
        const bool on = in && q < nK;
        const int64_t idx = base + ((int64_t)q * 2) * A + lane;
        bp[q] = on ? scores[idx] : 0.0; bm[q] = on ? scores[idx + A] : 0.0;
        rp[q] = on ? records[idx] : 0; rm[q] = on ? records[idx + A] : 0;
        em[q] = 0;
    }
    unsigned long long n_emitted = 0;
    double pbs = 0.0;
#pragma unroll
    for (int q = 0; q < CR; q++) {
        if (q >= nK) break;
        uint64_t emit_all = 0;
        if (!(pbs > upper)) {
            const bool valid = in && (MIPGEN_REC_FLAGS(rp[q]) & MIPGEN_FLAG_VALID) != 0;
            emit_all = replay_row(pbs, bp[q], bm[q], valid, heuristic, upper, L);
            n_emitted += 2ull * (unsigned)__builtin_popcountll(emit_all);
            if (emitted && __builtin_amdgcn_inverse_ballot_w64(emit_all)) {
                const int64_t idx = base + ((int64_t)q * 2) * A + lane;
                emitted[idx] = 1; emitted[idx + A] = 1;
            }
        }
        em[q] = emit_all;
    }
    if (n_emitted && lane == 0) atomicAdd(&emitted_per_region[ri], n_emitted);

    Fold F;
    F.chosen_copy = 0; F.chosen_masked = 0.0;
    for (int s = 0; s < 2; s++) {
        fold_strand_start(F);
#pragma unroll
        for (int q = CR - 1; q >= 0; q--) {
            if (F.stop || !em[q]) continue;
            condense_row(F, em[q], s ? rm[q] : rp[q], s ? bm[q] : bp[q], e, l, q, s, base + ((int64_t)q * 2 + s) * A, pi, P, R, copy);
        }
        write_survivor(survivors, gp, s, F, cand_base);
    }
}

extern "C" hipError_t mipgen_launch_replay_condense(
    hipStream_t stream, int total_pos, const DevParams* P, int n_pairs, int n_sizes_max, const DevRegion* regions,
    const int32_t* pos_region, const int32_t* pos_local, const double* scores, const uint64_t* records, const int32_t* copy, int64_t cand_base,
    uint8_t* emitted, mipgen_survivor* survivors, unsigned long long* emitted_per_region)
{
    if (total_pos <= 0) return hipSuccess;
    const int n_chunks = (n_pairs + 63) / 64;
    const int pitch = n_sizes_max * n_chunks;
    const size_t lds = (size_t)REPLAY_WAVES * pitch * sizeof(uint64_t);
    const dim3 grid((total_pos + REPLAY_WAVES - 1) / REPLAY_WAVES), block(REPLAY_WAVES * 64);
    if (n_chunks == 1 && n_sizes_max <= 3)
        hipLaunchKernelGGL(k_replay_condense_carry<3>, grid, block, 0, stream, total_pos, P, regions, pos_region, pos_local, scores, records, copy, cand_base, emitted,
                           survivors, emitted_per_region);
    else if (n_chunks == 1 && n_sizes_max <= 5)
        hipLaunchKernelGGL(k_replay_condense_carry<5>, grid, block, 0, stream, total_pos, P, regions, pos_region, pos_local, scores, records, copy, cand_base, emitted,
                           survivors, emitted_per_region);
    else if (n_chunks == 1 && n_sizes_max <= 8)
        hipLaunchKernelGGL(k_replay_condense_carry<8>, grid, block, 0, stream, total_pos, P, regions, pos_region, pos_local, scores, records, copy, cand_base, emitted,
                           survivors, emitted_per_region);
    else if (n_chunks == 1)
        if (n_sizes_max > 2 * REPLAY_ROWS)
            hipLaunchKernelGGL(k_replay_condense_narrow<true>, grid, block, lds, stream, total_pos, pitch, P, regions, pos_region, pos_local, scores, records, copy,
                               cand_base, emitted, survivors, emitted_per_region);
        else
            hipLaunchKernelGGL(k_replay_condense_narrow<false>, grid, block, lds, stream, total_pos, pitch, P, regions, pos_region, pos_local, scores, records, copy,
                               cand_base, emitted, survivors, emitted_per_region);
    else
        hipLaunchKernelGGL(k_replay_condense, grid, block, lds, stream, total_pos, n_chunks, pitch, P, regions, pos_region, pos_local, scores, records,
                           copy, cand_base, emitted, survivors, emitted_per_region);
    return hipGetLastError();
}


__global__ __launch_bounds__(256) void k_collapse(int n_tiles, const CollapseTile* __restrict__ tiles, const DevParams* __restrict__ P,
                                                  const DevRegion* __restrict__ regions, const int64_t* __restrict__ region_pos0,
                                                  const int64_t* __restrict__ region_base0, const mipgen_survivor* __restrict__ survivors,
                                                  const int32_t* __restrict__ copy, int64_t cand_base, int32_t* __restrict__ collapsed)
{
    extern __shared__ __align__(16) unsigned char col_smem[];
    const CollapseTile t = tiles[blockIdx.x];
    const DevRegion& R = regions[t.region];
    const int A = P->n_pairs, nK = R.n_sizes;
    const int max_scan = P->max_capture - R.k0 * P->inc - P->min_sum;
    const int n_base = R.n_pos + max_scan - 1;
    if (nK <= 0) return;
    const int p_lo = max(0, t.j0 - max_scan + 1), p_hi = min(t.j0 + 127, R.n_pos - 1), n_sv = 2 * (p_hi - p_lo + 1);
    double* s_score = (double*)col_smem;
    int* s_end = (int*)(s_score + max(n_sv, 0));
    int* s_snp = s_end + max(n_sv, 0);
    const int64_t per_pos = (int64_t)nK * A * 2;
    const mipgen_survivor* sv = survivors + 2 * region_pos0[t.region];
    const int target = P->target_arm_copy;
    const int64_t max_product = P->max_arm_copy_product;
    const double thr = P->masked_arm_threshold;
    for (int q = threadIdx.x; q < n_sv; q += blockDim.x) {
        const int pi = p_lo + (q >> 1), s = q & 1;
        const mipgen_survivor m = sv[2 * (int64_t)pi + s];
        int end = -1, snp = 0;
        if (m.cand_index >= 0) {
            const int rel = (int)(m.cand_index - cand_base - R.out_off - (int64_t)pi * per_pos);
            const int a = rel % A, ki = rel / (2 * A);
            const int e = P->arm_ext[a], l = P->arm_lig[a];
            const int C = P->max_capture - (R.k0 + ki) * P->inc, ss = C - e - l;
            const ArmStarts st = arm_starts(R.first_pos + pi, ss, e, l, s != 0);
            const int ext_copy = true_arm_copy(P, R, copy, st.ext, e, MIPGEN_REC_EXT_COPY(m.record));
            const int lig_copy = true_arm_copy(P, R, copy, st.lig, l, MIPGEN_REC_LIG_COPY(m.record));
            const bool keep = !((int64_t)ext_copy * lig_copy > max_product || ext_copy > target || lig_copy > target)
                              && !((double)MIPGEN_REC_MASKED_N(m.record) / (double)(l + e) > thr);
            if (keep) end = pi + ss - 1;
            snp = (int)MIPGEN_REC_SNP_COUNT(m.record);
        }
        s_end[q] = end; s_snp[q] = snp; s_score[q] = m.score;
    }
    __syncthreads();
    const int j = t.j0 + (threadIdx.x >> 1), s = threadIdx.x & 1;
    if (j >= n_base) return;
    int best = -1, best_snp = 0;
    double best_score = 0.0;
    for (int pi = max(0, j - max_scan + 1); pi <= min(j, R.n_pos - 1); pi++) {
        const int q = 2 * (pi - p_lo) + s;
        if (s_end[q] < j) continue;
        const int snp = s_snp[q];
        const double sc = s_score[q];
        if (best < 0 || snp < best_snp || (sc > best_score && snp == best_snp)) { best = pi; best_snp = snp; best_score = sc; }
    }
    collapsed[region_base0[t.region] + 2 * (int64_t)j + s] = best;
}

extern "C" hipError_t mipgen_launch_collapse(hipStream_t stream, int n_tiles, const CollapseTile* tiles, const DevParams* P, const DevRegion* regions,
                                             const int64_t* region_pos0, const int64_t* region_base0, const mipgen_survivor* survivors,
                                             const int32_t* copy, int64_t cand_base, int32_t* collapsed, int max_scan_all)
{
    if (n_tiles <= 0) return hipSuccess;
    const size_t lds = (size_t)2 * (size_t)(128 + (max_scan_all > 0 ? max_scan_all : 0)) * 16;
    if (lds > 160 * 1024) return hipErrorInvalidValue;
    if (lds > 48 * 1024) { hipError_t e = hipFuncSetAttribute((const void*)k_collapse, hipFuncAttributeMaxDynamicSharedMemorySize, (int)lds); if (e != hipSuccess) return e; }
    hipLaunchKernelGGL(k_collapse, dim3(n_tiles), dim3(256), lds, stream, n_tiles, tiles, P, regions, region_pos0, region_base0, survivors, copy, cand_base, collapsed);
    return hipGetLastError();
}

__global__ __launch_bounds__(256) void k_fill_pos_map(const int64_t* __restrict__ region_pos0, int n_regions, int64_t total, int32_t* __restrict__ pos_region,
                                                      int32_t* __restrict__ pos_local)
{
    const int64_t i = (int64_t)blockIdx.x * blockDim.x + threadIdx.x;
    if (i >= total) return;
    int lo = 0, hi = n_regions - 1;
    while (lo < hi) {
        const int mid = (lo + hi + 1) >> 1;
        if (region_pos0[mid] <= i) lo = mid; else hi = mid - 1;
    }
    pos_region[i] = lo;
    pos_local[i] = (int32_t)(i - region_pos0[lo]);
}

extern "C" hipError_t mipgen_launch_fill_pos_map(hipStream_t stream, const int64_t* region_pos0, int n_regions, int64_t total, int32_t* pos_region, int32_t* pos_local)
{
    if (total <= 0 || n_regions <= 0) return hipSuccess;
    hipLaunchKernelGGL(k_fill_pos_map, dim3((unsigned)((total + 255) / 256)), dim3(256), 0, stream, region_pos0, n_regions, total, pos_region, pos_local);
    return hipGetLastError();
}
```

Baseline: 1.874 billion.

## Add table-based SVR record kernel and fold count memsets into kernels

Adds a new k_records_tables kernel for the SVR path. Each tile precomputes per-arm window entries (copy, masked, SNP and junction counts) in LDS and reuses them across all candidate rows of that tile, where the old records_logistic pass computed them per candidate. It also folds the per-region emitted-count zeroing into that kernel and the print-boundary list-count zeroing into the replay kernel, removing two hipMemsetAsync calls per window. The cost is a new large-LDS kernel whose tile size depends on a host-side layout search, plus more coupling between stages.

```diff
diff --git a/mipgen_amd/csrc/accel.hip b/mipgen_amd/csrc/accel.hip
--- a/mipgen_amd/csrc/accel.hip
+++ b/mipgen_amd/csrc/accel.hip
@@ -139,7 +139,7 @@
     h->locus_ins.release();
     h->locus_ins_call.release();
     h->model.release(); h->model_t.release(); h->sv_norm.release(); h->sv_coef.release(); h->sv_center.release(); h->regions.release(); h->bases.release(); h->unmap.release(); h->copy.release();
-    h->log_tiles.release(); h->svr_tiles.release(); h->ld_tiles.release(); h->scores.release(); h->records.release();
+    h->log_tiles.release(); h->rec_tiles.release(); h->svr_tiles.release(); h->ld_tiles.release(); h->scores.release(); h->records.release();
     h->emitted.release(); h->survivors.release(); h->emitted_per_region.release(); h->pos_region.release(); h->pos_local.release();
     h->letters.release(); h->fmt_regions.release(); h->fmt_pool.release(); h->fmt_text.release(); h->scan_temp.release();
     h->fmt_a.release(); h->fmt_b.release(); h->fmt_c.release(); h->fmt_d.release();
@@ -458,7 +458,7 @@
     for (Window& w : h->windows) {
         w.col_tile0 = (int)ct.size();
         w.base0 = h->h_region_base0[(size_t)w.r0]; w.n_base_entries = h->h_region_base0[(size_t)w.r1] - w.base0;
-        w.log_tile0 = w.n_log_tiles = w.svr_tile0 = w.n_svr_tiles = w.ld_tile0 = w.n_ld_tiles = 0;
+        w.log_tile0 = w.n_log_tiles = w.rec_tile0 = w.n_rec_tiles = w.svr_tile0 = w.n_svr_tiles = w.ld_tile0 = w.n_ld_tiles = 0;
         for (int i = w.r0; i < w.r1; i++) {
             const DevRegion& d = h->hregions[i];
             if (d.n_pos <= 0 || d.n_sizes <= 0) continue;
@@ -468,7 +468,7 @@
     }
     h->record_tiles_ready = h->logistic_tiles_ready = h->svr_tiles_ready = false;
     h->svr_batch_error.clear();
-    h->ld_lds = 0; h->log_span_max = 0; h->svr_lds = 0;
+    h->ld_lds = 0; h->log_span_max = 0; h->rec_lds = 0; h->svr_lds = 0;
     DIAG_LAP("tiles");
     if (h->scores.reserve((size_t)std::max<int64_t>(win_cand_max, 1)) || h->records.reserve((size_t)std::max<int64_t>(win_cand_max, 1)) ||
         h->emitted.reserve((size_t)std::max<int64_t>(win_cand_max, 1)))
diff --git a/mipgen_amd/csrc/accel_internal.h b/mipgen_amd/csrc/accel_internal.h
--- a/mipgen_amd/csrc/accel_internal.h
+++ b/mipgen_amd/csrc/accel_internal.h
@@ -36,6 +36,7 @@
     int64_t cand0 = 0, n_cand = 0;
     int64_t pos0 = 0, n_pos = 0;
     int log_tile0 = 0, n_log_tiles = 0, svr_tile0 = 0, n_svr_tiles = 0, col_tile0 = 0, n_col_tiles = 0, ld_tile0 = 0, n_ld_tiles = 0;
+    int rec_tile0 = 0, n_rec_tiles = 0;
     int n_svr_few = 0;
     std::vector<int> lvl_tile0;
     int lvl0_few = 0;
@@ -369,7 +370,8 @@
     DevBuf<int32_t> copy;
     std::vector<int32_t> resident_lens;
     std::vector<mipgen_big_copy> big_copies;
-    DevBuf<LogTile> log_tiles;
+    DevBuf<LogTile> log_tiles, rec_tiles;
+    size_t rec_lds = 0;
     DevBuf<SvrTile> svr_tiles, ld_tiles;
     size_t ld_lds = 0;
     int log_span_max = 0;
diff --git a/mipgen_amd/csrc/accel_score.hip b/mipgen_amd/csrc/accel_score.hip
--- a/mipgen_amd/csrc/accel_score.hip
+++ b/mipgen_amd/csrc/accel_score.hip
@@ -28,7 +28,7 @@
     return {LIST_BATCH, {h->dp, h->regions.p, cands, h->bases.p, h->copy.p, h->unmap.p}, {}};
 }
 
-static int rescore(mipgen_accel* h, const RescoreSrc& src, int method, const ProbeSrc* ps = nullptr)
+static int rescore(mipgen_accel* h, const RescoreSrc& src, int method, const ProbeSrc* ps = nullptr, bool count_zeroed = false)
 {
     const bool sat = src.kind == RESCORE_SATURATED;
     if (!sat && (!h->print_exact || src.n <= 0 || (method == MIPGEN_SCORE_SVR && h->n_sv <= 0))) return MIPGEN_OK;
@@ -37,7 +37,7 @@
     if ((!ps && L.cands.reserve(lim.cap)) || L.idx.reserve(lim.cap) || L.vals.reserve(lim.cap) || L.count.reserve(1)) return MIPGEN_E_NOMEM;
     if (sat) HIP_TRY(mipgen_launch_index_candidates(h->stream, h->dp, h->regions.p, src.r0, src.r1, L.idx.p, L.count.p, lim.cap, L.cands.p));
     else {
-        HIP_TRY(hipMemsetAsync(L.count.p, 0, sizeof(unsigned int), h->stream));
+        if (!count_zeroed) HIP_TRY(hipMemsetAsync(L.count.p, 0, sizeof(unsigned int), h->stream));
         HIP_TRY(mipgen_launch_print_boundary_scan(h->stream, h->dp, h->regions.p, &src, lim.tol_rel, lim.tol_abs, L.cands.p, L.idx.p, L.count.p, lim.cap, h->n_cu));
     }
     ListSrc listed = list_src(h, L.cands.p, ps);
@@ -57,10 +57,10 @@
     return MIPGEN_OK;
 }
 
-static int fix_survivor_print_boundaries(mipgen_accel* h, int w, int method)
+static int fix_survivor_print_boundaries(mipgen_accel* h, int w, int method, bool count_zeroed)
 {
     const Window& W = h->windows[(size_t)w];
-    return rescore(h, {RESCORE_SURV, 2 * W.n_pos, nullptr, nullptr, nullptr, h->survivors.p + 2 * W.pos0, W.r0, W.r1, W.cand0}, method);
+    return rescore(h, {RESCORE_SURV, 2 * W.n_pos, nullptr, nullptr, nullptr, h->survivors.p + 2 * W.pos0, W.r0, W.r1, W.cand0}, method, nullptr, count_zeroed);
 }
 
 static bool list_is_batched(int n, int method, bool want_scores) { return method == MIPGEN_SCORE_SVR && n >= 256 && want_scores; }
@@ -102,8 +102,9 @@
     return MIPGEN_OK;
 }
 
-static int score_window_impl(mipgen_accel* h, int w, int32_t method, bool fix_dense = true)
-{
+static int score_window_impl(mipgen_accel* h, int w, int32_t method, bool fused = false, bool* counts_zeroed = nullptr)
+{
+    const bool fix_dense = !fused;
     if (int rc = mipgen_ensure_tiles(h, method)) return rc;
     const Window& W = h->windows[(size_t)w];
     const bool svr_via_list = method == MIPGEN_SCORE_SVR && (!h->svr_geometry_error.empty() || !h->svr_batch_error.empty());
@@ -120,7 +121,12 @@
     if (method == MIPGEN_SCORE_LOGISTIC && h->ld_lds > 0)
         HIP_TRY(mipgen_launch_logistic_dense(h->stream, W.n_ld_tiles, h->ld_lds, h->dp, h->regions.p, h->ld_tiles.p + W.ld_tile0, h->bases.p, h->copy.p,
                                              h->unmap.p, h->dconsts, h->scores.p, h->records.p, h->sat.idx.p, h->sat.count.p, sat_cap));
-    else
+    else if (method == MIPGEN_SCORE_SVR && h->rec_lds > 0) {
+        const bool zero_counts = fused && W.n_rec_tiles > 0 && W.r1 > W.r0;
+        HIP_TRY(mipgen_launch_records_tables(h->stream, W.n_rec_tiles, h->rec_lds, h->dp, h->regions.p, h->rec_tiles.p + W.rec_tile0, h->bases.p, h->copy.p, h->unmap.p,
+                                             h->records.p, zero_counts ? h->emitted_per_region.p + W.r0 : nullptr, zero_counts ? W.r1 - W.r0 : 0));
+        if (counts_zeroed) *counts_zeroed = zero_counts;
+    } else
         HIP_TRY(mipgen_launch_records_logistic(h->stream, method == MIPGEN_SCORE_LOGISTIC, W.n_log_tiles, h->log_span_max, h->dp, h->regions.p,
                                                h->log_tiles.p + W.log_tile0, h->bases.p, h->copy.p, h->unmap.p, h->dconsts, h->scores.p, h->records.p,
                                                sat_cap ? h->sat.idx.p : nullptr, sat_cap ? h->sat.count.p : nullptr, sat_cap));
@@ -176,15 +182,16 @@
     return MIPGEN_OK;
 }
 
-static int replay_window_impl(mipgen_accel* h, bool want_mask)
+static int replay_window_impl(mipgen_accel* h, bool want_mask, bool counts_zeroed = false, unsigned int* zero_word = nullptr)
 {
     const int w = h->cur_window;
     const Window& W = h->windows[(size_t)w];
-    if (W.r1 > W.r0) HIP_TRY(hipMemsetAsync(h->emitted_per_region.p + W.r0, 0, (size_t)(W.r1 - W.r0) * sizeof(unsigned long long), h->stream));
+    if (W.r1 > W.r0 && !counts_zeroed)
+        HIP_TRY(hipMemsetAsync(h->emitted_per_region.p + W.r0, 0, (size_t)(W.r1 - W.r0) * sizeof(unsigned long long), h->stream));
     if (want_mask && W.n_cand) HIP_TRY(hipMemsetAsync(h->emitted.p, 0, (size_t)W.n_cand, h->stream));
     HIP_TRY(mipgen_launch_replay_condense(h->stream, (int)W.n_pos, h->dp, h->hp.n_pairs, h->hp.n_sizes_all, h->regions.p, h->pos_region.p + W.pos0,
                                           h->pos_local.p + W.pos0, h->scores.p, h->records.p, h->copy.p, W.cand0, want_mask ? h->emitted.p : nullptr,
-                                          h->survivors.p + 2 * W.pos0, h->emitted_per_region.p));
+                                          h->survivors.p + 2 * W.pos0, h->emitted_per_region.p, zero_word));
     if (h->timing && h->ev.size() >= 4 * ((size_t)w + 1)) { HIP_TRY(hipEventRecord(h->ev[4 * (size_t)w + 3], h->stream)); h->ev_used[(size_t)w] |= 2; }
     h->win_state[(size_t)w] = (uint8_t)((h->win_state[(size_t)w] & WIN_TEXT) | WIN_SURVIVORS | (want_mask ? WIN_MASK : 0));
     return MIPGEN_OK;
@@ -231,21 +238,30 @@
     return mipgen_accel_score_window(h, 0, method);
 }
 
+static int score_condense_impl(mipgen_accel* h, int w, int32_t method)
+{
+    bool counts_zeroed = false;
+    if (int rc = score_window_impl(h, w, method, true, &counts_zeroed)) return rc;
+    unsigned int* list_count = nullptr;
+    if (h->print_exact && h->windows[(size_t)w].n_pos > 0) {
+        if (h->pb.count.reserve(1)) return MIPGEN_E_NOMEM;
+        list_count = h->pb.count.p;
+    }
+    if (int rc = replay_window_impl(h, false, counts_zeroed, list_count)) return rc;
+    return fix_survivor_print_boundaries(h, w, method, list_count != nullptr);
+}
+
 int mipgen_accel_score_condense_window(mipgen_accel* h, int32_t w, int32_t method)
 {
     if (int rc = begin_scoring_call(h, method, w)) return rc;
-    if (int rc = score_window_impl(h, w, method, false)) return rc;
-    if (int rc = replay_window_impl(h, false)) return rc;
-    return fix_survivor_print_boundaries(h, w, method);
+    return score_condense_impl(h, w, method);
 }
 
 int mipgen_accel_score_condense_all(mipgen_accel* h, int32_t method)
 {
     if (int rc = begin_scoring_call(h, method, 0)) return rc;
     for (int w = 0; w < (int)h->windows.size(); w++) {
-        if (int rc = score_window_impl(h, w, method, false)) return rc;
-        if (int rc = replay_window_impl(h, false)) return rc;
-        if (int rc = fix_survivor_print_boundaries(h, w, method)) return rc;
+        if (int rc = score_condense_impl(h, w, method)) return rc;
         if (int rc = collapse_window_impl(h)) return rc;
     }
     return MIPGEN_OK;
diff --git a/mipgen_amd/csrc/accel_tiles.hip b/mipgen_amd/csrc/accel_tiles.hip
--- a/mipgen_amd/csrc/accel_tiles.hip
+++ b/mipgen_amd/csrc/accel_tiles.hip
@@ -53,6 +53,27 @@
     if (h->log_tiles.reserve(std::max<size_t>(lt.size(), 1))) return MIPGEN_E_NOMEM;
     if (!lt.empty()) HIP_TRY(hipMemcpy(h->log_tiles.p, lt.data(), lt.size() * sizeof(LogTile), hipMemcpyHostToDevice));
     h->log_span_max = span_max;
+    std::vector<LogTile> rt;
+    size_t rec_lds = 0;
+    bool rec_ok = true;
+    for (Window& w : h->windows) {
+        w.rec_tile0 = (int)rt.size();
+        for (int i = w.r0; i < w.r1 && rec_ok; i++) {
+            const DevRegion& d = h->hregions[i];
+            if (d.n_pos <= 0 || d.n_sizes <= 0) continue;
+            size_t b = 0;
+            const int np = mipgen_records_tile_positions(d.n_pos, d.n_sizes, D.max_capture - d.k0 * D.inc, D.inc, D.min_sum, D.max_sum, D.e_min, D.e_max, D.l_min, D.l_max,
+                                                         D.n_pairs, &b);
+            if (np < 1) { rec_ok = false; break; }
+            rec_lds = std::max(rec_lds, b);
+            for (int p0 = 0; p0 < d.n_pos; p0 += np) { LogTile t = {i, p0, std::min(np, d.n_pos - p0), 0}; rt.push_back(t); }
+        }
+        w.n_rec_tiles = (int)rt.size() - w.rec_tile0;
+    }
+    if (!rec_ok) { for (Window& w : h->windows) { w.rec_tile0 = 0; w.n_rec_tiles = 0; } rt.clear(); rec_lds = 0; }
+    if (h->rec_tiles.reserve(std::max<size_t>(rt.size(), 1))) return MIPGEN_E_NOMEM;
+    if (!rt.empty()) HIP_TRY(hipMemcpy(h->rec_tiles.p, rt.data(), rt.size() * sizeof(LogTile), hipMemcpyHostToDevice));
+    h->rec_lds = rec_lds;
     h->record_tiles_ready = true;
     return MIPGEN_OK;
 }
diff --git a/mipgen_amd/csrc/kernels.h b/mipgen_amd/csrc/kernels.h
--- a/mipgen_amd/csrc/kernels.h
+++ b/mipgen_amd/csrc/kernels.h
@@ -65,6 +65,10 @@
 size_t mipgen_logistic_lds_bytes(int span);
 hipError_t mipgen_launch_records_logistic(hipStream_t, int score, int n_tiles, int span_max, const DevParams*, const DevRegion*, const LogTile*, const uint8_t*, const int32_t*,
                                           const uint8_t*, const HostConsts*, double*, uint64_t*, int64_t* sat_idx, unsigned int* sat_count, unsigned int sat_cap);
+int mipgen_records_tile_positions(int n_pos, int n_sizes, int Cmax, int inc, int min_sum, int max_sum, int e_min, int e_max, int l_min, int l_max, int n_pairs,
+                                  size_t* lds_bytes);
+hipError_t mipgen_launch_records_tables(hipStream_t, int n_tiles, size_t lds_bytes, const DevParams*, const DevRegion*, const LogTile*, const uint8_t*, const int32_t*,
+                                        const uint8_t*, uint64_t* records, unsigned long long* zero, int n_zero);
 size_t mipgen_logistic_dense_lds_bytes(int np_all, int np, int ssr, int ssmax, int Lmax, int n_up, int n_dn);
 hipError_t mipgen_launch_logistic_dense(hipStream_t, int n_tiles, size_t lds_bytes, const DevParams*, const DevRegion*, const SvrTile*, const uint8_t*, const int32_t*,
                                         const uint8_t*, const HostConsts*, double*, uint64_t*, int64_t* sat_idx, unsigned int* sat_count, unsigned int sat_cap);
@@ -98,7 +102,7 @@
 hipError_t mipgen_launch_long_range(hipStream_t, int n, const char* seqs, const int64_t* offs, const int32_t* lens, const int32_t* denoms, const LrcMers*, double* out);
 hipError_t mipgen_launch_replay_condense(hipStream_t, int total_pos, const DevParams*, int n_pairs, int n_sizes_max, const DevRegion*, const int32_t* pos_region,
                                          const int32_t* pos_local, const double* scores, const uint64_t* records, const int32_t* copy, int64_t cand_base, uint8_t* emitted,
-                                         mipgen_survivor* survivors, unsigned long long* emitted_per_region);
+                                         mipgen_survivor* survivors, unsigned long long* emitted_per_region, unsigned int* zero_word);
 hipError_t mipgen_launch_collapse(hipStream_t, int n_tiles, const CollapseTile* tiles, const DevParams*, const DevRegion*, const int64_t* region_pos0,
                                   const int64_t* region_base0, const mipgen_survivor* survivors, const int32_t* copy, int64_t cand_base, int32_t* collapsed, int max_scan_all);
 hipError_t mipgen_launch_fill_pos_map(hipStream_t, const int64_t* region_pos0, int n_regions, int64_t total, int32_t* pos_region, int32_t* pos_local);
diff --git a/mipgen_amd/csrc/kernels_logistic.hip b/mipgen_amd/csrc/kernels_logistic.hip
--- a/mipgen_amd/csrc/kernels_logistic.hip
+++ b/mipgen_amd/csrc/kernels_logistic.hip
@@ -104,6 +104,156 @@
     }
 }
 
+struct RecLayout {
+    int span;
+    int n_e, n_l;
+    int ss_lo, nd;
+    int nu;
+    int n_ent;
+    int off_tab, off_pairs, off_um, off_sb, bytes;
+};
+__host__ __device__ static inline RecLayout rec_layout(int np, int n_sizes, int Cmax, int inc, int min_sum, int max_sum, int e_min, int e_max, int l_min, int l_max,
+                                                       int n_pairs)
+{
+    RecLayout L;
+    const int Lmax = e_max > l_max ? e_max : l_max, Lmin = e_min < l_min ? e_min : l_min;
+    L.span = np + Cmax + Lmax;
+    L.n_e = e_max - e_min + 1; L.n_l = l_max - l_min + 1;
+    const int ss_hi = Cmax - min_sum, ss_min = Cmax - (n_sizes - 1) * inc - max_sum;
+    L.ss_lo = ss_min > 1 ? ss_min : 1;
+    L.nd = ss_hi >= L.ss_lo ? np + ss_hi - L.ss_lo : 0;
+    L.nu = np + Lmax - Lmin;
+    L.n_ent = (np + L.nd) * (L.n_e + L.n_l);
+    int b = (int)(prefix_words_u64(L.span) * sizeof(uint64_t));
+    L.off_tab = b; b += L.n_ent * 8;
+    L.off_pairs = b; b += (n_pairs * 2 + 7) & ~7;
+    L.off_um = b; b += n_sizes * L.nu;
+    L.off_sb = b; b += L.span;
+    L.bytes = (b + 16 + 15) & ~15;
+    return L;
+}
+
+__device__ __forceinline__ uint64_t arm_window_entry(const PrefixWords& W, const DevParams* P, const DevRegion& R, const int32_t* __restrict__ copy, int lo, int span,
+                                                     int s, int len, int jmode)
+{
+    if (s < 0 || s + len > span) return 0;
+    const ArmCounts c = arm_window(W, s, len);
+    const uint32_t cp = (uint32_t)min(max(oligo_copy(P, R, copy, lo + s, len), 0), 65535);
+    const uint32_t jc = jmode ? lig_junction(W.sb, s, len, jmode == 2) : 0u;
+    return (uint64_t)cp | ((uint64_t)min(c.masked, 255u) << 16) | ((uint64_t)min(c.snp_any, 255u) << 24) | ((uint64_t)min(c.snp_bad, 255u) << 32) |
+           ((uint64_t)min(c.snp_ok, 255u) << 40) | ((uint64_t)min(c.bad, 255u) << 48) | ((uint64_t)jc << 56);
+}
+
+__global__ __launch_bounds__(LOG_THREADS) void k_records_tables(
+    const DevParams* __restrict__ P, const DevRegion* __restrict__ regions, const LogTile* __restrict__ tiles, int n_tiles, const uint8_t* __restrict__ bases,
+    const int32_t* __restrict__ copy, const uint8_t* __restrict__ unmap, uint64_t* __restrict__ records, unsigned long long* __restrict__ zero, int n_zero)
+{
+    extern __shared__ __align__(16) unsigned char smem[];
+    const int tid = threadIdx.x;
+    if (zero) for (int i = blockIdx.x * LOG_THREADS + tid; i < n_zero; i += gridDim.x * LOG_THREADS) zero[i] = 0ull;
+    const LogTile tile = tiles[xcd_remap(blockIdx.x, n_tiles)];
+    const DevRegion& R = regions[tile.region];
+
+    const int A = P->n_pairs, nK = R.n_sizes, inc = P->inc;
+    const int Cmax = P->max_capture - R.k0 * inc;
+    const int e_min = P->e_min, l_min = P->l_min;
+    const int Lmax = max(P->e_max, P->l_max);
+    const int np = tile.np;
+    const RecLayout L = rec_layout(np, nK, Cmax, inc, P->min_sum, P->max_sum, e_min, P->e_max, l_min, P->l_max, A);
+    const int p_first = R.first_pos + tile.p0;
+    const int lo = p_first - Lmax;
+    const int span = L.span, n_e = L.n_e, n_l = L.n_l, nd = L.nd, nu = L.nu;
+
+    PrefixWords W = prefix_words_carve(smem, span);
+    uint64_t* tab = (uint64_t*)(smem + L.off_tab);
+    uint16_t* pairs = (uint16_t*)(smem + L.off_pairs);
+    uint8_t* um = smem + L.off_um;
+    W.sb = smem + L.off_sb;
+
+    for (int a = tid; a < A; a += LOG_THREADS) pairs[a] = (uint16_t)(P->arm_ext[a] | (P->arm_lig[a] << 8));
+    const bool tested = mapping_tested(P, R);
+    if (tested)
+        for (int t = tid; t < nK * nu; t += LOG_THREADS) {
+            const int ki = t / nu, ms = lo + (t - ki * nu) - R.seq_start;
+            um[t] = (ms >= 0 && ms < R.seq_len && unmapped_at(R, unmap, R.k0 + ki, ms)) ? 1 : 0;
+        }
+    prefix_words_build<LOG_THREADS>(W, R, bases, lo, span);
+
+    const int oUL = np * n_e, oDL = np * (n_e + n_l), oDE = oDL + nd * n_l;
+    for (int t = tid; t < L.n_ent; t += LOG_THREADS) {
+        int s, len, jmode;
+        if (t < oUL) { const int pl = t / n_e; len = e_min + (t - pl * n_e); s = Lmax + pl - len; jmode = 0; }
+        else if (t < oDL) { const int u = t - oUL, pl = u / n_l; len = l_min + (u - pl * n_l); s = Lmax + pl - len; jmode = 2; }
+        else if (t < oDE) { const int u = t - oDL, d = u / n_l; len = l_min + (u - d * n_l); s = Lmax + L.ss_lo + d; jmode = 1; }
+        else { const int u = t - oDE, d = u / n_e; len = e_min + (u - d * n_e); s = Lmax + L.ss_lo + d; jmode = 0; }
+        tab[t] = arm_window_entry(W, P, R, copy, lo, span, s, len, jmode);
+    }
+    __syncthreads();
+
+    const uint32_t row = (uint32_t)(2 * A);
+    const uint32_t per_pos = row * (uint32_t)nK;
+    const uint32_t n_cand = per_pos * (uint32_t)np;
+    const uint32_t M_row = 0xFFFFFFFFu / row + 1, M_k = 0xFFFFFFFFu / (uint32_t)nK + 1;
+    const int64_t out_base = R.out_off + (int64_t)tile.p0 * per_pos;
+    const double thr = P->masked_arm_threshold;
+
+    for (uint32_t idx = tid; idx < n_cand; idx += LOG_THREADS) {
+        uint32_t rc = fastdiv(idx, M_row);
+        uint32_t in_row = idx - rc * row;
+        uint32_t pl = nK == 1 ? rc : fastdiv(rc, M_k);
+        uint32_t ki = rc - pl * (uint32_t)nK;
+        const bool minus = in_row >= (uint32_t)A;
+        const int a = (int)(minus ? in_row - (uint32_t)A : in_row);
+        const uint32_t pr = pairs[a];
+        const int e = (int)(pr & 255u), l = (int)(pr >> 8);
+        const int C = Cmax - (int)ki * inc;
+        const int ss = C - e - l;
+        const int p = p_first + (int)pl;
+
+        uint64_t rec = 0;
+        if (constructed(R, p, C, e, l)) {
+            const int d = (int)pl + ss - L.ss_lo, ce = e - e_min, cl = l - l_min;
+            const uint64_t xe = tab[minus ? oDE + d * n_e + ce : (int)pl * n_e + ce];
+            const uint64_t xl = tab[minus ? oUL + (int)pl * n_l + cl : oDL + d * n_l + cl];
+            const bool mapping = tested && um[(int)ki * nu + Lmax + (int)pl - (minus ? l : e)] != 0;
+            auto f8 = [](uint64_t x, int sh) { return (int)((x >> sh) & 255u); };
+            const bool guard = (f8(xe, 48) + f8(xl, 48)) != 0;
+            const int masked_n = f8(xe, 16) + f8(xl, 16);
+            int snp_count;
+            const uint32_t flags = record_flags(mapping, masked_n, l + e, thr, f8(xe, 24) + f8(xl, 24), f8(xe, 32) + f8(xl, 32), f8(xe, 40) + f8(xl, 40), guard,
+                                                snp_count);
+            rec = pack_record((int)(xe & 65535u), (int)(xl & 65535u), masked_n, snp_count, flags, (uint32_t)(xl >> 56));
+        }
+        records[out_base + idx] = rec;
+    }
+}
+
+#define REC_NP_MAX 8
+extern "C" int mipgen_records_tile_positions(int n_pos, int n_sizes, int Cmax, int inc, int min_sum, int max_sum, int e_min, int e_max, int l_min, int l_max, int n_pairs,
+                                             size_t* lds_bytes)
+{
+    int np = n_pos < REC_NP_MAX ? (n_pos > 1 ? n_pos : 1) : REC_NP_MAX;
+    size_t b = 0;
+    for (; np >= 1; np--) {
+        b = (size_t)rec_layout(np, n_sizes, Cmax, inc, min_sum, max_sum, e_min, e_max, l_min, l_max, n_pairs).bytes;
+        if (b <= 80 * 1024) break;
+    }
+    if (lds_bytes) *lds_bytes = b;
+    return np;
+}
+
+extern "C" hipError_t mipgen_launch_records_tables(hipStream_t stream, int n_tiles, size_t lds_bytes, const DevParams* P, const DevRegion* regions, const LogTile* tiles,
+                                                   const uint8_t* bases, const int32_t* copy, const uint8_t* unmap, uint64_t* records, unsigned long long* zero, int n_zero)
+{
+    if (n_tiles <= 0) return hipSuccess;
+    if (lds_bytes > 48 * 1024) {
+        hipError_t e = hipFuncSetAttribute((const void*)k_records_tables, hipFuncAttributeMaxDynamicSharedMemorySize, (int)lds_bytes);
+        if (e != hipSuccess) return e;
+    }
+    hipLaunchKernelGGL(k_records_tables, dim3(n_tiles), dim3(LOG_THREADS), lds_bytes, stream, P, regions, tiles, n_tiles, bases, copy, unmap, records, zero, n_zero);
+    return hipGetLastError();
+}
+
 extern "C" size_t mipgen_logistic_lds_bytes(int span)
 {
     return (prefix_words_u64(span) + LOG_RINV) * sizeof(uint64_t) + (size_t)span + 16;
diff --git a/mipgen_amd/csrc/kernels_replay.hip b/mipgen_amd/csrc/kernels_replay.hip
--- a/mipgen_amd/csrc/kernels_replay.hip
+++ b/mipgen_amd/csrc/kernels_replay.hip
@@ -195,8 +195,9 @@
     int total_pos, int n_chunks, int lds_pitch, const DevParams* __restrict__ P, const DevRegion* __restrict__ regions,
     const int32_t* __restrict__ pos_region, const int32_t* __restrict__ pos_local, const double* __restrict__ scores,
     const uint64_t* __restrict__ records, const int32_t* __restrict__ copy, int64_t cand_base, uint8_t* __restrict__ emitted,
-    mipgen_survivor* __restrict__ survivors, unsigned long long* __restrict__ emitted_per_region)
-{
+    mipgen_survivor* __restrict__ survivors, unsigned long long* __restrict__ emitted_per_region, unsigned int* __restrict__ zero_word)
+{
+    if (zero_word && blockIdx.x == 0 && threadIdx.x == 0) *zero_word = 0u;
     extern __shared__ uint64_t s_masks[];
     const int lane = threadIdx.x & 63;
     const int wave = __builtin_amdgcn_readfirstlane(threadIdx.x >> 6);
@@ -295,8 +296,9 @@
     int total_pos, int lds_pitch, const DevParams* __restrict__ P, const DevRegion* __restrict__ regions,
     const int32_t* __restrict__ pos_region, const int32_t* __restrict__ pos_local, const double* __restrict__ scores,
     const uint64_t* __restrict__ records, const int32_t* __restrict__ copy, int64_t cand_base, uint8_t* __restrict__ emitted,
-    mipgen_survivor* __restrict__ survivors, unsigned long long* __restrict__ emitted_per_region)
-{
+    mipgen_survivor* __restrict__ survivors, unsigned long long* __restrict__ emitted_per_region, unsigned int* __restrict__ zero_word)
+{
+    if (zero_word && blockIdx.x == 0 && threadIdx.x == 0) *zero_word = 0u;
     extern __shared__ uint64_t s_masks[];
     const int lane = threadIdx.x & 63;
     const int wave = __builtin_amdgcn_readfirstlane(threadIdx.x >> 6);
@@ -422,8 +424,9 @@
     int total_pos, const DevParams* __restrict__ P, const DevRegion* __restrict__ regions,
     const int32_t* __restrict__ pos_region, const int32_t* __restrict__ pos_local, const double* __restrict__ scores,
     const uint64_t* __restrict__ records, const int32_t* __restrict__ copy, int64_t cand_base, uint8_t* __restrict__ emitted,
-    mipgen_survivor* __restrict__ survivors, unsigned long long* __restrict__ emitted_per_region)
-{
+    mipgen_survivor* __restrict__ survivors, unsigned long long* __restrict__ emitted_per_region, unsigned int* __restrict__ zero_word)
+{
+    if (zero_word && blockIdx.x == 0 && threadIdx.x == 0) *zero_word = 0u;
     const int lane = threadIdx.x & 63;
     const int gp = blockIdx.x * REPLAY_WAVES + __builtin_amdgcn_readfirstlane(threadIdx.x >> 6);
     if (gp >= total_pos) return;
@@ -475,7 +478,7 @@
 extern "C" hipError_t mipgen_launch_replay_condense(
     hipStream_t stream, int total_pos, const DevParams* P, int n_pairs, int n_sizes_max, const DevRegion* regions,
     const int32_t* pos_region, const int32_t* pos_local, const double* scores, const uint64_t* records, const int32_t* copy, int64_t cand_base,
-    uint8_t* emitted, mipgen_survivor* survivors, unsigned long long* emitted_per_region)
+    uint8_t* emitted, mipgen_survivor* survivors, unsigned long long* emitted_per_region, unsigned int* zero_word)
 {
     if (total_pos <= 0) return hipSuccess;
     const int n_chunks = (n_pairs + 63) / 64;
@@ -484,23 +487,23 @@
     const dim3 grid((total_pos + REPLAY_WAVES - 1) / REPLAY_WAVES), block(REPLAY_WAVES * 64);
     if (n_chunks == 1 && n_sizes_max <= 3)
         hipLaunchKernelGGL(k_replay_condense_carry<3>, grid, block, 0, stream, total_pos, P, regions, pos_region, pos_local, scores, records, copy, cand_base, emitted,
-                           survivors, emitted_per_region);
+                           survivors, emitted_per_region, zero_word);
     else if (n_chunks == 1 && n_sizes_max <= 5)
         hipLaunchKernelGGL(k_replay_condense_carry<5>, grid, block, 0, stream, total_pos, P, regions, pos_region, pos_local, scores, records, copy, cand_base, emitted,
-                           survivors, emitted_per_region);
+                           survivors, emitted_per_region, zero_word);
     else if (n_chunks == 1 && n_sizes_max <= 8)
         hipLaunchKernelGGL(k_replay_condense_carry<8>, grid, block, 0, stream, total_pos, P, regions, pos_region, pos_local, scores, records, copy, cand_base, emitted,
-                           survivors, emitted_per_region);
+                           survivors, emitted_per_region, zero_word);
     else if (n_chunks == 1)
         if (n_sizes_max > 2 * REPLAY_ROWS)
             hipLaunchKernelGGL(k_replay_condense_narrow<true>, grid, block, lds, stream, total_pos, pitch, P, regions, pos_region, pos_local, scores, records, copy,
-                               cand_base, emitted, survivors, emitted_per_region);
+                               cand_base, emitted, survivors, emitted_per_region, zero_word);
         else
             hipLaunchKernelGGL(k_replay_condense_narrow<false>, grid, block, lds, stream, total_pos, pitch, P, regions, pos_region, pos_local, scores, records, copy,
-                               cand_base, emitted, survivors, emitted_per_region);
+                               cand_base, emitted, survivors, emitted_per_region, zero_word);
     else
         hipLaunchKernelGGL(k_replay_condense, grid, block, lds, stream, total_pos, n_chunks, pitch, P, regions, pos_region, pos_local, scores, records,
-                           copy, cand_base, emitted, survivors, emitted_per_region);
+                           copy, cand_base, emitted, survivors, emitted_per_region, zero_word);
     return hipGetLastError();
 }
 
```

Result: no change. 1.888 billion (median of 6 runs) (+0.7%).
